# Tongji-MIC-Lab/TDVC

Measured on AMD Instinct MI355X. Metric: 1080p P-frames/sec (encode + reconstruct, lambda=2048 config), higher is better.
Workload: dtype f16; 1 GPU; 1x 1920x1080 (padded 1088x1920) 7-frame synthetic GOP (seed 1234), batch 1, P-frames coded in GOP order; gop=7, batch=1, parallelism=gop-sharded x1, weights=closed-form filler (no checkpoint ships)

## Files before the change

include/tdvc_hip.h:

```cpp
#ifndef TDVC_HIP_H
#define TDVC_HIP_H

#include <stdint.h>

#ifdef __cplusplus
extern "C" {
#endif

#define TDVC_OK 0
#define TDVC_EINVAL (-1)
#define TDVC_ENOSUP (-2)

typedef struct {
  void* p;
  int32_t N, H, W, C;
  int64_t sn;
  int32_t sp;
  int32_t dtype;
} tdvc_fmap;

enum { TDVC_F16 = 0, TDVC_F32 = 1 };
enum { TDVC_ACT_NONE = 0, TDVC_ACT_RELU = 1, TDVC_ACT_LRELU = 2, TDVC_ACT_CLAMP01 = 3, TDVC_ACT_SIGMOID = 4 };
enum { TDVC_GDN_NONE = 0, TDVC_GDN_FWD = 1, TDVC_GDN_INV = 2 };
enum { TDVC_OUT_NHWC = 0,
       TDVC_OUT_SHUFFLE2 = 1,
       TDVC_OUT_NCHW_F32 = 2 };

#define TDVC_MAX_TAPS 49

typedef struct {
  tdvc_fmap x;
  tdvc_fmap y;
  const void* w;
  const float* bias;
  int32_t cout;
  int32_t ntaps;
  int8_t tap_dy[TDVC_MAX_TAPS], tap_dx[TDVC_MAX_TAPS];
  int32_t kh, kw, stride, pad;
  int32_t ck;
  int32_t square_input;
  int32_t gdn;
  tdvc_fmap aux;
  int32_t act; float slope;
  int32_t round_before_act;
  tdvc_fmap res;
  tdvc_fmap res2;
  int32_t out_mode;
  int32_t s2d;
  int32_t bcast_T;
  float bcast_slope;
  float* chan_sum;
} tdvc_conv_desc;

int tdvc_abi_version(void);
const char* tdvc_last_error(void);
int tdvc_prepare_device(void);
const char* tdvc_last_conv_kernel(void);


int tdvc_conv_plan(int cin, int kh, int kw, int stride);
int64_t tdvc_conv_packed_bytes(int cout, int cin, int ntaps, int ck);
int tdvc_pack_conv_weights(const float* w_oihw, int cout, int cin_real, int cin, int kh, int kw,
                           int ntaps, const int8_t* tap_dy, const int8_t* tap_dx, int ck, uint16_t* dst);
int tdvc_conv2d(const tdvc_conv_desc* d, void* stream);
int tdvc_conv_chan_sum_rows(const tdvc_conv_desc* d);
int tdvc_conv2d_f32(const tdvc_conv_desc* d, void* stream);

typedef struct {
  tdvc_fmap x, y;
  const void* w;
  const float* bias;
  int32_t act1; float slope1;
  int32_t act2; float slope2;
  int32_t add_input;
  tdvc_fmap res2;
} tdvc_conv_pair_desc;
int64_t tdvc_conv_pair_packed_bytes(void);
int tdvc_pack_conv_pair_weights(const float* w1_oihw, const float* w2_oihw, uint16_t* dst);
int tdvc_conv_pair_supported(const tdvc_conv_pair_desc* d);
int tdvc_conv_pair(const tdvc_conv_pair_desc* d, void* stream);

typedef struct {
  tdvc_fmap x, om, y;
  const void* w;
  const float* bias;
  int32_t groups;
  int32_t act; float slope; int32_t round_before_act;
  void* x_planar;
} tdvc_dcn_desc;
int tdvc_dcn_fused(const tdvc_dcn_desc* d, void* stream);

int tdvc_dcn_v2_forward_f32(const float* input, const float* weight, const float* bias,
                            const float* offset, const float* mask, float* output,
                            int B, int C, int H, int W, int Cout,
                            int kh, int kw, int sh, int sw, int ph, int pw, int dh, int dw,
                            int deformable_group, void* stream);
int tdvc_dcn_v2_backward_f32(const float* input, const float* weight, const float* bias,
                             const float* offset, const float* mask, const float* grad_output,
                             float* grad_input, float* grad_offset, float* grad_mask,
                             float* grad_weight, float* grad_bias, float* columns,
                             int B, int C, int H, int W, int Cout,
                             int kh, int kw, int sh, int sw, int ph, int pw, int dh, int dw,
                             int deformable_group, void* stream);

int tdvc_nchw_to_fmap(const float* src, int C, const tdvc_fmap* y, void* stream);
int tdvc_fmap_to_nchw(const tdvc_fmap* x, int C, float* dst, void* stream);
int tdvc_scale_act_res(const tdvc_fmap* a, const float* gate, int act, float slope,
                       const tdvc_fmap* r, float r_sign, const tdvc_fmap* y, const tdvc_fmap* y2, void* stream);
int tdvc_add_flow(const tdvc_fmap* off, const tdvc_fmap* flow, void* stream);
int tdvc_bcast_add_act(const tdvc_fmap* x, const tdvc_fmap* b, int T, float slope, void* stream);

int tdvc_channel_sum(const tdvc_fmap* x, float* partial, int nblocks, void* stream);
int tdvc_se_gate(const float* partial, int nblocks, float inv_count, int N, int C, int Cmid,
                 const float* w1, const float* b1, const float* w2, const float* b2,
                 float* gate, void* stream);

int tdvc_upsample2x(const tdvc_fmap* x, const tdvc_fmap* y, void* stream);
int tdvc_avgpool2(const tdvc_fmap* x, const tdvc_fmap* y, void* stream);
int tdvc_spynet_level_input(const tdvc_fmap* ref, const tdvc_fmap* supp, const tdvc_fmap* flow_lo,
                            const tdvc_fmap* flow_up, const tdvc_fmap* cat8, void* stream);
int tdvc_resize_bilinear(const tdvc_fmap* x, const tdvc_fmap* y, const float* chscale, void* stream);

int64_t tdvc_avgpool_k_work_floats(int N, int hp, int wp, int C, int scale);
int tdvc_avgpool_k(const tdvc_fmap* x, int scale, float* pooled, int hp, int wp, float* work, int64_t work_floats, void* stream);
int tdvc_patch_match(const float* pin, const float* pref, int N, int hp, int wp, int C,
                     int32_t* idx, void* stream);
int tdvc_match_gather(const tdvc_fmap* fin, const tdvc_fmap* fref, const int32_t* idx, int scale,
                      int hp, int wp, const tdvc_fmap* cat, void* stream);

int tdvc_eb_forward(const tdvc_fmap* z, const float* params, const tdvc_fmap* noise,
                    const tdvc_fmap* z_hat, double* bits_out, float* partial, int partial_cap, void* stream);
int tdvc_gc_forward(const tdvc_fmap* y, const tdvc_fmap* gp, const tdvc_fmap* noise,
                    double* bits_out, float* partial, int partial_cap, void* stream);
int tdvc_quantize(const tdvc_fmap* y, const tdvc_fmap* noise, const tdvc_fmap* y_hat, void* stream);

int64_t tdvc_rans_encode(const int32_t* symbols, const int32_t* indexes, int64_t n,
                         const int32_t* cdfs, int32_t cdf_stride, const int32_t* cdf_sizes,
                         const int32_t* offsets, uint8_t* out, int64_t cap);
int tdvc_rans_decode(const uint8_t* data, int64_t nbytes, const int32_t* indexes, int64_t n,
                     const int32_t* cdfs, int32_t cdf_stride, const int32_t* cdf_sizes,
                     const int32_t* offsets, int32_t* symbols_out);

void* tdvc_rans_decoder_create(const uint8_t* data, int64_t nbytes);
int tdvc_rans_decoder_decode(void* handle, const int32_t* indexes, int64_t n, const int32_t* cdfs,
                             int32_t cdf_stride, const int32_t* cdf_sizes, const int32_t* offsets,
                             int32_t* symbols_out);
void tdvc_rans_decoder_destroy(void* handle);

int tdvc_pmf_to_quantized_cdf(const float* pmf, int n, int precision, int32_t* cdf_out);

int tdvc_ar_gather(const tdvc_fmap* y_hat, const tdvc_fmap* params, const int32_t* pos, int npos,
                   const tdvc_fmap* x1, const tdvc_fmap* pc, void* stream);
int tdvc_ar_quantize(const tdvc_fmap* y, const tdvc_fmap* gp, const int32_t* pos, int npos,
                     const float* scale_table, int ntable, const int32_t* symbols_in,
                     const tdvc_fmap* y_hat, int32_t* symbols, int32_t* indexes, void* stream);
int tdvc_ar_indexes(const tdvc_fmap* gp, const int32_t* pos, int npos, const float* scale_table, int ntable,
                    int M, int W, int32_t* indexes, void* stream);
int tdvc_ar_decode_serial(const uint8_t* data, int64_t nbytes, const int32_t* cdfs, int32_t cdf_stride, const int32_t* cdf_sizes,
                          const int32_t* offsets, const tdvc_fmap* y_hat, const tdvc_fmap* params, const tdvc_fmap* x1,
                          const tdvc_fmap* pc, const tdvc_conv_desc* convs, int nconvs, const tdvc_fmap* gp,
                          const int32_t* pos_table, int npos_total, int M, int W, const float* scale_table, int ntable,
                          int32_t* idx_dev, int32_t* sym_dev, void* stream);
int tdvc_ar_wavefront(const uint8_t* data, int64_t nbytes, const int32_t* cdfs, int32_t cdf_stride, const int32_t* cdf_sizes,
                      const int32_t* offsets, const tdvc_fmap* y, const tdvc_fmap* y_hat, const tdvc_fmap* params,
                      const tdvc_fmap* x1, const tdvc_fmap* pc, const tdvc_conv_desc* convs, int nconvs, const tdvc_fmap* gp,
                      const int32_t* pos_dev, const int32_t* step_sizes, int nsteps, int M, int W,
                      const float* scale_table, int ntable, int32_t* idx_dev, int32_t* sym_dev, void* stream);
int tdvc_round_symbols(const tdvc_fmap* z, const float* median, int32_t* out, void* stream);

int tdvc_pack_conv_weights_indexed(const float* w, const int32_t* row_off, const int32_t* chan_off, const int32_t* tap_off,
                                   const uint8_t* row_mask, const uint8_t* chan_mask, const uint8_t* tap_mask,
                                   int cout, int cin, int ntaps, int ck, void* dst, void* stream);
int tdvc_pack_conv_weights_indexed_f32(const float* w, const int32_t* row_off, const int32_t* chan_off, const int32_t* tap_off,
                                       const uint8_t* row_mask, const uint8_t* chan_mask, const uint8_t* tap_mask,
                                       int cout, int cin, int ntaps, int ck, float* dst, void* stream);
typedef struct tdvc_pack_job {
  const float* w;
  const int32_t *row_off, *chan_off, *tap_off;
  const uint8_t *row_mask, *chan_mask, *tap_mask;
  void* dst;
  const float* bias_src;
  float* bias_dst;
  const int32_t* bias_perm;
  int32_t cout, cin, ntaps, ck;
} tdvc_pack_job;
int64_t tdvc_pack_job_blocks(int cout, int cin, int ntaps, int ck);
int tdvc_pack_conv_weights_batch(const tdvc_pack_job* jobs, const int32_t* block_start, int njobs, int total_blocks, void* stream);
int64_t tdvc_conv_wgrad_work_floats(int cout, int cin, int ntaps, int N, int Ho, int Wo);
int tdvc_conv_wgrad(const tdvc_fmap* g, const tdvc_fmap* x, int cout, int kh, int kw, int stride, int pad,
                    int ntaps, const int8_t* tap_dy, const int8_t* tap_dx, const int32_t* row_off, const int32_t* chan_off,
                    const int32_t* tap_off, int square_x, float scale, float* dw, float* work, int64_t work_floats, void* stream);
int tdvc_conv_wgrad_bias(const tdvc_fmap* g, const tdvc_fmap* x, int cout, int kh, int kw, int stride, int pad,
                         int ntaps, const int8_t* tap_dy, const int8_t* tap_dx, const int32_t* row_off, const int32_t* chan_off,
                         const int32_t* tap_off, int square_x, float scale, float* dw, const int32_t* bias_index, float* db,
                         float* work, int64_t work_floats, void* stream);

typedef struct tdvc_wgrad_reduce_job {
  const float* work;
  const float* bwork;
  const int32_t *row_off, *chan_off, *tap_off, *bias_index;
  float *dw, *db;
  float scale;
  int32_t nworkers, cow, ciw, ntaps, cout, cin, wblocks, nblocks;
} tdvc_wgrad_reduce_job;
int tdvc_conv_wgrad_partials(const tdvc_fmap* g, const tdvc_fmap* x, int cout, int kh, int kw, int stride, int pad,
                             int ntaps, const int8_t* tap_dy, const int8_t* tap_dx, const int32_t* row_off, const int32_t* chan_off,
                             const int32_t* tap_off, int square_x, float scale, float* dw, const int32_t* bias_index, float* db,
                             float* work, int64_t work_floats, tdvc_wgrad_reduce_job* job, void* stream);
int tdvc_wgrad_reduce_batch(const tdvc_wgrad_reduce_job* jobs, const int32_t* block_start, int njobs, int total_blocks, void* stream);

int tdvc_act_backward(const tdvc_fmap* g, const tdvc_fmap* y, const tdvc_fmap* res, int act, float slope, const tdvc_fmap* out, void* stream);
int tdvc_pixel_unshuffle(const tdvc_fmap* y, const tdvc_fmap* out, void* stream);
int64_t tdvc_bias_grad_work_floats(int N, int C);
int tdvc_bias_grad(const tdvc_fmap* g, int nvalid, const int32_t* dst_index, float scale, float* db, float* work, int64_t work_floats, void* stream);

int tdvc_copy_cast(const tdvc_fmap* src, const tdvc_fmap* dst, void* stream);
int tdvc_clamp01_backward(const tdvc_fmap* g, const tdvc_fmap* y, void* stream);
int64_t tdvc_gate_backward_work_floats(int N, int C);
int tdvc_gate_backward(const tdvc_fmap* g, const tdvc_fmap* a, const float* gate, const tdvc_fmap* da, float* dgate, float* work,
                       int64_t work_floats, void* stream);
int tdvc_se_gate_backward(const float* partial, int nblocks, float inv_count, int N, int C, int Cmid, const float* w1, const float* b1,
                          const float* w2, const float* b2, const float* gate, const float* dgate, float scale, float* dmean,
                          float* dw1, float* db1, float* dw2, float* db2, void* stream);
int tdvc_bcast_channel_add(const tdvc_fmap* dx, const float* v, float scale, void* stream);
int tdvc_add_flow_backward(const tdvc_fmap* doff, const tdvc_fmap* dflow, void* stream);
int tdvc_bcast_add_act_backward(const tdvc_fmap* dx, const tdvc_fmap* x, const tdvc_fmap* db, float slope, void* stream);
int tdvc_upsample2x_backward(const tdvc_fmap* dy, const tdvc_fmap* dx, void* stream);
int tdvc_resize_bilinear_backward(const tdvc_fmap* dy, const tdvc_fmap* dx, const float* chscale, void* stream);

int tdvc_spynet_level_input_backward(const tdvc_fmap* supp, const tdvc_fmap* flow_up, const tdvc_fmap* dcat8, const tdvc_fmap* dflow_up,
                                     const tdvc_fmap* dflow_lo, void* stream);

int tdvc_sigmoid_f32(const float* x, float* out, int64_t n, void* stream);
int tdvc_sigmoid_backward_f32(float* g, const float* s, int64_t n, void* stream);
int tdvc_axpy_f32(float* dst, const float* src, float scale, int64_t n, void* stream);

int tdvc_match_gather_backward(const tdvc_fmap* fin, const tdvc_fmap* fref, const int32_t* idx, int scale, int hp, int wp,
                               const tdvc_fmap* dcat, const tdvc_fmap* dfin, const tdvc_fmap* dfref, void* stream);

int tdvc_gdn_backward(const tdvc_fmap* g, const tdvc_fmap* x, const tdvc_fmap* n32, int inverse, const tdvc_fmap* dn, const tdvc_fmap* dx, void* stream);
int tdvc_mul2_accumulate(const tdvc_fmap* dx, const tdvc_fmap* x, const tdvc_fmap* t, void* stream);

int tdvc_eb_backward(const tdvc_fmap* z, const float* params, const tdvc_fmap* noise, float gscale, const tdvc_fmap* dz, float* dparams, void* stream);
int tdvc_gc_backward(const tdvc_fmap* y, const tdvc_fmap* gp, const tdvc_fmap* noise, float gscale, const tdvc_fmap* dy, const tdvc_fmap* dgp, void* stream);
int tdvc_eb_pack(const float* const* raw, const float* quantiles, float* packed, int C, void* stream);
int tdvc_eb_param_chain(const float* dpacked, const float* const* raw, float* const* grad, float scale, int C, void* stream);
int tdvc_eb_aux(const float* params, const float* quantiles, float target, float* dq, float* loss, int C, void* stream);

int tdvc_dcn_columns(const tdvc_fmap* x, const tdvc_fmap* om, int groups, const tdvc_fmap* col, void* stream);
int64_t tdvc_dcn_col2im_work_floats(int N, int H, int W, int groups);
int tdvc_dcn_col2im(const tdvc_fmap* x, const tdvc_fmap* om, const tdvc_fmap* dcol, int groups, float* dx32, const tdvc_fmap* dom,
                    float* work, int64_t work_floats, void* stream);
int tdvc_dcn_col2im_det(const tdvc_fmap* x, const tdvc_fmap* om, const tdvc_fmap* dcol, int groups, float* dx32, const tdvc_fmap* dom,
                        float* work, int64_t work_floats, int64_t* far_keys, float* far_vals, int32_t* far_count, int32_t far_cap, void* stream);
int tdvc_dcn_far_apply(const int64_t* keys_sorted, const int64_t* order, const float* far_vals, int32_t count, float* dx32, void* stream);

int64_t tdvc_ssim_level_work_floats(int N, int C, int H, int W, int win_size);
int tdvc_ssim_level(const float* x, const float* y, int N, int C, int H, int W, const float* win, int win_size,
                    float c1, float c2, float* ssim_out, float* cs_out, float* work, int64_t work_floats, void* stream);
int tdvc_avgpool2_pad_f32(const float* x, int64_t planes, int H, int W, float* out, void* stream);

#ifdef __cplusplus
}
#endif
#endif
```

tdvc_amd/_lib.py:

```python
from __future__ import annotations

import ctypes as C
import os

_HERE = os.path.dirname(os.path.abspath(__file__))
LIB_PATH = os.path.join(_HERE, "libtdvc_hip.so")

MAX_TAPS = 49
F16, F32 = 0, 1
ACT_NONE, ACT_RELU, ACT_LRELU, ACT_CLAMP01, ACT_SIGMOID = 0, 1, 2, 3, 4
GDN_NONE, GDN_FWD, GDN_INV = 0, 1, 2
OUT_NHWC, OUT_SHUFFLE2, OUT_NCHW_F32 = 0, 1, 2


class FMapDesc(C.Structure):
    _fields_ = [("p", C.c_void_p), ("N", C.c_int32), ("H", C.c_int32), ("W", C.c_int32), ("C", C.c_int32),
                ("sn", C.c_int64), ("sp", C.c_int32), ("dtype", C.c_int32)]


class ConvDesc(C.Structure):
    _fields_ = [("x", FMapDesc), ("y", FMapDesc), ("w", C.c_void_p), ("bias", C.c_void_p),
                ("cout", C.c_int32), ("ntaps", C.c_int32),
                ("tap_dy", C.c_int8 * MAX_TAPS), ("tap_dx", C.c_int8 * MAX_TAPS),
                ("kh", C.c_int32), ("kw", C.c_int32), ("stride", C.c_int32), ("pad", C.c_int32),
                ("ck", C.c_int32), ("square_input", C.c_int32), ("gdn", C.c_int32),
                ("aux", FMapDesc), ("act", C.c_int32), ("slope", C.c_float),
                ("round_before_act", C.c_int32), ("res", FMapDesc), ("res2", FMapDesc), ("out_mode", C.c_int32), ("s2d", C.c_int32),
                ("bcast_T", C.c_int32), ("bcast_slope", C.c_float), ("chan_sum", C.c_void_p)]


class DcnDesc(C.Structure):
    _fields_ = [("x", FMapDesc), ("om", FMapDesc), ("y", FMapDesc), ("w", C.c_void_p), ("bias", C.c_void_p),
                ("groups", C.c_int32), ("act", C.c_int32), ("slope", C.c_float), ("round_before_act", C.c_int32), ("x_planar", C.c_void_p)]


class ConvPairDesc(C.Structure):
    _fields_ = [("x", FMapDesc), ("y", FMapDesc), ("w", C.c_void_p), ("bias", C.c_void_p), ("act1", C.c_int32), ("slope1", C.c_float),
                ("act2", C.c_int32), ("slope2", C.c_float), ("add_input", C.c_int32), ("res2", FMapDesc)]


class WgradReduceJob(C.Structure):
    _fields_ = [("work", C.c_void_p), ("bwork", C.c_void_p), ("row_off", C.c_void_p), ("chan_off", C.c_void_p), ("tap_off", C.c_void_p),
                ("bias_index", C.c_void_p), ("dw", C.c_void_p), ("db", C.c_void_p), ("scale", C.c_float),
                ("nworkers", C.c_int32), ("cow", C.c_int32), ("ciw", C.c_int32), ("ntaps", C.c_int32), ("cout", C.c_int32), ("cin", C.c_int32),
                ("wblocks", C.c_int32), ("nblocks", C.c_int32)]


_P = C.c_void_p
_FM = C.POINTER(FMapDesc)
_i, _f, _i64 = C.c_int, C.c_float, C.c_int64

SIGNATURES = {
    "tdvc_abi_version": (_i, []),
    "tdvc_conv_chan_sum_rows": (_i, [C.POINTER(ConvDesc)]),
    "tdvc_last_error": (C.c_char_p, []),
    "tdvc_last_conv_kernel": (C.c_char_p, []),
    "tdvc_prepare_device": (_i, []),
    "tdvc_conv_plan": (_i, [_i, _i, _i, _i]),
    "tdvc_conv_packed_bytes": (_i64, [_i, _i, _i, _i]),
    "tdvc_pack_conv_weights": (_i, [_P, _i, _i, _i, _i, _i, _i, _P, _P, _i, _P]),
    "tdvc_conv2d": (_i, [C.POINTER(ConvDesc), _P]),
    "tdvc_conv2d_f32": (_i, [C.POINTER(ConvDesc), _P]),
    "tdvc_pack_conv_weights_indexed": (_i, [_P] * 7 + [_i] * 4 + [_P, _P]),
    "tdvc_pack_conv_weights_indexed_f32": (_i, [_P] * 7 + [_i] * 4 + [_P, _P]),
    "tdvc_pack_job_blocks": (_i64, [_i, _i, _i, _i]),
    "tdvc_pack_conv_weights_batch": (_i, [_P, _P, _i, _i, _P]),
    "tdvc_act_backward": (_i, [_FM, _FM, _FM, _i, _f, _FM, _P]),
    "tdvc_pixel_unshuffle": (_i, [_FM, _FM, _P]),
    "tdvc_bias_grad_work_floats": (_i64, [_i, _i]),
    "tdvc_bias_grad": (_i, [_FM, _i, _P, _f, _P, _P, _i64, _P]),
    "tdvc_copy_cast": (_i, [_FM, _FM, _P]),
    "tdvc_clamp01_backward": (_i, [_FM, _FM, _P]),
    "tdvc_gate_backward_work_floats": (_i64, [_i, _i]),
    "tdvc_gate_backward": (_i, [_FM, _FM, _P, _FM, _P, _P, _i64, _P]),
    "tdvc_se_gate_backward": (_i, [_P, _i, _f, _i, _i, _i] + [_P] * 6 + [_f] + [_P] * 6),
    "tdvc_bcast_channel_add": (_i, [_FM, _P, _f, _P]),
    "tdvc_add_flow_backward": (_i, [_FM, _FM, _P]),
    "tdvc_bcast_add_act_backward": (_i, [_FM, _FM, _FM, _f, _P]),
    "tdvc_upsample2x_backward": (_i, [_FM, _FM, _P]),
    "tdvc_resize_bilinear_backward": (_i, [_FM, _FM, _P, _P]),
    "tdvc_spynet_level_input_backward": (_i, [_FM, _FM, _FM, _FM, _FM, _P]),
    "tdvc_sigmoid_f32": (_i, [_P, _P, _i64, _P]),
    "tdvc_sigmoid_backward_f32": (_i, [_P, _P, _i64, _P]),
    "tdvc_axpy_f32": (_i, [_P, _P, _f, _i64, _P]),
    "tdvc_match_gather_backward": (_i, [_FM, _FM, _P, _i, _i, _i, _FM, _FM, _FM, _P]),
    "tdvc_eb_backward": (_i, [_FM, _P, _FM, _f, _FM, _P, _P]),
    "tdvc_eb_pack": (_i, [_P, _P, _P, _i, _P]),
    "tdvc_eb_param_chain": (_i, [_P, _P, _P, _f, _i, _P]),
    "tdvc_eb_aux": (_i, [_P, _P, _f, _P, _P, _i, _P]),
    "tdvc_gc_backward": (_i, [_FM, _FM, _FM, _f, _FM, _FM, _P]),
    "tdvc_dcn_columns": (_i, [_FM, _FM, _i, _FM, _P]),
    "tdvc_ar_decode_serial": (_i, [_P, _i64, _P, _i, _P, _P, _FM, _FM, _FM, _FM, _P, _i, _FM, _P, _i, _i, _i, _P, _i, _P, _P, _P]),
    "tdvc_ar_wavefront": (_i, [_P, _i64, _P, _i, _P, _P, _FM, _FM, _FM, _FM, _FM, _P, _i, _FM, _P, _P, _i, _i, _i, _P, _i, _P, _P, _P]),
    "tdvc_ssim_level_work_floats": (_i64, [_i] * 5),
    "tdvc_ssim_level": (_i, [_P, _P, _i, _i, _i, _i, _P, _i, _f, _f, _P, _P, _P, _i64, _P]),
    "tdvc_avgpool2_pad_f32": (_i, [_P, _i64, _i, _i, _P, _P]),
    "tdvc_dcn_col2im_work_floats": (_i64, [_i, _i, _i, _i]),
    "tdvc_dcn_col2im": (_i, [_FM, _FM, _FM, _i, _P, _FM, _P, _i64, _P]),
    "tdvc_dcn_col2im_det": (_i, [_FM, _FM, _FM, _i, _P, _FM, _P, _i64, _P, _P, _P, _i, _P]),
    "tdvc_dcn_far_apply": (_i, [_P, _P, _P, _i, _P, _P]),
    "tdvc_conv_wgrad_work_floats": (_i64, [_i] * 6),
    "tdvc_conv_wgrad": (_i, [_FM, _FM] + [_i] * 6 + [_P] * 5 + [_i, _f, _P, _P, _i64, _P]),
    "tdvc_conv_wgrad_bias": (_i, [_FM, _FM] + [_i] * 6 + [_P] * 5 + [_i, _f, _P, _P, _P, _P, _i64, _P]),
    "tdvc_conv_wgrad_partials": (_i, [_FM, _FM] + [_i] * 6 + [_P] * 5 + [_i, _f, _P, _P, _P, _P, _i64, C.POINTER(WgradReduceJob), _P]),
    "tdvc_wgrad_reduce_batch": (_i, [_P, _P, _i, _i, _P]),
    "tdvc_gdn_backward": (_i, [_FM, _FM, _FM, _i, _FM, _FM, _P]),
    "tdvc_mul2_accumulate": (_i, [_FM, _FM, _FM, _P]),
    "tdvc_dcn_fused": (_i, [C.POINTER(DcnDesc), _P]),
    "tdvc_conv_pair_packed_bytes": (_i64, []),
    "tdvc_pack_conv_pair_weights": (_i, [_P, _P, _P]),
    "tdvc_conv_pair_supported": (_i, [C.POINTER(ConvPairDesc)]),
    "tdvc_conv_pair": (_i, [C.POINTER(ConvPairDesc), _P]),
    "tdvc_dcn_v2_forward_f32": (_i, [_P] * 6 + [_i] * 14 + [_P]),
    "tdvc_dcn_v2_backward_f32": (_i, [_P] * 12 + [_i] * 14 + [_P]),
    "tdvc_nchw_to_fmap": (_i, [_P, _i, _FM, _P]),
    "tdvc_fmap_to_nchw": (_i, [_FM, _i, _P, _P]),
    "tdvc_scale_act_res": (_i, [_FM, _P, _i, _f, _FM, _f, _FM, _FM, _P]),
    "tdvc_add_flow": (_i, [_FM, _FM, _P]),
    "tdvc_bcast_add_act": (_i, [_FM, _FM, _i, _f, _P]),
    "tdvc_channel_sum": (_i, [_FM, _P, _i, _P]),
    "tdvc_se_gate": (_i, [_P, _i, _f, _i, _i, _i, _P, _P, _P, _P, _P, _P]),
    "tdvc_upsample2x": (_i, [_FM, _FM, _P]),
    "tdvc_avgpool2": (_i, [_FM, _FM, _P]),
    "tdvc_spynet_level_input": (_i, [_FM, _FM, _FM, _FM, _FM, _P]),
    "tdvc_resize_bilinear": (_i, [_FM, _FM, _P, _P]),
    "tdvc_avgpool_k_work_floats": (_i64, [_i, _i, _i, _i, _i]),
    "tdvc_avgpool_k": (_i, [_FM, _i, _P, _i, _i, _P, _i64, _P]),
    "tdvc_patch_match": (_i, [_P, _P, _i, _i, _i, _i, _P, _P]),
    "tdvc_match_gather": (_i, [_FM, _FM, _P, _i, _i, _i, _FM, _P]),
    "tdvc_eb_forward": (_i, [_FM, _P, _FM, _FM, _P, _P, _i, _P]),
    "tdvc_gc_forward": (_i, [_FM, _FM, _FM, _P, _P, _i, _P]),
    "tdvc_quantize": (_i, [_FM, _FM, _FM, _P]),
    "tdvc_rans_encode": (_i64, [_P, _P, _i64, _P, C.c_int32, _P, _P, _P, _i64]),
    "tdvc_rans_decode": (_i, [_P, _i64, _P, _i64, _P, C.c_int32, _P, _P, _P]),
    "tdvc_rans_decoder_create": (_P, [_P, _i64]),
    "tdvc_rans_decoder_decode": (_i, [_P, _P, _i64, _P, C.c_int32, _P, _P, _P]),
    "tdvc_rans_decoder_destroy": (None, [_P]),
    "tdvc_pmf_to_quantized_cdf": (_i, [_P, _i, _i, _P]),
    "tdvc_ar_gather": (_i, [_FM, _FM, _P, _i, _FM, _FM, _P]),
    "tdvc_ar_quantize": (_i, [_FM, _FM, _P, _i, _P, _i, _P, _FM, _P, _P, _P]),
    "tdvc_ar_indexes": (_i, [_FM, _P, _i, _P, _i, _i, _i, _P, _P]),
    "tdvc_round_symbols": (_i, [_FM, _P, _P, _P]),
}

_lib = None


class TdvcHipError(RuntimeError):
    pass


def lib():
    global _lib
    if _lib is None:
        if not os.path.exists(LIB_PATH):
            raise TdvcHipError(
                f"{LIB_PATH} is missing: build it with `python -c 'import __graft_entry__ as g; g.build()'` "
                "(hipcc --offload-arch=gfx950).  tdvc_amd has no CPU fallback.")
        l = C.CDLL(LIB_PATH)
        for name, (res, args) in SIGNATURES.items():
            fn = getattr(l, name)
            fn.restype = res
            fn.argtypes = args
        _lib = l
    return _lib


def check(rc: int, what: str = ""):
    if rc != 0:
        msg = lib().tdvc_last_error().decode("utf-8", "replace")
        raise TdvcHipError(f"{what}: rc={rc}: {msg}")
```

tdvc_amd/csrc/conv_mfma.hip:

```cpp
#include "conv_common.h"

using convk::ConvParams;
int launch_conv_v2(const ConvParams& p, int ntiles, int cout_blocks, int N, hipStream_t st);
bool conv_v2_eligible(const tdvc_conv_desc* d, int Ho, int Wo);
int launch_conv_v3(const ConvParams& p, int cout_blocks, int N, hipStream_t st);
bool conv_v3_eligible(const tdvc_conv_desc* d, int Ho, int Wo);
int launch_conv_v5(const ConvParams& p, int cout_blocks, int N, hipStream_t st);
bool conv_v5_eligible(const tdvc_conv_desc* d, int Ho, int Wo);
int conv_v5_chan_sum_rows(int Ho, int Wo, int cout_blocks, int N);
int launch_conv_v7(const ConvParams& p, int cout_blocks, int N, hipStream_t st);
bool conv_v7_eligible(const tdvc_conv_desc* d, const ConvParams& p, int Ho, int Wo);
int launch_conv_v11(const ConvParams& p, int cout_blocks, int N, hipStream_t st);
bool conv_v11_eligible(const tdvc_conv_desc* d, const ConvParams& p, int Ho, int Wo);
int launch_conv_row(int geo, const ConvParams& p, int N, hipStream_t st);
int conv_row_geometry(const tdvc_conv_desc* d, const ConvParams& p, int Ho, int Wo);
int launch_conv_v10(const ConvParams& p, int cout_blocks, int N, hipStream_t st);
bool conv_v10_eligible(const tdvc_conv_desc* d, const ConvParams& p, int Ho, int Wo);
int launch_conv_v9(const ConvParams& p, int ck8, int cout_tiles32, int N, hipStream_t st);
bool conv_v9_eligible(const tdvc_conv_desc* d, int Ho, int Wo, bool v3_ok);
bool conv_c8_eligible(const tdvc_conv_desc* d, const ConvParams& p, int Ho, int Wo);
int launch_conv_c8(const ConvParams& p, int N, hipStream_t st);
bool conv_n16_eligible(const tdvc_conv_desc* d, int Ho, int Wo);
int launch_conv_n16(const ConvParams& p, int N, hipStream_t st);
bool gdn128_eligible(const tdvc_conv_desc* d, const ConvParams& p, int Ho, int Wo);
int launch_gdn128(const ConvParams& p, int N, hipStream_t st);

namespace {

constexpr int TH = 8, TW = 32;

template <int CK8, int MT, int STRIDE, bool LEAN = false>
__global__ __launch_bounds__(256, LEAN ? 3 : 1) void conv_mfma_kernel(const ConvParams p) {
  extern __shared__ __attribute__((aligned(16))) unsigned char smem[];
  constexpr int CK = CK8 * 8;
  constexpr int PS = (CK8 == 1) ? 16 : CK * 2 + 16;
  int* tapoff = reinterpret_cast<int*>(smem);
  unsigned char* tile = smem + 256;

  const int tid = threadIdx.x, lane = tid & 63, wave = tid >> 6;
  const int hh = lane >> 5, r = lane & 31;
  const int tile_id = p.reverse ? (int)gridDim.x - 1 - tdvc_xcd_tile(blockIdx.x) : tdvc_xcd_tile(blockIdx.x);
  const int tx = tile_id % p.tiles_x, ty = tile_id / p.tiles_x;
  const int cb = blockIdx.y, n = blockIdx.z;

  const int TIH = (TH - 1) * STRIDE + p.kh;
  const int TIW = (TW - 1) * STRIDE + p.kw;
  const int HALFW = (TIW + 1) >> 1;
  const int TIWp = (STRIDE == 2) ? 2 * HALFW : TIW;

  if (tid < p.ntaps) {
    const int dy = p.tap_dy[tid], dx = p.tap_dx[tid];
    tapoff[tid] = (STRIDE == 2) ? (dy * TIWp + (dx & 1) * HALFW + (dx >> 1)) * PS : (dy * TIWp + dx) * PS;
  }

  int base[2];
#pragma unroll
  for (int nt = 0; nt < 2; ++nt) base[nt] = (((wave * 2 + nt) * STRIDE) * TIWp + r) * PS;

  f32x16 acc[MT][2];
#pragma unroll
  for (int mt = 0; mt < MT; ++mt)
#pragma unroll
    for (int nt = 0; nt < 2; ++nt)
#pragma unroll
      for (int i = 0; i < 16; ++i) acc[mt][nt][i] = 0.f;

  const half_t* xn = p.x + (long)n * p.x_sn;
  const int iy0 = ty * TH * STRIDE - p.pad, ix0 = tx * TW * STRIDE - p.pad;
  const int total = TIH * TIW * CK8;

  for (int ch = 0; ch < p.nchunks; ++ch) {
    if (ch > 0) __syncthreads();
    for (int idx = tid; idx < total; idx += 256) {
      const int c8 = idx % CK8;
      const int pix = idx / CK8;
      const int c = pix % TIW, rr = pix / TIW;
      const int iy = iy0 + rr, ix = ix0 + c;
      const int cg = ch * CK + c8 * 8;
      half8 v = {0, 0, 0, 0, 0, 0, 0, 0};
      if (iy >= 0 && iy < p.H && ix >= 0 && ix < p.W && cg < p.Cin)
        v = *reinterpret_cast<const half8*>(xn + ((long)iy * p.W + ix) * p.x_sp + cg);
      if (p.square) v = v * v;
      const int cpos = (STRIDE == 2) ? ((c & 1) * HALFW + (c >> 1)) : c;
      *reinterpret_cast<half8*>(tile + (rr * TIWp + cpos) * PS + c8 * 16) = v;
    }
    __syncthreads();

    const half_t* wp[MT];
#pragma unroll
    for (int mt = 0; mt < MT; ++mt)
      wp[mt] = p.w + ((((long)(cb * MT + mt) * p.nchunks + ch) * p.steps) * 64 + lane) * 8;

    if constexpr (CK8 == 1) {
      for (int s = 0; s < p.steps; ++s) {
        int tap = 2 * s + hh;
        tap = tap < p.ntaps ? tap : p.ntaps - 1;
        const int toff = tapoff[tap];
        half8 a[MT], b[2];
#pragma unroll
        for (int mt = 0; mt < MT; ++mt) { a[mt] = *reinterpret_cast<const half8*>(wp[mt]); wp[mt] += 512; }
#pragma unroll
        for (int nt = 0; nt < 2; ++nt) b[nt] = *reinterpret_cast<const half8*>(tile + base[nt] + toff);
#pragma unroll
        for (int mt = 0; mt < MT; ++mt)
#pragma unroll
          for (int nt = 0; nt < 2; ++nt)
            acc[mt][nt] = __builtin_amdgcn_mfma_f32_32x32x16_f16(a[mt], b[nt], acc[mt][nt], 0, 0, 0);
      }
    } else {
      for (int tap = 0; tap < p.ntaps; ++tap) {
        const int toff = tapoff[tap] + hh * 16;
#pragma unroll
        for (int s2 = 0; s2 < CK8 / 2; ++s2) {
          half8 a[MT], b[2];
#pragma unroll
          for (int mt = 0; mt < MT; ++mt) { a[mt] = *reinterpret_cast<const half8*>(wp[mt]); wp[mt] += 512; }
#pragma unroll
          for (int nt = 0; nt < 2; ++nt)
            b[nt] = *reinterpret_cast<const half8*>(tile + base[nt] + toff + s2 * 32);
#pragma unroll
          for (int mt = 0; mt < MT; ++mt)
#pragma unroll
            for (int nt = 0; nt < 2; ++nt)
              acc[mt][nt] = __builtin_amdgcn_mfma_f32_32x32x16_f16(a[mt], b[nt], acc[mt][nt], 0, 0, 0);
        }
      }
    }
  }

  if constexpr (MT == 2 && LEAN) {
    __syncthreads();
    convk::epilogue_simple_rows<2, false, 2>(p, acc, p.bias + cb * 64, tile + wave * (32 * 144), n, cb * 64,
                                             ty * TH + wave * 2, tx * TW, lane, false);
    return;
  } else if constexpr (MT == 2) {
    if (p.simple) {
      __syncthreads();
      convk::epilogue_simple_rows<2, false, 1>(p, acc, p.bias + cb * 64, tile + wave * (32 * 144), n, cb * 64,
                                               ty * TH + wave * 2, tx * TW, lane, false);
      return;
    }
  }
  const int ox = tx * TW + r;
#pragma unroll
  for (int nt = 0; nt < 2; ++nt) {
    const int oy = ty * TH + wave * 2 + nt;
    if (oy >= p.Ho || ox >= p.Wo) continue;
#pragma unroll
    for (int mt = 0; mt < MT; ++mt) {
#pragma unroll
      for (int g = 0; g < 4; ++g) {
        const int co = (cb * MT + mt) * 32 + 8 * g + 4 * hh;
        float v[4];
#pragma unroll
        for (int i = 0; i < 4; ++i) v[i] = acc[mt][nt][4 * g + i];
        convk::epilogue4(p, n, oy, ox, co, v);
      }
    }
  }
}

template <int CK8, int MT, int STRIDE>
int launch(const ConvParams& p, dim3 grid, size_t lds, hipStream_t st) {
  if constexpr (MT == 2) {
    if (p.simple == 2) {
      hipLaunchKernelGGL((conv_mfma_kernel<CK8, MT, STRIDE, true>), grid, dim3(256), lds, st, p);
      return tdvc_launch_status("tdvc_conv2d");
    }
  }
  hipLaunchKernelGGL((conv_mfma_kernel<CK8, MT, STRIDE, false>), grid, dim3(256), lds, st, p);
  return tdvc_launch_status("tdvc_conv2d");
}

template <int CK8, int MT>
int launch_s(const ConvParams& p, int stride, dim3 grid, size_t lds, hipStream_t st) {
  return stride == 1 ? launch<CK8, MT, 1>(p, grid, lds, st) : launch<CK8, MT, 2>(p, grid, lds, st);
}

template <int CK8>
int launch_m(const ConvParams& p, int mt, int stride, dim3 grid, size_t lds, hipStream_t st) {
  return mt == 1 ? launch_s<CK8, 1>(p, stride, grid, lds, st) : launch_s<CK8, 2>(p, stride, grid, lds, st);
}

inline int lds_bytes(int ck, int kh, int kw, int stride) {
  const int ps = (ck == 8) ? 16 : ck * 2 + 16;
  const int tih = (TH - 1) * stride + kh, tiw = (TW - 1) * stride + kw;
  const int tiwp = stride == 2 ? 2 * ((tiw + 1) >> 1) : tiw;
  return 256 + tih * tiwp * ps;
}

inline int cout_tiles(int cout) { return cout <= 32 ? 1 : 2 * ((cout + 63) / 64); }

}

extern "C" int tdvc_conv_plan(int cin, int kh, int kw, int stride) {
  if (cin <= 0 || (cin % 8) != 0 || kh < 1 || kw < 1 || kh > 7 || kw > 7 || (stride != 1 && stride != 2)) {
    tdvc_set_error("tdvc_conv_plan: unsupported geometry cin=%d k=%dx%d stride=%d", cin, kh, kw, stride);
    return TDVC_EINVAL;
  }
  const int cands[4] = {64, 32, 16, 8};
  for (int i = 0; i < 4; ++i) {
    const int ck = cands[i];
    if (ck > cin && ck != 8) {
      if (cin % ck != 0 && cin < ck) continue;
    }
    if (lds_bytes(ck, kh, kw, stride) <= 64 * 1024) return ck;
  }
  tdvc_set_error("tdvc_conv_plan: no LDS plan for k=%dx%d stride=%d", kh, kw, stride);
  return TDVC_EINVAL;
}

extern "C" int64_t tdvc_conv_packed_bytes(int cout, int cin, int ntaps, int ck) {
  if (cout <= 0 || cin <= 0 || ntaps <= 0 || ntaps > TDVC_MAX_TAPS || (ck != 8 && ck != 16 && ck != 32 && ck != 64)) return TDVC_EINVAL;
  const int ck8 = ck / 8;
  const int64_t nchunks = (cin + ck - 1) / ck;
  const int64_t steps = (ntaps * ck8 + 1) / 2;
  return (int64_t)cout_tiles(cout) * nchunks * steps * 64 * 8 * 2;
}

extern "C" int tdvc_pack_conv_weights(const float* w, int cout, int cin_real, int cin, int kh, int kw,
                                      int ntaps, const int8_t* tap_dy, const int8_t* tap_dx, int ck, uint16_t* dst) {
  TDVC_CHECK(w && dst && tap_dy && tap_dx, "tdvc_pack_conv_weights: null pointer");
  TDVC_CHECK(tdvc_conv_packed_bytes(cout, cin, ntaps, ck) > 0, "tdvc_pack_conv_weights: bad geometry");
  TDVC_CHECK(cin_real <= cin, "tdvc_pack_conv_weights: cin_real > cin");
  const int ck8 = ck / 8;
  const int nchunks = (cin + ck - 1) / ck;
  const int steps = (ntaps * ck8 + 1) / 2;
  const int tiles = cout_tiles(cout);
  half_t* out = reinterpret_cast<half_t*>(dst);
  for (int t = 0; t < tiles; ++t)
    for (int ch = 0; ch < nchunks; ++ch)
      for (int s = 0; s < steps; ++s)
        for (int lane = 0; lane < 64; ++lane) {
          const int r = lane & 31, h = lane >> 5;
          const int co = t * 32 + r;
          const int kc = 2 * s + h;
          half_t* o = out + ((((int64_t)t * nchunks + ch) * steps + s) * 64 + lane) * 8;
          for (int j = 0; j < 8; ++j) {
            float v = 0.f;
            if (kc < ntaps * ck8 && co < cout) {
              const int tap = kc / ck8, c8 = kc % ck8;
              const int ci = ch * ck + c8 * 8 + j;
              const int dy = tap_dy[tap], dx = tap_dx[tap];
              if (ci < cin_real && dy >= 0 && dy < kh && dx >= 0 && dx < kw)
                v = w[(((int64_t)co * cin_real + ci) * kh + dy) * kw + dx];
            }
            o[j] = (half_t)v;
          }
        }
  return TDVC_OK;
}

static thread_local char g_last_kernel[48] = "";

static thread_local unsigned g_walk_parity = 0;
static int g_walk_mode = -1;
extern "C" void tdvc_debug_set_conv_walk(int mode) { g_walk_mode = mode; }
static int next_walk_reverse() {
  if (g_walk_mode < 0) { const char* e = getenv("TDVC_CONV_WALK"); g_walk_mode = e ? atoi(e) : 1; }
  return g_walk_mode == 1 ? (int)(g_walk_parity++ & 1u) : 0;
}

static int conv2d_impl(const tdvc_conv_desc* d, void* stream, bool query_rows) {
  TDVC_CHECK(d, "tdvc_conv2d: null descriptor");
  if (d->x.dtype == TDVC_F32) {
    if (query_rows) return 0;
    TDVC_CHECK(!d->chan_sum, "tdvc_conv2d: chan_sum is not available on the fp32 path (tdvc_conv_chan_sum_rows() == 0)");
    snprintf(g_last_kernel, sizeof(g_last_kernel), "conv_f32");
    return tdvc_conv2d_f32(d, stream);
  }
  TDVC_CHECK(fmap_ok16(d->x), "tdvc_conv2d: input must be an fp16 fmap with C,sp %% 8 == 0 and 16-byte aligned");
  TDVC_CHECK(d->w && aligned16(d->w), "tdvc_conv2d: weights null/unaligned");
  TDVC_CHECK(d->stride == 1 || d->stride == 2, "tdvc_conv2d: stride %d unsupported", d->stride);
  TDVC_CHECK(d->ntaps >= 1 && d->ntaps <= TDVC_MAX_TAPS && d->kh >= 1 && d->kh <= 7 && d->kw >= 1 && d->kw <= 7,
             "tdvc_conv2d: bad kernel %dx%d ntaps=%d", d->kh, d->kw, d->ntaps);
  TDVC_CHECK(d->ck == 8 || d->ck == 16 || d->ck == 32 || d->ck == 64, "tdvc_conv2d: bad ck %d", d->ck);
  TDVC_CHECK(d->cout >= 1, "tdvc_conv2d: cout");
  for (int t = 0; t < d->ntaps; ++t)
    TDVC_CHECK(d->tap_dy[t] >= 0 && d->tap_dy[t] < d->kh && d->tap_dx[t] >= 0 && d->tap_dx[t] < d->kw,
               "tdvc_conv2d: tap %d out of the %dx%d window", t, d->kh, d->kw);
  int Ho = (d->x.H + 2 * d->pad - d->kh) / d->stride + 1;
  int Wo = (d->x.W + 2 * d->pad - d->kw) / d->stride + 1;
  if (d->s2d) {
    TDVC_CHECK(d->kh == 2 && d->kw == 2 && d->stride == 1 && d->pad == 1 && d->ntaps == 4 && d->ck == 32 && !d->square_input && !d->gdn,
               "tdvc_conv2d: s2d expects the virtual 2x2 / stride 1 / pad 1 conv packed with ck=32");
    TDVC_CHECK((d->x.H % 2) == 0 && (d->x.W % 2) == 0 && (d->x.C % 32) == 0 && d->cout >= 64,
               "tdvc_conv2d: s2d needs even H, W, C %% 32 == 0 and cout >= 64 (got %dx%dx%d, cout %d)", d->x.H, d->x.W, d->x.C, d->cout);
    Ho = d->x.H / 2;
    Wo = d->x.W / 2;
  }
  TDVC_CHECK(Ho > 0 && Wo > 0, "tdvc_conv2d: empty output");
  TDVC_CHECK((long)Ho * Wo * 4 < 2147483647L && (long)d->x.H * d->x.W < 2147483647L, "tdvc_conv2d: image too large (pixel indices are 32-bit)");
  const int lds = lds_bytes(d->ck, d->kh, d->kw, d->stride);

  const int shuf = d->out_mode == TDVC_OUT_SHUFFLE2;
  if (d->out_mode == TDVC_OUT_NCHW_F32) {
    TDVC_CHECK(d->y.p && d->y.N == d->x.N, "tdvc_conv2d: NCHW output null / batch mismatch");
  } else {
    TDVC_CHECK(d->y.dtype == TDVC_F32 ? fmap_ok32(d->y) : fmap_ok16(d->y), "tdvc_conv2d: bad output fmap");
    TDVC_CHECK(d->y.N == d->x.N && d->y.H == (shuf ? 2 * Ho : Ho) && d->y.W == (shuf ? 2 * Wo : Wo),
               "tdvc_conv2d: output geometry %dx%d does not match conv result %dx%d%s", d->y.H, d->y.W, Ho, Wo,
               shuf ? " (x2 shuffle)" : "");
    if (shuf) TDVC_CHECK((d->cout % 128) == 0, "tdvc_conv2d: SHUFFLE2 needs cout %% 128 == 0");
    if (d->y.dtype == TDVC_F16) TDVC_CHECK((d->y.C % 8) == 0, "tdvc_conv2d: fp16 output C %% 8");
  }
  if (d->gdn) {
    TDVC_CHECK(fmap_ok16(d->aux) && d->aux.H == Ho && d->aux.W == Wo && d->aux.N == d->x.N && d->aux.C >= d->cout &&
                   !shuf && (d->cout % 64) == 0,
               "tdvc_conv2d: GDN aux fmap mismatch");
  }
  if (d->res.p) {
    TDVC_CHECK(d->res.dtype == TDVC_F32 ? fmap_ok32(d->res) : fmap_ok16(d->res), "tdvc_conv2d: bad residual fmap");
    TDVC_CHECK(d->res.N == d->x.N && d->res.H == (shuf ? 2 * Ho : Ho) && d->res.W == (shuf ? 2 * Wo : Wo),
               "tdvc_conv2d: residual geometry mismatch");
  }
  if (d->res2.p) {
    TDVC_CHECK(fmap_ok16(d->res2) && d->res2.N == d->x.N && d->res2.H == (shuf ? 2 * Ho : Ho) && d->res2.W == (shuf ? 2 * Wo : Wo),
               "tdvc_conv2d: bad second residual fmap");
  }
  if (d->bias) TDVC_CHECK(aligned16(d->bias), "tdvc_conv2d: bias unaligned");

  ConvParams p;
  memset(&p, 0, sizeof(p));
  p.x = reinterpret_cast<const half_t*>(d->x.p); p.x_sn = d->x.sn; p.x_sp = d->x.sp;
  p.H = d->x.H; p.W = d->x.W; p.Cin = d->x.C;
  p.w = reinterpret_cast<const half_t*>(d->w); p.bias = d->bias;
  p.y = to_dev(d->y); p.Ho = Ho; p.Wo = Wo; p.cout = d->cout;
  p.aux = d->gdn ? to_dev(d->aux) : null_fmap();
  p.res = d->res.p ? to_dev(d->res) : null_fmap();
  p.res2 = d->res2.p ? to_dev(d->res2) : null_fmap();
  p.ntaps = d->ntaps; p.kh = d->kh; p.kw = d->kw; p.pad = d->pad;
  p.in_stride = d->stride;
  const int ck8 = d->ck / 8;
  p.s2d = d->s2d; p.Corig = d->x.C;
  p.bcast_T = d->bcast_T; p.bcast_slope = d->bcast_slope;
  p.nchunks = d->s2d ? (4 * d->x.C) / d->ck : (d->x.C + d->ck - 1) / d->ck;
  p.steps = (d->ntaps * ck8 + 1) / 2;
  p.square = d->square_input; p.gdn = d->gdn; p.act = d->act; p.slope = d->slope;
  p.round16 = d->round_before_act; p.out_mode = d->out_mode;
  memcpy(p.tap_dy, d->tap_dy, sizeof(p.tap_dy));
  memcpy(p.tap_dx, d->tap_dx, sizeof(p.tap_dx));
  const int tiles_x = (Wo + TW - 1) / TW, tiles_y = (Ho + TH - 1) / TH;
  p.tiles_x = tiles_x;
  p.reverse = query_rows ? 0 : next_walk_reverse();
  p.csum = nullptr;
  const int tiles = cout_tiles(d->cout);
  const int mt = tiles == 1 ? 1 : 2;
  if (mt == 2 && convk::conv_is_simple(p)) {
    p.simple = convk::conv_is_lean(p) ? 2 : 1;
    p.slope = convk::conv_simple_slope(p);
  }
  {
    const bool csum_ok = !d->bcast_T && !d->s2d && tiles == 2 && p.simple == 2 && !conv_v9_eligible(d, Ho, Wo, conv_v3_eligible(d, Ho, Wo)) &&
                         !gdn128_eligible(d, p, Ho, Wo) && conv_v5_eligible(d, Ho, Wo);
    if (query_rows) return csum_ok ? conv_v5_chan_sum_rows(Ho, Wo, 1, d->x.N) : 0;
    TDVC_CHECK(!d->chan_sum || (csum_ok && (reinterpret_cast<uintptr_t>(d->chan_sum) & 15) == 0),
               "tdvc_conv2d: chan_sum on a conv whose kernel has no fused channel sum (tdvc_conv_chan_sum_rows() == 0) or unaligned");
    p.csum = d->chan_sum;
  }
  hipStream_t st = reinterpret_cast<hipStream_t>(stream);
  auto chose = [](const char* name) { snprintf(g_last_kernel, sizeof(g_last_kernel), "%s", name); };
  if (d->bcast_T) {
    TDVC_CHECK(d->bcast_T == 4 && d->kh == 1 && d->kw == 1 && d->stride == 1 && d->pad == 0 && d->cout == 64 && d->y.C == 64 && d->y.sp >= 4 * 64 &&
                   d->y.dtype == TDVC_F16 && d->out_mode == TDVC_OUT_NHWC && d->act == TDVC_ACT_NONE && !d->gdn && !d->res.p && !d->res2.p &&
                   !d->square_input && !d->round_before_act && d->bias && d->bcast_slope >= 0.f && d->bcast_slope <= 1.f && conv_v5_eligible(d, Ho, Wo) &&
                   convk::conv_is_lean(p),
               "tdvc_conv2d: bcast_T needs a plain 1x1 / stride 1 conv to 64 channels of >= 8192 pixels, y a 64-channel window of a buffer with >= 4 slices, bcast_T == 4");
    p.simple = 2;
    p.slope = 1.f;
    chose("conv_mfma_v5(bcast)");
    return launch_conv_v5(p, 1, d->x.N, st);
  }
  if (d->s2d) {
    if (const int geo = conv_row_geometry(d, p, Ho, Wo); geo >= 0) { chose("conv_row(s2d)"); return launch_conv_row(geo, p, d->x.N, st); }
    TDVC_CHECK(conv_v3_eligible(d, Ho, Wo), "tdvc_conv2d: s2d conv not eligible for the stage-pipelined kernel");
    chose("conv_mfma_v3(s2d)");
    return launch_conv_v3(p, tiles / 2, d->x.N, st);
  }
  if (conv_v9_eligible(d, Ho, Wo, conv_v3_eligible(d, Ho, Wo))) { chose("conv_mfma_v9"); return launch_conv_v9(p, ck8, tiles, d->x.N, st); }
  if (gdn128_eligible(d, p, Ho, Wo)) { chose("gdn128"); return launch_gdn128(p, d->x.N, st); }
  if (conv_v5_eligible(d, Ho, Wo)) { chose("conv_mfma_v5"); return launch_conv_v5(p, tiles / 2, d->x.N, st); }
  if (conv_c8_eligible(d, p, Ho, Wo)) { chose("conv_c8"); return launch_conv_c8(p, d->x.N, st); }
  if (conv_n16_eligible(d, Ho, Wo)) { chose("conv_n16"); return launch_conv_n16(p, d->x.N, st); }
  if (const int geo = conv_row_geometry(d, p, Ho, Wo); geo >= 0) { chose("conv_row"); return launch_conv_row(geo, p, d->x.N, st); }
  if (conv_v10_eligible(d, p, Ho, Wo)) { chose("conv_mfma_v10"); return launch_conv_v10(p, tiles / 2, d->x.N, st); }
  if (conv_v7_eligible(d, p, Ho, Wo)) { chose("conv_mfma_v7"); return launch_conv_v7(p, tiles / 2, d->x.N, st); }
  if (conv_v11_eligible(d, p, Ho, Wo)) { chose("conv_mfma_v11"); return launch_conv_v11(p, tiles / 2, d->x.N, st); }
  if (conv_v3_eligible(d, Ho, Wo)) { chose("conv_mfma_v3"); return launch_conv_v3(p, tiles / 2, d->x.N, st); }
  if (conv_v2_eligible(d, Ho, Wo)) { chose("conv_mfma_v2"); return launch_conv_v2(p, 0, tiles / 2, d->x.N, st); }
  TDVC_CHECK(lds <= 64 * 1024, "tdvc_conv2d: LDS plan %d bytes too large for the direct kernel (use tdvc_conv_plan)", lds);
  dim3 grid(tiles_x * tiles_y, tiles / mt, d->x.N);
  snprintf(g_last_kernel, sizeof(g_last_kernel), "conv_mfma<%d,%d,%d>", ck8, mt, d->stride);
  const size_t lds_v1 = (p.simple && lds < 256 + 4 * 32 * 144) ? 256 + 4 * 32 * 144 : lds;
  switch (ck8) {
    case 1: return launch_m<1>(p, mt, d->stride, grid, lds_v1, st);
    case 2: return launch_m<2>(p, mt, d->stride, grid, lds_v1, st);
    case 4: return launch_m<4>(p, mt, d->stride, grid, lds_v1, st);
    default: return launch_m<8>(p, mt, d->stride, grid, lds_v1, st);
  }
}

extern "C" int tdvc_conv2d(const tdvc_conv_desc* d, void* stream) { return conv2d_impl(d, stream, false); }
extern "C" int tdvc_conv_chan_sum_rows(const tdvc_conv_desc* d) { return conv2d_impl(d, nullptr, true); }

extern "C" const char* tdvc_last_conv_kernel(void) { return g_last_kernel; }
```

tdvc_amd/csrc/conv_row.hip:

```cpp
#include <type_traits>

#include "conv_common.h"

using convk::ConvParams;

namespace {

enum { GEO_C128 = 0, GEO_C64 = 1, GEO_C128W = 2, GEO_S2D64 = 3 };
template <int GID> struct RowGeo;
template <> struct RowGeo<GEO_C128> { static constexpr int NKC = 4, KH = 3, KW = 3, SW = 32, NCG = 8, PIECES = 9, XRING = 8, PF = 6, HD = 4, DMA_POS = 1, CORIG = 128; static constexpr bool S2D = false; };
template <> struct RowGeo<GEO_C64> { static constexpr int NKC = 2, KH = 3, KW = 3, SW = 64, NCG = 4, PIECES = 9, XRING = 8, PF = 6, HD = 4, DMA_POS = 2, CORIG = 64; static constexpr bool S2D = false; };
template <> struct RowGeo<GEO_C128W> { static constexpr int NKC = 4, KH = 3, KW = 3, SW = 64, NCG = 4, PIECES = 17, XRING = 6, PF = 4, HD = 2, DMA_POS = 2, CORIG = 128; static constexpr bool S2D = false; };
template <> struct RowGeo<GEO_S2D64> { static constexpr int NKC = 8, KH = 2, KW = 2, SW = 32, NCG = 8, PIECES = 17, XRING = 6, PF = 4, HD = 2, DMA_POS = 1, CORIG = 64; static constexpr bool S2D = true; };
template <int GID> struct RowDerived : RowGeo<GID> {
  using G = RowGeo<GID>;
  static constexpr int CO = 16 * G::NCG;
  static constexpr int PXB = G::NKC * 64;
  static constexpr int LPP = PXB / 16;
  static constexpr int SLOTS = CO / 8;
  static constexpr int ROWB = G::PIECES * 1024;
  static constexpr int STEPS = (G::KH * G::KW * 4 + 1) / 2;
  static constexpr int NP = G::PIECES / 4 + 1;
  static constexpr int X0 = 0, S0 = G::XRING * ROWB, B0 = S0 + 4 * 8192, LDS = B0 + 512;
  static_assert(G::SW * CO * 2 == 8192, "a staging row is 8 KB = 512 items of 16 bytes");
  static_assert((G::SW + G::KW - 1) * PXB <= ROWB && (G::PIECES % 4) == 1, "ring row");
  static_assert(G::SW / 16 == 2 * (8 / G::NCG), "a wave computes two column blocks");
  static_assert(G::PF + 2 <= G::XRING && G::PF >= G::HD + 2, "ring conditions (BI = 2)");
  static_assert(G::HD == 4 || G::HD == 2, "land_wait(): four-step history with the odd piece going round the loaders, or two steps with a fixed owner");
  static_assert(LDS <= 160 * 1024, "LDS");
};
constexpr int RW_BI = 2;
constexpr int RW_SRING = 2 * RW_BI;
constexpr int RW_SROW = 8192;
constexpr int RW_NTHR = 512;
#ifndef RW_DMA_POS
#define RW_DMA_POS G::DMA_POS
#endif

struct RowParams {
  const half_t* x; long x_sn; int x_sp;
  half_t* y; long y_sn; int y_sp;
  const half_t* res; long r1_sn; int r1_sp;
  const half_t* w;
  const float* bias;
  const half_t* zeros;
  half_t* dump;
  int N, H, W;
  int Win;
  int ncb;
  int cq;
  int strips;
  float slope;
  int reverse;
};

template <int PXB> __device__ __forceinline__ int rw_f(int q) {
  return PXB == 128 ? ((q >> 1) & 7) : ((q & 12) | ((q & 1) << 1) | ((q >> 1) & 1));
}
__device__ __forceinline__ int rw_sigma(int r) { return r < 4 ? 2 * r : (r >= 12 ? 2 * r - 16 : 2 * r - 7); }
__device__ __forceinline__ int rw_g(int q) { return (q >> 1) & 7; }

__device__ __forceinline__ void rw_glds16(const half_t* gsrc, unsigned lds_dst) {
  unsigned keep;
  asm volatile("s_mov_b32 %0, m0\n\ts_mov_b32 m0, %2\n\ts_nop 0\n\tglobal_load_lds_dwordx4 %1, off\n\ts_mov_b32 m0, %0"
               : "=&s"(keep) : "v"(gsrc), "s"(lds_dst) : "memory");
}
template <int XRING> __device__ __forceinline__ int rw_slot(int kk) {
  if constexpr ((XRING & (XRING - 1)) == 0) return kk & (XRING - 1);
  else return __builtin_amdgcn_readfirstlane(kk) % XRING;
}
__device__ __forceinline__ void rw_barrier(bool skip = false) {
  asm volatile("s_waitcnt lgkmcnt(0)" ::: "memory");
  if (!skip) __builtin_amdgcn_s_barrier();
  asm volatile("" ::: "memory");
}

template <int GID> constexpr bool rw_frag(int dy, int dx, int kc) {
  using G = RowGeo<GID>;
  if (!G::S2D) return true;
  const int q = kc / (G::CORIG / 32), py = q >> 1, px = q & 1;
  return (dy == 1 || py == 1) && (dx == 1 || px == 1);
}
template <int GID> constexpr bool rw_group(int dx, int kc) {
  for (int dy = 0; dy < RowGeo<GID>::KH; ++dy)
    if (rw_frag<GID>(dy, dx, kc)) return true;
  return false;
}
template <int GID> constexpr int rw_ngroups() {
  int n = 0;
  for (int g = 0; g < RowGeo<GID>::KW * RowGeo<GID>::NKC; ++g) n += rw_group<GID>(g % RowGeo<GID>::KW, g / RowGeo<GID>::KW);
  return n;
}
template <int GID> constexpr int rw_group_at(int i) {
  int n = 0;
  for (int g = 0; g < RowGeo<GID>::KW * RowGeo<GID>::NKC; ++g)
    if (rw_group<GID>(g % RowGeo<GID>::KW, g / RowGeo<GID>::KW)) {
      if (n == i) return g;
      ++n;
    }
  return -1;
}
template <int GID> constexpr int rw_first_group_of_row0() {
  for (int i = 0; i < rw_ngroups<GID>(); ++i) {
    const int g = rw_group_at<GID>(i);
    if (rw_frag<GID>(0, g % RowGeo<GID>::KW, g / RowGeo<GID>::KW)) return i;
  }
  return -1;
}

template <int GID, int ACT, int NRES, bool SHUF>
__global__ __launch_bounds__(RW_NTHR, 1) void conv_row_kernel(const RowParams p) {
  using G = RowDerived<GID>;
  constexpr int NKC = G::NKC, KH = G::KH, KW = G::KW, SW = G::SW, CO = G::CO, PXB = G::PXB, XRING = G::XRING, PF = G::PF, NP = G::NP;
  constexpr int NG = rw_ngroups<GID>(), G0 = rw_first_group_of_row0<GID>();
  extern __shared__ __attribute__((aligned(1024))) unsigned char smem[];
  const unsigned lds0 = static_cast<unsigned>(reinterpret_cast<uintptr_t>(smem));
  const int tid = threadIdx.x, lane = tid & 63;
  const int wave = __builtin_amdgcn_readfirstlane(tid >> 6);
  const bool loader = wave < 4;
  const int wq = wave & 3;
  const int cg = wave % G::NCG, cbp = wave / G::NCG;
  const int r16 = lane & 15, kb = lane >> 4;

  const int nwg = (int)gridDim.x, b = (int)blockIdx.x;
  int cbk, pos_slot, nslots;
  if ((nwg & 7) == 0 && ((nwg >> 3) % p.ncb) == 0) {
    const int slot = b >> 3, per_xcd = (nwg >> 3) / p.ncb;
    cbk = slot % p.ncb;
    pos_slot = (b & 7) * per_xcd + slot / p.ncb;
    nslots = 8 * per_xcd;
  } else {
    cbk = b % p.ncb; pos_slot = b / p.ncb; nslots = nwg / p.ncb;
  }
  if (p.reverse) pos_slot = nslots - 1 - pos_slot;
  const long allrows = (long)p.N * p.strips * p.H;
  const long run_begin = allrows * pos_slot / nslots, run_end = allrows * (pos_slot + 1) / nslots;

  half8 wf[KH * KW * NKC];
  {
    const int co = cbk * CO + 16 * cg + r16;
    const half_t* wb = p.w + ((long)(co >> 5) * NKC * G::STEPS * 64 + (kb & 1) * 32 + (co & 31)) * 8 + (long)(kb >> 1) * 512;
#pragma unroll
    for (int tap = 0; tap < KH * KW; ++tap)
#pragma unroll
      for (int kc = 0; kc < NKC; ++kc)
        if (rw_frag<GID>(tap / KW, tap % KW, kc))
          wf[tap * NKC + kc] = *reinterpret_cast<const half8*>(wb + ((long)kc * G::STEPS + tap * 2) * 512);
  }
  if (tid < CO) reinterpret_cast<float*>(smem + G::B0)[tid] = p.bias[cbk * CO + tid];
  const int boff = G::B0 + (16 * cg + 4 * kb) * 4;

  int foff[KW];
#pragma unroll
  for (int dx = 0; dx < KW; ++dx) {
    const int q = 32 * cbp + dx + rw_sigma(r16), f = rw_f<PXB>(q);
    foff[dx] = q * PXB + ((kb ^ f) << 4);
  }
  int doff[2];
#pragma unroll
  for (int cb = 0; cb < 2; ++cb) {
    const int q = 32 * cbp + 16 * cb + rw_sigma(r16), c = 2 * cg + (kb >> 1);
    doff[cb] = q * (CO * 2) + ((c ^ rw_g(q)) << 4) + 8 * (kb & 1);
  }
  auto run = [&](auto LOADERc) __attribute__((always_inline)) {
  constexpr bool LOADER = decltype(LOADERc)::value;
  constexpr int SRC = G::S2D ? NP : 2;
  constexpr int QSTEP = 4 * (64 / G::LPP);
  static_assert(G::S2D || (QSTEP % 16) == 0, "regular pieces of a loader share their swizzle terms");
  int soff[SRC], sq[SRC];
#pragma unroll
  for (int j = 0; j < SRC; ++j) {
    const int piece = j == SRC - 1 ? G::PIECES - 1 : wq + 4 * j;
    const int q = (64 / G::LPP) * piece + lane / G::LPP, c = (lane % G::LPP) ^ rw_f<PXB>(q);
    sq[j] = q;
    if constexpr (G::S2D) {
      const int par = c / (G::CORIG / 8), within = c % (G::CORIG / 8);
      soff[j] = (2 * q + (par & 1)) * p.x_sp + (par >> 1) * p.Win * p.x_sp + within * 8;
    } else {
      soff[j] = q * p.x_sp + c * 8;
    }
  }
  const int s_t = tid & 255;
  int s_px[2], s_co[2];
#pragma unroll
  for (int j = 0; j < 2; ++j) {
    const int it = s_t + 256 * j;
    s_px[j] = it / G::SLOTS;
    s_co[j] = cbk * CO + (((it % G::SLOTS) ^ rw_g(it / G::SLOTS)) << 3);
  }
  int s_pc[2], s_sub[2];
#pragma unroll
  for (int j = 0; j < 2; ++j) {
    if constexpr (SHUF) { s_sub[j] = s_co[j] / p.cq; s_pc[j] = s_co[j] - s_sub[j] * p.cq; }
    else { s_sub[j] = 0; s_pc[j] = s_co[j]; }
  }
  const int OW = SHUF ? 2 * p.W : p.W;

  const half_t hs = (half_t)p.slope;
  const half4 sl4 = {hs, hs, hs, hs};
  f32x4 acc[KH][2];
  half8 r1v[2] = {};

  for (long pos = run_begin; pos < run_end;) {
    const int sid = (int)(pos / p.H);
    const int ra = (int)(pos - (long)sid * p.H), rb = (int)min((long)p.H, ra + (run_end - pos));
    const int rows = rb - ra;
    pos += rows;
    const int n = sid / p.strips, strip = sid - n * p.strips;
    const int c0 = strip * SW;
    const half_t* xn = p.x + (long)n * p.x_sn;
    const int last_in = rows + KH - 2;

    unsigned colok = 0;
#pragma unroll
    for (int j = 0; j < NP; ++j) {
      const int q = G::S2D ? sq[j] : (j == NP - 1 ? sq[1] : sq[0] + QSTEP * j);
      colok |= (q < SW + KW - 1 && c0 - 1 + q >= 0 && c0 - 1 + q < p.W) ? (1u << j) : 0u;
    }
    bool s_ok[2];
    int y_lo[2], r_lo[2];
#pragma unroll
    for (int j = 0; j < 2; ++j) {
      const int col = c0 + s_px[j], colc = min(col, p.W - 1);
      s_ok[j] = col < p.W;
      const int off = SHUF ? (s_sub[j] >> 1) * OW + 2 * col + (s_sub[j] & 1) : col;
      const int offc = SHUF ? (s_sub[j] >> 1) * OW + 2 * colc + (s_sub[j] & 1) : colc;
      y_lo[j] = off * p.y_sp + s_pc[j];
      r_lo[j] = offc * p.r1_sp + s_pc[j];
    }
    const half_t* const yimg = p.y + (long)n * p.y_sn;
    const half_t* const rimg = NRES >= 1 ? p.res + (long)n * p.r1_sn : nullptr;
    const long yrow_stride = (long)(SHUF ? 2 : 1) * OW * p.y_sp, rrow_stride = (long)(SHUF ? 2 : 1) * OW * p.r1_sp;
    const long xrow_stride = (long)(G::S2D ? 2 : 1) * p.Win * p.x_sp;
    const half_t* const xcol = xn + (long)(G::S2D ? 2 : 1) * (c0 - 1) * p.x_sp;
#pragma unroll
    for (int s3 = 0; s3 < KH; ++s3)
#pragma unroll
      for (int cb = 0; cb < 2; ++cb) acc[s3][cb] = f32x4{0.f, 0.f, 0.f, 0.f};

    auto issue_row = [&](int kk) __attribute__((always_inline)) -> int {
      const int row = ra - 1 + kk;
      const bool rowok = row >= 0 && row < p.H;
      const half_t* base = xcol + row * xrow_stride;
      const unsigned dst = lds0 + G::X0 + rw_slot<XRING>(kk) * G::ROWB;
      const unsigned okb = rowok ? colok : 0u;
      if constexpr (G::S2D || NP <= 3) {
#pragma unroll
        for (int j = 0; j < NP - 1; ++j) {
          const half_t* src = G::S2D ? base + soff[j] : base + (long)(QSTEP * j) * p.x_sp + soff[0];
          rw_glds16(((okb >> j) & 1u) ? src : p.zeros, dst + (wq + 4 * j) * 1024);
        }
      } else {
#pragma nounroll
        for (int j = 0; j < NP - 1; ++j) {
          const half_t* src = base + (long)(QSTEP * j) * p.x_sp + soff[0];
          rw_glds16(((okb >> j) & 1u) ? src : p.zeros, dst + (wq + 4 * j) * 1024);
        }
      }
      if (G::HD == 4 ? wq == (kk & 3) : wq == 0) {
        rw_glds16(((okb >> (NP - 1)) & 1u) ? base + soff[SRC - 1] : p.zeros, dst + (G::PIECES - 1) * 1024);
        return NP;
      }
      return NP - 1;
    };

    if constexpr (LOADER) {
#pragma unroll
      for (int kk = 0; kk < PF; ++kk)
        if (kk <= last_in) issue_row(kk);
    }
    asm volatile("s_waitcnt vmcnt(0)" ::: "memory");
    rw_barrier();

    const int K = (rows + KH - 1 + RW_BI + RW_BI - 1) & ~(RW_BI - 1);
    auto land_wait = [&](int nvm) __attribute__((always_inline)) {
      if (!nvm) { asm volatile("s_waitcnt vmcnt(0)" ::: "memory"); return; }
      if constexpr (G::HD == 4) {
        static_assert(G::HD != 4 || NP == 3, "vmcnt(9)");
        asm volatile("s_waitcnt vmcnt(9)" ::: "memory");
      } else {
        static_assert(G::HD != 2 || NP == 5, "vmcnt(10) / vmcnt(8)");
        if (wq == 0) asm volatile("s_waitcnt vmcnt(10)" ::: "memory");
        else asm volatile("s_waitcnt vmcnt(8)" ::: "memory");
      }
    };

    auto step = [&](auto PHc, auto FULLc, int k) __attribute__((always_inline)) {
      constexpr int PH = decltype(PHc)::value;
      constexpr bool FULL = decltype(FULLc)::value;
      constexpr int SD = (PH + 1) % KH;
      if constexpr (!LOADER) {
        const int srow = ra + k - RW_BI - (KH - 1);
        if (FULL || (srow >= ra && srow < rb)) {
          const unsigned char* sb = smem + G::S0 + ((k - RW_BI) & (RW_SRING - 1)) * RW_SROW;
          half_t* const yrow = const_cast<half_t*>(yimg) + srow * yrow_stride;
#pragma unroll
          for (int j = 0; j < 2; ++j) {
            half8 yv = *reinterpret_cast<const half8*>(sb + (s_t + 256 * j) * 16);
            if constexpr (NRES >= 1) yv = yv + r1v[j];
            *reinterpret_cast<half8*>(s_ok[j] ? yrow + y_lo[j] : p.dump + (s_t + 256 * j) * 8) = yv;
          }
        }
        if constexpr (NRES >= 1) {
          const int nrow = srow + 1;
          const bool rok = FULL || (nrow >= ra && nrow < rb);
          const half_t* const rrow = rimg + (rok ? nrow : ra) * rrow_stride;
#pragma unroll
          for (int j = 0; j < 2; ++j) r1v[j] = *reinterpret_cast<const half8*>(rrow + r_lo[j]);
        }
      }
      int nvm = 0;
      if (FULL || k <= last_in) {
        const unsigned char* xb = smem + G::X0 + rw_slot<XRING>(k) * G::ROWB;
        constexpr int FBN = (PXB == 256 && (NRES == 1 || GID == GEO_C128W)) ? 2 : 3;
        half8 fb[FBN][2];
        auto load_group = [&](int gi, int buf) __attribute__((always_inline)) {
          const int g = rw_group_at<GID>(gi), kc = g / KW, dx = g - KW * kc;
          const unsigned char* b0 = xb + (foff[dx] ^ (kc << 6));
#pragma unroll
          for (int cb = 0; cb < 2; ++cb) fb[buf][cb] = *reinterpret_cast<const half8*>(b0 + cb * 16 * PXB);
        };
        const f32x4 bias4 = *reinterpret_cast<const f32x4*>(smem + boff);
        load_group(0, 0);
        if (FBN == 3) load_group(1, 1);
        if (RW_DMA_POS == 0 && LOADER && k + PF <= last_in) nvm = issue_row(k + PF);
#pragma unroll
        for (int gi = 0; gi < NG; ++gi) {
          const int g = rw_group_at<GID>(gi), kc = g / KW, dx = g - KW * kc;
          if (gi + FBN - 1 < NG) load_group(gi + FBN - 1, (gi + FBN - 1) % FBN);
          if (RW_DMA_POS == 1 && gi == NG / 2 && LOADER && k + PF <= last_in) nvm = issue_row(k + PF);
#pragma unroll
          for (int dyo = 0; dyo < KH; ++dyo) {
            const int dy = KH - 1 - dyo;
            if (!rw_frag<GID>(dy, dx, kc)) continue;
            const int slot = (PH + KH - dy) % KH;
#pragma unroll
            for (int cb = 0; cb < 2; ++cb) {
              const bool first = dy == 0 && gi == G0;
              acc[slot][cb] = __builtin_amdgcn_mfma_f32_16x16x32_f16(wf[(dy * KW + dx) * NKC + kc], fb[gi % FBN][cb],
                                                                     first ? bias4 : acc[slot][cb], 0, 0, 0);
            }
          }
        }
        if (RW_DMA_POS == 2 && LOADER && k + PF <= last_in) nvm = issue_row(k + PF);
        {
          unsigned char* sb = smem + G::S0 + (k & (RW_SRING - 1)) * RW_SROW;
#pragma unroll
          for (int cb = 0; cb < 2; ++cb) {
            const f32x4 v = acc[SD][cb];
            half4 h = {(half_t)v[0], (half_t)v[1], (half_t)v[2], (half_t)v[3]};
            if constexpr (ACT == 1) {
              const half4 z = {(half_t)0.f, (half_t)0.f, (half_t)0.f, (half_t)0.f};
              h = __builtin_elementwise_max(h, z);
            } else if constexpr (ACT == 2) {
              h = __builtin_elementwise_max(h, h * sl4);
            }
            *reinterpret_cast<half4*>(sb + doff[cb]) = h;
          }
        }
      }
      if constexpr (LOADER) land_wait(nvm);
      rw_barrier((k & (RW_BI - 1)) != RW_BI - 1);
    };
    auto steps_of = [&](auto FULLc, int k0, int kend) __attribute__((always_inline)) {
      step(std::integral_constant<int, 0>{}, FULLc, k0);
      if (k0 + 1 < kend) step(std::integral_constant<int, 1 % KH>{}, FULLc, k0 + 1);
      if constexpr (KH == 3) {
        if (k0 + 2 < kend) step(std::integral_constant<int, 2 % KH>{}, FULLc, k0 + 2);
      }
    };
    constexpr int KF = ((RW_BI + KH - 1 + KH - 1) / KH) * KH;
    int k = 0;
    for (; k < KF; k += KH) steps_of(std::false_type{}, k, KF);
    for (; k + KH - 1 <= last_in; k += KH) steps_of(std::true_type{}, k, k + KH);
    for (; k < K; k += KH) steps_of(std::false_type{}, k, K);
    rw_barrier();
  }
  };
  if (loader) run(std::true_type{});
  else run(std::false_type{});
}

}

static int g_row_enabled = 15;
extern "C" void tdvc_debug_enable_conv_row(int enable) { g_row_enabled = enable; }

static bool row_off() {
  static const bool off = getenv("TDVC_CONV_NO_ROW") != nullptr || getenv("TDVC_CONV_V1") != nullptr;
  return off || !g_row_enabled;
}

int conv_row_geometry(const tdvc_conv_desc* d, const ConvParams& p, int Ho, int Wo) {
  if (row_off() || d->ck != 32 || d->square_input || !d->bias || (long)Ho * Wo < 8192 || Ho < 16 || (d->res.p && d->res2.p)) return -1;
  const bool shuf = p.out_mode == TDVC_OUT_SHUFFLE2;
  const int ych = shuf ? (d->cout >> 2) : d->cout;
  if (d->y.C < ych || (d->res.p && d->res.C < ych) || (d->res2.p && d->res2.C < ych)) return -1;
  if (d->s2d) {
    const bool ok = (g_row_enabled & 8) && d->x.C == 64 && (d->cout % 128) == 0 && convk::conv_is_lean(p) && d->kh == 2 && d->kw == 2 && d->ntaps == 4 &&
                    d->tap_dy[0] == 0 && d->tap_dx[0] == 0 && d->tap_dy[1] == 0 && d->tap_dx[1] == 1 && d->tap_dy[2] == 1 && d->tap_dx[2] == 0 &&
                    d->tap_dy[3] == 1 && d->tap_dx[3] == 1;
    return ok ? GEO_S2D64 : -1;
  }
  bool taps33 = d->ntaps == 9 && d->kh == 3 && d->kw == 3 && d->pad == 1 && d->stride == 1;
  for (int t = 0; taps33 && t < 9; ++t) taps33 = d->tap_dy[t] == t / 3 && d->tap_dx[t] == t % 3;
  if (!taps33) return -1;
  const bool lean = convk::conv_is_lean(p);
  if (d->x.C == 128 && (d->cout % 128) == 0 && (g_row_enabled & 1) && (lean || (convk::conv_is_simple(p) && !p.gdn && shuf && (ych % 8) == 0))) return GEO_C128;
  if (d->x.C == 128 && (d->cout % 64) == 0 && (g_row_enabled & 4) && lean) return GEO_C128W;
  if (d->x.C == 64 && (d->cout % 64) == 0 && (g_row_enabled & 2) && lean) return GEO_C64;
  return -1;
}

template <int GID>
static int launch_conv_row_t(const ConvParams& p, int N, hipStream_t st) {
  using G = RowDerived<GID>;
  const void* zeros = nullptr;
  void* dump = nullptr;
  if (const int zrc = tdvc_scratch_pages(&zeros, &dump)) return zrc;
  RowParams q;
  q.x = p.x; q.x_sn = p.x_sn; q.x_sp = p.x_sp;
  q.y = reinterpret_cast<half_t*>(p.y.p); q.y_sn = p.y.sn; q.y_sp = p.y.sp;
  q.res = reinterpret_cast<const half_t*>(p.res.p); q.r1_sn = p.res.p ? p.res.sn : 0; q.r1_sp = p.res.p ? p.res.sp : 0;
  q.w = p.w; q.bias = p.bias;
  q.zeros = reinterpret_cast<const half_t*>(zeros);
  q.dump = reinterpret_cast<half_t*>(dump);
  q.N = N; q.H = p.Ho; q.W = p.Wo; q.Win = p.W;
  q.ncb = p.cout / G::CO;
  const bool shuf = p.out_mode == TDVC_OUT_SHUFFLE2;
  q.cq = shuf ? p.cout >> 2 : 0;
  q.slope = convk::conv_simple_slope(p);
  q.reverse = p.reverse;
  q.strips = (q.W + G::SW - 1) / G::SW;
  const long allrows = (long)N * q.strips * q.H;
  int per = 256 / q.ncb;
  if (per < 1) per = 1;
  if (allrows < per) per = (int)allrows;
  const int grid = per * q.ncb;
  if (!p.res.p && p.res2.p) {
    q.res = reinterpret_cast<const half_t*>(p.res2.p); q.r1_sn = p.res2.sn; q.r1_sp = p.res2.sp;
  }
  const bool has1 = q.res != nullptr;
  const int act = q.slope == 1.f ? 0 : (q.slope == 0.f ? 1 : 2);
  auto go = [&](auto kern) -> int {
    hipError_t err = hipFuncSetAttribute(reinterpret_cast<const void*>(kern), hipFuncAttributeMaxDynamicSharedMemorySize, G::LDS);
    if (err != hipSuccess) { tdvc_set_error("conv_row: hipFuncSetAttribute failed: %s", hipGetErrorString(err)); return (int)err; }
    hipLaunchKernelGGL(kern, dim3(grid), dim3(RW_NTHR), G::LDS, st, q);
    return 0;
  };
  const int nres = has1 ? 1 : 0;
  int rc = TDVC_EINVAL;
#define RW_CASE(A, R, S) if (act == A && nres == R && shuf == S) rc = go(&conv_row_kernel<GID, A, R, S>);
  RW_CASE(0, 0, false) RW_CASE(0, 1, false) RW_CASE(1, 0, false) RW_CASE(1, 1, false) RW_CASE(2, 0, false) RW_CASE(2, 1, false)
  if constexpr (GID == GEO_C128) {
    RW_CASE(0, 0, true) RW_CASE(0, 1, true) RW_CASE(1, 0, true) RW_CASE(1, 1, true) RW_CASE(2, 0, true) RW_CASE(2, 1, true)
  }
#undef RW_CASE
  if (rc) return rc;
  return tdvc_launch_status("tdvc_conv2d(conv_row)");
}

int launch_conv_row(int geo, const ConvParams& p, int N, hipStream_t st) {
  switch (geo) {
    case GEO_C128: return launch_conv_row_t<GEO_C128>(p, N, st);
    case GEO_C64: return launch_conv_row_t<GEO_C64>(p, N, st);
    case GEO_C128W: return launch_conv_row_t<GEO_C128W>(p, N, st);
    default: return launch_conv_row_t<GEO_S2D64>(p, N, st);
  }
}
```

tdvc_amd/csrc/lib.cpp:

```cpp
#include <hip/hip_runtime.h>
#include <stdarg.h>
#include <stdio.h>

#include <mutex>

#include "../../include/tdvc_hip.h"

static thread_local char g_err[512] = "";

void tdvc_set_error(const char* fmt, ...) {
  va_list ap;
  va_start(ap, fmt);
  vsnprintf(g_err, sizeof(g_err), fmt, ap);
  va_end(ap);
}

extern "C" int tdvc_abi_version(void) { return 4; }
extern "C" const char* tdvc_last_error(void) { return g_err; }

namespace {
constexpr int kMaxDev = 64;
constexpr size_t kZeroBytes = 4096, kDumpBytes = 16384;
std::mutex g_scratch_mu;
unsigned char* g_scratch[kMaxDev] = {};
}

int tdvc_scratch_pages(const void** zeros, void** dump) {
  int dev = 0;
  hipError_t err = hipGetDevice(&dev);
  if (err != hipSuccess || dev < 0 || dev >= kMaxDev) {
    tdvc_set_error("scratch pages: hipGetDevice failed or device index %d out of range: %s", dev, hipGetErrorString(err));
    return err != hipSuccess ? (int)err : TDVC_EINVAL;
  }
  std::lock_guard<std::mutex> lk(g_scratch_mu);
  if (!g_scratch[dev]) {
    unsigned char* p = nullptr;
    err = hipMalloc(reinterpret_cast<void**>(&p), kZeroBytes + kDumpBytes);
    if (err == hipSuccess) err = hipMemset(p, 0, kZeroBytes + kDumpBytes);
    if (err == hipSuccess) err = hipDeviceSynchronize();
    if (err != hipSuccess) {
      if (p) (void)hipFree(p);
      tdvc_set_error("scratch pages: allocation on device %d failed: %s", dev, hipGetErrorString(err));
      return (int)err;
    }
    g_scratch[dev] = p;
  }
  if (zeros) *zeros = g_scratch[dev];
  if (dump) *dump = g_scratch[dev] + kZeroBytes;
  return TDVC_OK;
}

extern "C" int tdvc_prepare_device(void) { return tdvc_scratch_pages(nullptr, nullptr); }
```

tdvc_amd/model/coder.py:

```python
from __future__ import annotations

import math

import numpy as np
import torch
import torch.nn as nn
import torch.nn.functional as F

from .. import ops
from ..ops import ACT_LRELU, ACT_NONE, FM, GDN_FWD, GDN_INV
from .modules import PackCache, SELayer, pk_conv


class _LowerBoundGrad(torch.autograd.Function):

    @staticmethod
    def forward(ctx, x, bound):
        ctx.save_for_backward(x, bound)
        return torch.max(x, bound)

    @staticmethod
    def backward(ctx, g):
        x, bound = ctx.saved_tensors
        return ((x >= bound) | (g < 0)).to(g.dtype) * g, None


class LowerBound(nn.Module):
    def __init__(self, bound):
        super().__init__()
        self.register_buffer("bound", torch.Tensor([float(bound)]))

    def forward(self, x):
        return _LowerBoundGrad.apply(x, self.bound)


class NonNegativeParametrizer(nn.Module):
    def __init__(self, minimum=0.0, reparam_offset=2 ** -18):
        super().__init__()
        ped = float(reparam_offset) ** 2
        self.register_buffer("pedestal", torch.Tensor([ped]))
        self.lower_bound = LowerBound((float(minimum) + ped) ** 0.5)

    def init(self, x):
        return torch.sqrt(torch.max(x + self.pedestal, self.pedestal))

    def effective(self, x):
        return self.lower_bound(x) ** 2 - self.pedestal


class GDN(nn.Module, PackCache):
    def __init__(self, ch, inverse=False, beta_min=1e-6, gamma_init=0.1):
        super().__init__()
        self.inverse = bool(inverse)
        self.beta_reparam = NonNegativeParametrizer(minimum=beta_min)
        self.beta = nn.Parameter(self.beta_reparam.init(torch.ones(ch)))
        self.gamma_reparam = NonNegativeParametrizer()
        self.gamma = nn.Parameter(self.gamma_reparam.init(gamma_init * torch.eye(ch)))

    def run(self, x: FM, out: FM | None = None, res: FM | None = None) -> FM:
        def build():
            g = self.gamma_reparam.effective(self.gamma.detach())
            b = self.beta_reparam.effective(self.beta.detach())
            c = g.shape[0]
            pc = ops.pack_conv(g.reshape(c, c, 1, 1).contiguous(), b.contiguous(), stride=1, pad=0, device=self.gamma.device)
            pc.owner = self
            return pc
        pc = self._pk("gdn", build)
        return ops.conv(x, pc, out=out, square=True, gdn=GDN_INV if self.inverse else GDN_FWD, aux=x, res=res)

    def refresh_packed(self):
        pc = self.__dict__.get("_packed", {}).get("gdn")
        if pc is not None:
            with torch.no_grad():
                pc.wsrc.copy_(self.gamma_reparam.effective(self.gamma).reshape(pc.wsrc.shape))
                pc.bsrc.copy_(self.beta_reparam.effective(self.beta))
            pc.repack()

    def accumulate_param_grads(self, dgamma_eff: torch.Tensor, dbeta_eff: torch.Tensor):
        with torch.enable_grad():
            g = self.gamma_reparam.effective(self.gamma)
            b = self.beta_reparam.effective(self.beta)
            torch.autograd.backward([g, b], [dgamma_eff.to(g.dtype), dbeta_eff.to(b.dtype)])


def gdn_refresh_batched(gdns) -> list:
    gdns = [m for m in gdns if m.__dict__.get("_packed", {}).get("gdn") is not None]
    if not gdns:
        return []
    pcs = [m.__dict__["_packed"]["gdn"] for m in gdns]
    with torch.no_grad():
        for attr, rep, dst in (("gamma", "gamma_reparam", "wsrc"), ("beta", "beta_reparam", "bsrc")):
            rp = getattr(gdns[0], rep)
            eff = torch.maximum(torch.stack([getattr(m, attr) for m in gdns]), rp.lower_bound.bound) ** 2 - rp.pedestal
            torch._foreach_copy_([getattr(pc, dst).view(getattr(m, attr).shape) for pc, m in zip(pcs, gdns)], list(eff.unbind(0)))
    return pcs


def gdn_chain_batched(items, grad_of) -> None:
    if not items:
        return
    with torch.no_grad():
        for k, attr, rep in ((1, "gamma", "gamma_reparam"), (2, "beta", "beta_reparam")):
            rp = getattr(items[0][0], rep)
            bound = rp.lower_bound.bound
            P = torch.stack([getattr(it[0], attr) for it in items])
            D = torch.stack([it[k].to(P.dtype).view(getattr(it[0], attr).shape) for it in items])
            d_lb = D * (torch.maximum(P, bound) * 2.0)
            G = d_lb * ((P >= bound) | (d_lb < 0)).to(d_lb.dtype)
            torch._foreach_add_([grad_of(getattr(it[0], attr)) for it in items], list(G.unbind(0)))


def conv3x3(cin, cout, stride=1):
    return nn.Conv2d(cin, cout, 3, stride, 1)


def conv1x1(cin, cout, stride=1):
    return nn.Conv2d(cin, cout, 1, stride)


def subpel_conv3x3(cin, cout, r=1):
    return nn.Sequential(nn.Conv2d(cin, cout * r ** 2, 3, padding=1), nn.PixelShuffle(r))


LR = dict(act=ACT_LRELU, slope=0.01)
STREAM_ORDERS = ("raster", "wavefront")

_RANS_POOL = None


def _rans_pool():
    global _RANS_POOL
    if _RANS_POOL is None:
        from concurrent.futures import ThreadPoolExecutor
        _RANS_POOL = ThreadPoolExecutor(max_workers=2, thread_name_prefix="tdvc-rans")
    return _RANS_POOL


class PendingStrings:

    def __init__(self, y_futs, z_strings):
        self._y, self._z = y_futs, z_strings

    def result(self):
        return [[f.result() for f in self._y], self._z]


class ResidualBlock(nn.Module, PackCache):
    def __init__(self, cin, cout):
        super().__init__()
        self.conv1 = conv3x3(cin, cout)
        self.conv2 = conv3x3(cout, cout)
        self.skip = conv1x1(cin, cout) if cin != cout else None

    def run(self, x: FM, out: FM | None = None) -> FM:
        t = ops.conv(x, pk_conv(self, "c1", self.conv1), **LR)
        idt = x if self.skip is None else ops.conv(x, pk_conv(self, "sk", self.skip))
        return ops.conv(t, pk_conv(self, "c2", self.conv2), out=out, res=idt, **LR)


class ResidualBlockWithStride(nn.Module, PackCache):
    def __init__(self, cin, cout, stride=2):
        super().__init__()
        self.conv1 = conv3x3(cin, cout, stride)
        self.conv2 = conv3x3(cout, cout)
        self.gdn = GDN(cout)
        self.skip = conv1x1(cin, cout, stride) if (stride != 1 or cin != cout) else None

    def run(self, x: FM, out: FM | None = None) -> FM:
        t = ops.conv(x, pk_conv(self, "c1", self.conv1), **LR)
        t = ops.conv(t, pk_conv(self, "c2", self.conv2))
        idt = x if self.skip is None else ops.conv(x, pk_conv(self, "sk", self.skip))
        return self.gdn.run(t, out=out, res=idt)


class ResidualBlockUpsample(nn.Module, PackCache):
    def __init__(self, cin, cout, upsample=2):
        super().__init__()
        assert upsample == 2
        self.subpel_conv = subpel_conv3x3(cin, cout, upsample)
        self.conv = conv3x3(cout, cout)
        self.igdn = GDN(cout, inverse=True)
        self.upsample = subpel_conv3x3(cin, cout, upsample)

    def run(self, x: FM, out: FM | None = None) -> FM:
        t = ops.conv(x, pk_conv(self, "sp", self.subpel_conv[0], shuffle=True), **LR)
        t = ops.conv(t, pk_conv(self, "c", self.conv))
        up = ops.conv(x, pk_conv(self, "up", self.upsample[0], shuffle=True))
        return self.igdn.run(t, out=out, res=up)


class MaskedConv2d(nn.Conv2d):

    def __init__(self, *args, **kwargs):
        super().__init__(*args, **kwargs)
        self.register_buffer("mask", torch.ones_like(self.weight.data))
        _, _, h, w = self.mask.shape
        self.mask[:, :, h // 2, w // 2:] = 0
        self.mask[:, :, h // 2 + 1:] = 0

    def live_taps(self):
        h, w = self.kernel_size
        return [(dy, dx) for dy in range(h) for dx in range(w) if dy < h // 2 or (dy == h // 2 and dx < w // 2)]


class _CdfBuffers:

    _cdf_buffer_names = ("_quantized_cdf", "_offset", "_cdf_length", "scale_table")

    def _load_from_state_dict(self, state_dict, prefix, *args, **kwargs):
        for n in self._cdf_buffer_names:
            src = state_dict.get(prefix + n)
            buf = self._buffers.get(n)
            if src is not None and buf is not None and buf.shape != src.shape:
                self._buffers[n] = torch.empty(src.shape, dtype=buf.dtype, device=buf.device)
        return super()._load_from_state_dict(state_dict, prefix, *args, **kwargs)


class EntropyBottleneck(_CdfBuffers, nn.Module, PackCache):

    def __init__(self, channels, tail_mass=1e-9, init_scale=10, filters=(3, 3, 3, 3), likelihood_bound=1e-9):
        super().__init__()
        self.channels = int(channels)
        self.filters = tuple(int(f) for f in filters)
        self.init_scale = float(init_scale)
        self.tail_mass = float(tail_mass)
        self.likelihood_lower_bound = LowerBound(likelihood_bound)
        self.register_buffer("_offset", torch.IntTensor())
        self.register_buffer("_quantized_cdf", torch.IntTensor())
        self.register_buffer("_cdf_length", torch.IntTensor())
        f = (1,) + self.filters + (1,)
        scale = self.init_scale ** (1 / (len(self.filters) + 1))
        for i in range(len(self.filters) + 1):
            init = np.log(np.expm1(1 / scale / f[i + 1]))
            self.register_parameter(f"_matrix{i:d}", nn.Parameter(torch.full((channels, f[i + 1], f[i]), float(init))))
            self.register_parameter(f"_bias{i:d}", nn.Parameter(torch.zeros(channels, f[i + 1], 1).uniform_(-0.5, 0.5)))
            if i < len(self.filters):
                self.register_parameter(f"_factor{i:d}", nn.Parameter(torch.zeros(channels, f[i + 1], 1)))
        q = torch.Tensor([-self.init_scale, 0, self.init_scale])
        self.quantiles = nn.Parameter(q.repeat(channels, 1, 1))
        target = np.log(2 / self.tail_mass - 1)
        self.register_buffer("target", torch.Tensor([-target, 0, target]))

    def _packed_tensor(self) -> torch.Tensor:
        C_ = self.channels
        parts = [F.softplus(getattr(self, f"_matrix{i}")).reshape(C_, -1) for i in range(5)]
        parts += [getattr(self, f"_bias{i}").reshape(C_, -1) for i in range(5)]
        parts += [torch.tanh(getattr(self, f"_factor{i}")).reshape(C_, -1) for i in range(4)]
        parts += [self.quantiles[:, 0, 1:2]]
        p = torch.cat(parts, 1).float().contiguous()
        assert p.shape == (C_, 59)
        return p

    def packed_params(self) -> torch.Tensor:
        def build():
            with torch.no_grad():
                p = self._packed_tensor()
            p.owner = self
            return p
        return self._pk("eb", build)

    def _raw_params(self):
        return ([getattr(self, f"_matrix{i}") for i in range(5)] + [getattr(self, f"_bias{i}") for i in range(5)] +
                [getattr(self, f"_factor{i}") for i in range(4)])

    def _ptr_table(self, name, tensors):
        ptrs = tuple(t.data_ptr() for t in tensors)
        c = self.__dict__.get(name)
        if c is None or c[0] != ptrs:
            assert all(t.is_cuda and t.dtype == torch.float32 and t.is_contiguous() for t in tensors)
            c = self.__dict__[name] = (ptrs, torch.tensor(ptrs, dtype=torch.int64, device=tensors[0].device))
        return c[1]

    def refresh_packed(self):
        p = self.__dict__.get("_packed", {}).get("eb")
        if p is None:
            return
        if not p.is_cuda:
            self.__dict__["_packed"].pop("eb", None)
            return
        raw = self._raw_params()
        ops.eb_pack(self._ptr_table("_raw_table", [t.data for t in raw]), self.quantiles.data, p, self.channels)

    def accumulate_param_grads(self, dpacked: torch.Tensor, scale: float = 1.0):
        if dpacked.is_cuda:
            from ..autograd import param_grad
            raw = self._raw_params()
            grads = [param_grad(t) for t in raw]
            ops.eb_param_chain(dpacked, self._ptr_table("_raw_table", [t.data for t in raw]), self._ptr_table("_grad_table", grads), scale, self.channels)
            return
        with torch.enable_grad():
            p = self._packed_tensor()
            d = dpacked * scale
            d[:, 58] = 0.0
            torch.autograd.backward([p], [d])

    @torch.no_grad()
    def loss_fused(self, write_grad: bool = True) -> torch.Tensor:
        q = self.quantiles
        if write_grad:
            if q.grad is None or q.grad.shape != q.shape:
                q.grad = torch.empty_like(q)
            dq = q.grad
        else:
            dq = self.__dict__.get("_dq_scratch")
            if dq is None or dq.device != q.device:
                dq = self.__dict__["_dq_scratch"] = torch.empty_like(q)
        out = torch.empty(1, dtype=torch.float32, device=q.device)
        ops.eb_aux(self.packed_params(), q.data, float(np.log(2 / self.tail_mass - 1)), dq, out, self.channels)
        return out

    def logits_cumulative(self, x, stop_gradient):
        for i in range(len(self.filters) + 1):
            m, b = getattr(self, f"_matrix{i:d}"), getattr(self, f"_bias{i:d}")
            if stop_gradient:
                m, b = m.detach(), b.detach()
            x = torch.matmul(F.softplus(m), x) + b
            if i < len(self.filters):
                fac = getattr(self, f"_factor{i:d}")
                if stop_gradient:
                    fac = fac.detach()
                x = x + torch.tanh(fac) * torch.tanh(x)
        return x

    def loss(self):
        logits = self.logits_cumulative(self.quantiles, stop_gradient=True)
        return torch.abs(logits - self.target).sum()


class GaussianConditional(_CdfBuffers, nn.Module):
    def __init__(self, scale_bound=0.11, tail_mass=1e-9, likelihood_bound=1e-9):
        super().__init__()
        self.tail_mass = float(tail_mass)
        self.likelihood_lower_bound = LowerBound(likelihood_bound)
        self.register_buffer("_offset", torch.IntTensor())
        self.register_buffer("_quantized_cdf", torch.IntTensor())
        self.register_buffer("_cdf_length", torch.IntTensor())
        self.register_buffer("scale_table", torch.Tensor())
        self.lower_bound_scale = LowerBound(scale_bound)


class Cheng2020Anchor(nn.Module, PackCache):
    def __init__(self, N=192):
        super().__init__()
        self.N = self.M = M = N
        self.entropy_bottleneck = EntropyBottleneck(N)
        self.h_a = nn.Sequential(
            conv3x3(N, N), nn.LeakyReLU(inplace=True), conv3x3(N, N), nn.LeakyReLU(inplace=True),
            conv3x3(N, N, stride=2), nn.LeakyReLU(inplace=True), conv3x3(N, N), nn.LeakyReLU(inplace=True),
            conv3x3(N, N, stride=2))
        self.h_s = nn.Sequential(
            conv3x3(N, N), nn.LeakyReLU(inplace=True), subpel_conv3x3(N, N, 2), nn.LeakyReLU(inplace=True),
            conv3x3(N, N * 3 // 2), nn.LeakyReLU(inplace=True), subpel_conv3x3(N * 3 // 2, N * 3 // 2, 2),
            nn.LeakyReLU(inplace=True), conv3x3(N * 3 // 2, N * 2))
        self.entropy_parameters = nn.Sequential(
            nn.Conv2d(M * 12 // 3, M * 10 // 3, 1), nn.LeakyReLU(inplace=True),
            nn.Conv2d(M * 10 // 3, M * 8 // 3, 1), nn.LeakyReLU(inplace=True),
            nn.Conv2d(M * 8 // 3, M * 6 // 3, 1))
        self.context_prediction = MaskedConv2d(M, 2 * M, kernel_size=5, padding=2, stride=1)
        self.gaussian_conditional = GaussianConditional()

    def run_g_a(self, x: FM):
        g = self.g_a
        t = g[0].run(x)
        t = g[1].run(t)
        t = g[2].run(t)
        t = g[3].run(t)
        t = g[4].run(t)
        t = g[5].run(t)
        t = g[6].run(t)
        f32 = x.f32
        t = ops.conv(t, pk_conv(self, "ga7", g[7]), out_dtype=torch.float32)
        y32 = FM.empty(t.N, t.H, t.W, t.C, dtype=torch.float32, device=t.t.device)
        if f32:
            g[8].run(t, out=y32)
            return y32, y32
        y16 = FM.empty(t.N, t.H, t.W, t.C, device=t.t.device)
        g[8].run(t, out=y32, out2=y16)
        return y32, y16

    def run_g_s(self, y_hat: FM, out: FM | None = None, res: FM | None = None) -> FM:
        g = self.g_s
        t = g[0].run(y_hat)
        for i in range(1, 5):
            t = g[i].run(t)
        t = g[5].run(t)
        for i in range(6, 9):
            t = g[i].run(t)
        return ops.conv(t, pk_conv(self, "gs9", g[9][0], shuffle=True), out=out, res=res, out_dtype=torch.float16)

    def run_h_a(self, y16: FM) -> FM:
        h = self.h_a
        t = ops.conv(y16, pk_conv(self, "ha0", h[0]), **LR)
        t = ops.conv(t, pk_conv(self, "ha2", h[2]), **LR)
        t = ops.conv(t, pk_conv(self, "ha4", h[4]), **LR)
        t = ops.conv(t, pk_conv(self, "ha6", h[6]), **LR)
        return ops.conv(t, pk_conv(self, "ha8", h[8]), out_dtype=torch.float32)

    def run_h_s(self, z_hat: FM, out: FM) -> FM:
        h = self.h_s
        t = ops.conv(z_hat, pk_conv(self, "hs0", h[0]), **LR)
        t = ops.conv(t, pk_conv(self, "hs2", h[2][0], shuffle=True), **LR)
        t = ops.conv(t, pk_conv(self, "hs4", h[4]), **LR)
        t = ops.conv(t, pk_conv(self, "hs6", h[6][0], shuffle=True), **LR)
        return ops.conv(t, pk_conv(self, "hs8", h[8]), out=out)

    def run_entropy_parameters(self, pc_in: FM) -> FM:
        e = self.entropy_parameters
        t = ops.conv(pc_in, pk_conv(self, "ep0", e[0]), **LR)
        t = ops.conv(t, pk_conv(self, "ep2", e[2]), **LR)
        return ops.conv(t, pk_conv(self, "ep4", e[4]), out_dtype=torch.float32)

    def ctx_conv(self) -> ops.PackedConv:
        cp = self.context_prediction

        def build():
            pc = ops.pack_conv(cp.weight, cp.bias, stride=1, pad=2, taps=cp.live_taps(), device=cp.weight.device)
            pc.orig["wgrad_taps"] = [(dy, dx) for dy in range(5) for dx in range(5)]
            return pc
        return self._pk("ctx", build)

    def _as_f32(self, x: FM) -> FM:
        return x if x.f32 else ops.copy_cast(x, FM.empty(x.N, x.H, x.W, x.C, dtype=torch.float32, device=x.t.device))

    def run(self, x: FM, training: bool, out: FM | None = None, res: FM | None = None, trace=None, noise=None, f32=False):
        dev = x.t.device
        if f32:
            if training:
                raise RuntimeError("the fp32-island mode has no backward: train with the default (fp16-in / fp32-accumulate) coders")
            x = self._as_f32(x)
        adt = torch.float32 if f32 else torch.float16
        y32, y16 = self.run_g_a(x)
        z = self.run_h_a(y16)
        B, h, w, M = y32.N, y32.H, y32.W, self.M
        bits = torch.zeros(2, dtype=torch.float64, device=dev)
        z_hat = FM.empty(z.N, z.H, z.W, z.C, dtype=adt, device=dev)
        nz = ny = nl = None
        if training:
            noise = noise or {}
            nz = noise.get("z") or FM(torch.rand((z.N, z.H, z.W, z.C), device=dev) - 0.5)
            ny = noise.get("y") or FM(torch.rand((B, h, w, M), device=dev) - 0.5)
            nl = noise.get("y_lik") or FM(torch.rand((B, h, w, M), device=dev) - 0.5)
        ops.eb_forward(z, self.entropy_bottleneck.packed_params(), z_hat, bits[1:2], noise=nz)
        pcat = FM.empty(B, h, w, 4 * M, dtype=adt, device=dev)
        self.run_h_s(z_hat, out=pcat.ch(0, 2 * M))
        y_hat = ops.quantize(y32, FM.empty(B, h, w, M, dtype=adt, device=dev), noise=ny)
        ops.conv(y_hat, self.ctx_conv(), out=pcat.ch(2 * M, 2 * M))
        gp = self.run_entropy_parameters(pcat)
        ops.gc_forward(y32, gp, bits[0:1], noise=nl)
        x_hat = self.run_g_s(y_hat, out=out, res=res)
        if trace is not None:
            trace.update(y=y32, z=z, z_hat=z_hat, y_hat=y_hat, gp=gp)
        return x_hat, bits

    def aux_loss(self):
        eb = self.entropy_bottleneck
        if ops.TAPE is not None and getattr(ops.TAPE, "fused_aux", False) and eb.quantiles.is_cuda:
            return eb.loss_fused(write_grad=False).reshape(())
        return eb.loss()

    @torch.no_grad()
    def update(self, force=False):
        import scipy.stats
        dev = self.context_prediction.weight.device
        eb, gc = self.entropy_bottleneck, self.gaussian_conditional
        changed = False
        if gc._offset.numel() == 0 or force:
            table = torch.exp(torch.linspace(math.log(0.11), math.log(256), 64))
            mult = -scipy.stats.norm.ppf(gc.tail_mass / 2)
            center = torch.ceil(table * mult).int()
            length = 2 * center + 1
            maxlen = int(length.max())
            samples = torch.abs(torch.arange(maxlen).int() - center[:, None]).float()
            sc = table.unsqueeze(1).float()
            cdfn = lambda v: 0.5 * torch.erfc(-(2 ** -0.5) * v)
            upper, lower = cdfn((0.5 - samples) / sc), cdfn((-0.5 - samples) / sc)
            pmf, tail = upper - lower, 2 * lower[:, :1]
            cdf = torch.zeros((64, maxlen + 2), dtype=torch.int32)
            for i in range(64):
                prob = torch.cat((pmf[i, : int(length[i])], tail[i])).numpy()
                c = ops.pmf_to_quantized_cdf(prob)
                cdf[i, : c.size] = torch.from_numpy(c)
            gc._quantized_cdf, gc._offset, gc._cdf_length = cdf.to(dev), (-center).to(dev), (length + 2).to(dev)
            gc.scale_table = table.to(dev)
            changed = True
        if eb._offset.numel() == 0 or force:
            q = eb.quantiles.detach().float().cpu()
            med = q[:, 0, 1]
            minima = torch.clamp(torch.ceil(med - q[:, 0, 0]).int(), min=0)
            maxima = torch.clamp(torch.ceil(q[:, 0, 2] - med).int(), min=0)
            start, length = med - minima, maxima + minima + 1
            maxlen = int(length.max())
            samples = torch.arange(maxlen)[None, :] + start[:, None, None]
            ebc = EntropyBottleneck(eb.channels)
            ebc.load_state_dict({k: v.cpu() for k, v in eb.state_dict().items()}, strict=False)
            lower = ebc.logits_cumulative(samples - 0.5, True)
            upper = ebc.logits_cumulative(samples + 0.5, True)
            sign = -torch.sign(lower + upper)
            pmf = torch.abs(torch.sigmoid(sign * upper) - torch.sigmoid(sign * lower))[:, 0, :]
            tail = torch.sigmoid(lower[:, 0, :1]) + torch.sigmoid(-upper[:, 0, -1:])
            cdf = torch.zeros((eb.channels, maxlen + 2), dtype=torch.int32)
            for i in range(eb.channels):
                prob = torch.cat((pmf[i, : int(length[i])], tail[i])).numpy()
                c = ops.pmf_to_quantized_cdf(prob)
                cdf[i, : c.size] = torch.from_numpy(c)
            eb._quantized_cdf, eb._offset, eb._cdf_length = cdf.to(dev), (-minima).to(dev), (length + 2).to(dev)
            changed = True
        self.__dict__.pop("_tables", None)
        return changed

    def _coder_tables(self):
        t = self.__dict__.get("_tables")
        if t is None:
            eb, gc = self.entropy_bottleneck, self.gaussian_conditional
            if eb._offset.numel() == 0 or gc._offset.numel() == 0:
                raise RuntimeError("entropy coder tables are empty: call update(force=True) first (pnet.py:47)")
            t = (ops.CdfTables(eb._quantized_cdf, eb._cdf_length, eb._offset),
                 ops.CdfTables(gc._quantized_cdf, gc._cdf_length, gc._offset), gc.scale_table.float().contiguous())
            self.__dict__["_tables"] = t
        return t

    def _ctx_1x1(self) -> ops.PackedConv:
        cp = self.context_prediction

        def build():
            co, ci, kh, kw = cp.weight.shape
            chan = np.array([c * kh * kw + dy * kw + dx for dy, dx in cp.live_taps() for c in range(ci)], dtype=np.int64)
            lay = ops.convpack.WeightLayout(co, len(chan), 1, 1, np.arange(co, dtype=np.int64) * ci * kh * kw, chan, np.zeros(1, dtype=np.int64))
            return ops.pack_conv(cp.weight, cp.bias, stride=1, pad=0, device=cp.weight.device, layout=lay, param_w=cp.weight, param_b=cp.bias)
        return self._pk("ctx1x1", build)

    @staticmethod
    def wavefront_steps(H, W):
        steps = []
        for t in range(W + 3 * (H - 1)):
            ps = [(h, t - 3 * h) for h in range(H) if 0 <= t - 3 * h < W]
            if ps:
                steps.append(ps)
        return steps

    def _ar_setup(self, H, W, adt, dev, B):
        cache = self.__dict__.setdefault("_ar_cache", {})
        key = (H, W, adt, str(dev), B)
        c = cache.get(key)
        if c is not None and not all(a is b for a, b in zip(c["chain"]["pcs"], self._ar_packed())):
            c = None
        if c is None:
            steps = self.wavefront_steps(H, W)
            flat = torch.tensor([p for st in steps for p in st], dtype=torch.int32, device=dev)
            c = dict(flat=flat, fl=flat.long(), sizes=np.array([len(st) for st in steps], dtype=np.int32), chain=self._ar_chain(H, adt, dev),
                     host=[(torch.empty((H * W, self.M), dtype=torch.int32).pin_memory(), torch.empty((H * W, self.M), dtype=torch.int32).pin_memory())
                           for _ in range(B)])
            cache.clear()
            cache[key] = c
        return c

    @torch.no_grad()
    def compress(self, x: FM, f32=False, order="raster", defer=False):
        if order not in STREAM_ORDERS:
            raise ValueError(f"order must be one of {STREAM_ORDERS}, got {order!r}")
        dev = x.t.device
        ebt, gct, table = self._coder_tables()
        M = self.M
        if f32:
            x = self._as_f32(x)
        adt = torch.float32 if f32 else torch.float16
        y32, y16 = self.run_g_a(x)
        z = self.run_h_a(y16)
        B, H, W = y32.N, y32.H, y32.W
        med = self.entropy_bottleneck.quantiles.detach()[:, 0, 1].float().contiguous()
        zsym = ops.round_symbols(z, med)
        z_hat = FM((zsym.float() + med).to(adt))
        params = FM.empty(B, H, W, 2 * M, dtype=adt, device=dev)
        self.run_h_s(z_hat, out=params)
        zs = zsym.permute(0, 3, 1, 2).contiguous().cpu().numpy()
        zidx = np.broadcast_to(np.arange(M, dtype=np.int32)[:, None, None], zs.shape[1:])
        z_strings = [ops.rans_encode(zs[b], zidx, ebt) for b in range(B)]
        st = self._ar_setup(H, W, adt, dev, B)
        flat, sizes, chain, fl = st["flat"], st["sizes"], st["chain"], st["fl"]
        y_jobs, dbg = [], []
        for b in range(B):
            y_hat = FM.empty(1, H, W, M, dtype=adt, device=dev)
            sym = torch.empty((H, W, M), dtype=torch.int32, device=dev)
            idx = torch.empty((H, W, M), dtype=torch.int32, device=dev)
            ops.ar_wavefront(None, None, y32.batch(b, 1), y_hat, params.batch(b, 1), chain["x1"], chain["pc"], chain["descs"], chain["gp"],
                             flat, sizes, M, W, table, idx, sym)
            hs, hi = st["host"][b]
            if order == "wavefront":
                hs.copy_(sym[fl[:, 0], fl[:, 1]], non_blocking=True)
                hi.copy_(idx[fl[:, 0], fl[:, 1]], non_blocking=True)
            else:
                hs.copy_(sym.view(H * W, M), non_blocking=True)
                hi.copy_(idx.view(H * W, M), non_blocking=True)
            ev = torch.cuda.Event()
            ev.record()

            def job(ev=ev, hs=hs, hi=hi):
                ev.synchronize()
                return ops.rans_encode(hs.numpy(), hi.numpy(), gct)
            y_jobs.append(_rans_pool().submit(job) if defer else job())
            dbg.append({"y_hat": y_hat, "symbols": sym, "indexes": idx})
        if defer:
            return {"strings": PendingStrings(y_jobs, z_strings), "shape": (z.H, z.W), "_debug": dbg}
        return {"strings": [y_jobs, z_strings], "shape": (z.H, z.W), "_debug": dbg}

    @torch.no_grad()
    def decompress(self, strings, shape, synth=True, f32=False, order="raster"):
        if order not in STREAM_ORDERS:
            raise ValueError(f"order must be one of {STREAM_ORDERS}, got {order!r}")
        dev = self.context_prediction.weight.device
        adt = torch.float32 if f32 else torch.float16
        ebt, gct, table = self._coder_tables()
        M = self.M
        zh, zw = shape
        B = len(strings[1])
        H, W = zh * 4, zw * 4
        med = self.entropy_bottleneck.quantiles.detach()[:, 0, 1].float().contiguous()
        zidx = np.broadcast_to(np.arange(M, dtype=np.int32)[:, None, None], (M, zh, zw))
        zs = np.stack([ops.RansDecoder(s).decode(zidx, ebt).reshape(M, zh, zw) for s in strings[1]])
        zsym = torch.from_numpy(zs).to(dev).permute(0, 2, 3, 1).contiguous()
        z_hat = FM((zsym.float() + med).to(adt))
        params = FM.empty(B, H, W, 2 * M, dtype=adt, device=dev)
        self.run_h_s(z_hat, out=params)
        y_hat_all = FM.zeros(B, H, W, M, dtype=adt, device=dev)
        sym = torch.zeros((H, W, M), dtype=torch.int32, device=dev)
        idx = torch.zeros((H, W, M), dtype=torch.int32, device=dev)
        if order == "wavefront":
            for b in range(B):
                self._decode_wavefront(strings[0][b], gct, table, y_hat_all.batch(b, 1), params.batch(b, 1))
            return {"x_hat": self.run_g_s(y_hat_all) if synth else None, "y_hat": y_hat_all}
        chain = self._ar_chain(1, adt, dev)
        pos_table = torch.tensor([[h, w] for h in range(H) for w in range(W)], dtype=torch.int32, device=dev)
        for b in range(B):
            ops.ar_decode_serial(strings[0][b], gct, y_hat_all.batch(b, 1), params.batch(b, 1), chain["x1"], chain["pc"], chain["descs"],
                                 chain["gp"], pos_table, M, W, table, idx, sym)
        return {"x_hat": self.run_g_s(y_hat_all) if synth else None, "y_hat": y_hat_all}

    def _ar_chain(self, cap, adt, dev):
        M, e = self.M, self.entropy_parameters
        x1 = FM.empty(1, 1, cap, 12 * M, dtype=adt, device=dev)
        pc = FM.empty(1, 1, cap, 4 * M, dtype=adt, device=dev)
        t0 = FM.empty(1, 1, cap, ops.pad8(e[0].out_channels), dtype=adt, device=dev)
        t1 = FM.empty(1, 1, cap, ops.pad8(e[2].out_channels), dtype=adt, device=dev)
        gp = FM.empty(1, 1, cap, 2 * M, dtype=torch.float32, device=dev)
        v = lambda fm, c0, C_: FM(fm.t, c0, 1, C_)
        pcs = self._ar_packed()
        descs = [ops.conv_desc(v(x1, 0, x1.C), pcs[0], out=v(pc, 2 * M, 2 * M))[0],
                 ops.conv_desc(v(pc, 0, 4 * M), pcs[1], out=t0, **LR)[0],
                 ops.conv_desc(t0, pcs[2], out=t1, **LR)[0],
                 ops.conv_desc(t1, pcs[3], out=gp, out_dtype=torch.float32)[0]]
        return {"x1": x1, "pc": pc, "gp": gp, "descs": descs, "keep": (t0, t1), "pcs": pcs}

    def _ar_packed(self):
        e = self.entropy_parameters
        return [self._ctx_1x1(), pk_conv(self, "ep0", e[0]), pk_conv(self, "ep2", e[2]), pk_conv(self, "ep4", e[4])]

    def _decode_wavefront(self, data, gct, table, y_hat, params):
        dev, M = y_hat.t.device, self.M
        H, W = y_hat.H, y_hat.W
        steps = self.wavefront_steps(H, W)
        flat = torch.tensor([p for st in steps for p in st], dtype=torch.int32, device=dev)
        chain = self._ar_chain(H, y_hat.t.dtype, dev)
        sym = torch.zeros((H * W, M), dtype=torch.int32, device=dev)
        idx = torch.zeros((H * W, M), dtype=torch.int32, device=dev)
        ops.ar_wavefront(data, gct, None, y_hat, params, chain["x1"], chain["pc"], chain["descs"], chain["gp"], flat,
                         np.array([len(st) for st in steps], dtype=np.int32), M, W, table, idx, sym)

def _g_a(N):
    return nn.Sequential(
        ResidualBlockWithStride(64, N, stride=2), ResidualBlock(N, N),
        ResidualBlockWithStride(N, N, stride=2), SELayer(N), ResidualBlock(N, N),
        ResidualBlockWithStride(N, N, stride=2), ResidualBlock(N, N),
        conv3x3(N, N, stride=2), SELayer(N))


def _g_s(N):
    return nn.Sequential(
        SELayer(N), ResidualBlock(N, N), ResidualBlockUpsample(N, N, 2), ResidualBlock(N, N),
        ResidualBlockUpsample(N, N, 2), SELayer(N), ResidualBlock(N, N),
        ResidualBlockUpsample(N, N, 2), ResidualBlock(N, N), subpel_conv3x3(N, 64, 2))


class ResCoder(Cheng2020Anchor):

    def __init__(self, N=192):
        super().__init__(N=N)
        self.g_a, self.g_s = _g_a(N), _g_s(N)


class MVCoder(Cheng2020Anchor):

    def __init__(self, N=192):
        super().__init__(N=N)
        self.g_a, self.g_s = _g_a(N), _g_s(N)
```

tdvc_amd/ops.py:

```python
from __future__ import annotations

import ctypes as C
from dataclasses import dataclass

import numpy as np
import torch

from . import _lib as L
from . import convpack
from ._lib import (ACT_CLAMP01, ACT_LRELU, ACT_NONE, ACT_RELU, GDN_FWD, GDN_INV, GDN_NONE, OUT_NCHW_F32,
                   OUT_NHWC, OUT_SHUFFLE2)


_raw_stream = torch._C._cuda_getCurrentRawStream
_cur_dev = torch._C._cuda_getDevice
FORCE_STREAM = None
FORCE_KEEP = None


def _stream():
    if FORCE_STREAM is not None:
        return C.c_void_p(FORCE_STREAM)
    return C.c_void_p(_raw_stream(_cur_dev()))


PROFILE = None
TAPE = None
_IN_BACKWARD = False


def _rec(name, *args):
    if TAPE is not None and not _IN_BACKWARD:
        from . import autograd
        getattr(autograd, "record_" + name)(TAPE, *args)


def pad8(c: int) -> int:
    return (c + 7) // 8 * 8


class FM:

    __slots__ = ("t", "off", "N", "C", "H", "W", "sn", "sp", "_d")

    def __init__(self, t: torch.Tensor, off: int = 0, N: int | None = None, C_: int | None = None, sn: int | None = None):
        assert t.dim() == 4 and (t.shape[3] == 1 or t.stride(3) == 1)
        self.t, self.off = t, off
        self._d = None
        self.N = t.shape[0] if N is None else N
        self.C = t.shape[3] if C_ is None else C_
        self.H, self.W = t.shape[1], t.shape[2]
        if self.W > 1:
            self.sp = t.stride(2)
        elif self.H > 1:
            self.sp = t.stride(1)
        else:
            self.sp = t.shape[3]
        assert self.H == 1 or t.stride(1) == self.W * self.sp, "rows of a feature map must be dense (row stride = W * pixel stride)"
        self.sn = (t.stride(0) if t.shape[0] > 1 else self.H * self.W * self.sp) if sn is None else sn

    @staticmethod
    def empty(N, H, W, C_, dtype=torch.float16, device="cuda"):
        return FM(torch.empty((N, H, W, C_), dtype=dtype, device=device))

    @staticmethod
    def zeros(N, H, W, C_, dtype=torch.float16, device="cuda"):
        return FM(torch.zeros((N, H, W, C_), dtype=dtype, device=device))

    @property
    def f32(self):
        return self.t.dtype == torch.float32

    def ch(self, c0, C_):
        assert 0 <= c0 and c0 + C_ <= self.C
        return FM(self.t, self.off + c0, self.N, C_, self.sn)

    def batch(self, n0, N):
        assert 0 <= n0 and n0 + N <= self.N
        return FM(self.t, self.off + n0 * self.sn, N, self.C, self.sn)

    def as_slices(self, b, T, Cs):
        assert self.C == T * Cs and 0 <= b < self.N
        return FM(self.t, self.off + b * self.sn, T, Cs, Cs)

    def desc(self) -> L.FMapDesc:
        d = self._d
        if d is None:
            p = self.t.data_ptr() + self.off * self.t.element_size()
            d = self._d = L.FMapDesc(p, self.N, self.H, self.W, self.C, self.sn, self.sp, L.F32 if self.f32 else L.F16)
        return d

    def to_nchw(self, C_=None) -> torch.Tensor:
        C_ = self.C if C_ is None else C_
        out = torch.empty((self.N, C_, self.H, self.W), dtype=torch.float32, device=self.t.device)
        d = self.desc()
        L.check(L.lib().tdvc_fmap_to_nchw(C.byref(d), C_, out.data_ptr(), _stream()), "fmap_to_nchw")
        return out


_NULL_FM = L.FMapDesc(None, 0, 0, 0, 0, 0, 0, 0)


def from_nchw(x: torch.Tensor, Cpad: int | None = None, dtype=torch.float16, out: FM | None = None) -> FM:
    assert x.is_cuda and x.dtype == torch.float32
    x = x.contiguous()
    N, Cc, H, W = x.shape
    if out is None:
        out = FM.empty(N, H, W, pad8(Cc) if Cpad is None else Cpad, dtype=dtype, device=x.device)
    d = out.desc()
    L.check(L.lib().tdvc_nchw_to_fmap(x.data_ptr(), Cc, C.byref(d), _stream()), "nchw_to_fmap")
    return out


@dataclass
class PackedConv:
    w: torch.Tensor
    bias: torch.Tensor
    cout: int
    cin: int
    kh: int
    kw: int
    stride: int
    pad: int
    ck: int
    taps: list
    shuffle: bool = False
    cin_real: int = 0
    s2d: bool = False
    flops_per_px: float = 0.0
    wsrc: torch.Tensor | None = None
    bsrc: torch.Tensor | None = None
    layout: convpack.WeightLayout | None = None
    tables: convpack.PackTables | None = None
    orig: dict | None = None
    dgrad: "PackedConv | None" = None
    param_w: torch.Tensor | None = None
    param_b: torch.Tensor | None = None
    owner: object | None = None
    w32: torch.Tensor | None = None

    def packed_f32(self) -> torch.Tensor:
        if self.w32 is None:
            self.w32 = _pack_from_tables_f32(self.wsrc, self.tables)
        return self.w32

    def repack(self):
        _pack_from_tables(self.wsrc, self.tables, self.w)
        self.w32 = None
        if self.bsrc is not None:
            b = self.bsrc.detach().float()
            self.bias[:self.cout] = b[torch.from_numpy(convpack.shuffle_perm(self.cout)).to(b.device)] if self.shuffle else b
        if self.dgrad is not None:
            self.dgrad.repack()
        for key in ("_colpc", "_plain"):
            aux = self.__dict__.get(key)
            if aux is not None:
                aux.repack()


def _cout_pad(cout):
    return 32 if cout <= 32 else 64 * ((cout + 63) // 64)


def _s2d_weights(w: torch.Tensor) -> torch.Tensor:
    cout, C_, kh, kw = w.shape
    assert (kh, kw) == (3, 3)
    w2 = torch.zeros(cout, 4 * C_, 2, 2)
    for py in range(2):
        for px in range(2):
            q = py * 2 + px
            for dy in range(2):
                for dx in range(2):
                    ky, kx = 2 * dy + py - 1, 2 * dx + px - 1
                    if 0 <= ky <= 2 and 0 <= kx <= 2:
                        w2[:, q * C_:(q + 1) * C_, dy, dx] = w[:, :, ky, kx]
    return w2


def _pack_from_tables(wsrc: torch.Tensor, tb: convpack.PackTables, dst: torch.Tensor | None = None) -> torch.Tensor:
    lib = L.lib()
    nbytes = lib.tdvc_conv_packed_bytes(tb.cout, tb.cin, len(tb.taps), tb.ck)
    assert nbytes > 0
    w = wsrc.detach()
    assert w.is_cuda and w.dtype == torch.float32 and w.is_contiguous()
    if dst is None:
        dst = torch.empty(nbytes, dtype=torch.uint8, device=w.device)
    assert dst.numel() == nbytes
    L.check(lib.tdvc_pack_conv_weights_indexed(w.data_ptr(), tb.row_off.data_ptr(), tb.chan_off.data_ptr(), tb.tap_off.data_ptr(),
                                               tb.row_mask.data_ptr(), tb.chan_mask.data_ptr(), tb.tap_mask.data_ptr(),
                                               tb.cout, tb.cin, len(tb.taps), tb.ck, dst.data_ptr(), _stream()), "pack_conv_weights_indexed")
    return dst


def _pack_from_tables_f32(wsrc: torch.Tensor, tb: convpack.PackTables) -> torch.Tensor:
    lib = L.lib()
    nbytes = lib.tdvc_conv_packed_bytes(tb.cout, tb.cin, len(tb.taps), tb.ck)
    assert nbytes > 0
    w = wsrc.detach()
    assert w.is_cuda and w.dtype == torch.float32 and w.is_contiguous()
    dst = torch.empty(nbytes // 2, dtype=torch.float32, device=w.device)
    L.check(lib.tdvc_pack_conv_weights_indexed_f32(w.data_ptr(), tb.row_off.data_ptr(), tb.chan_off.data_ptr(), tb.tap_off.data_ptr(),
                                                   tb.row_mask.data_ptr(), tb.chan_mask.data_ptr(), tb.tap_mask.data_ptr(),
                                                   tb.cout, tb.cin, len(tb.taps), tb.ck, dst.data_ptr(), _stream()), "pack_conv_weights_indexed_f32")
    return dst


class _PackJob(C.Structure):
    _fields_ = [("w", C.c_void_p), ("row_off", C.c_void_p), ("chan_off", C.c_void_p), ("tap_off", C.c_void_p),
                ("row_mask", C.c_void_p), ("chan_mask", C.c_void_p), ("tap_mask", C.c_void_p), ("dst", C.c_void_p),
                ("bias_src", C.c_void_p), ("bias_dst", C.c_void_p), ("bias_perm", C.c_void_p),
                ("cout", C.c_int32), ("cin", C.c_int32), ("ntaps", C.c_int32), ("ck", C.c_int32)]


class PackBatch:

    def __init__(self, pcs):
        self.pcs = []
        seen = set()

        def walk(pc):
            if pc is None or id(pc) in seen:
                return
            seen.add(id(pc))
            self.pcs.append(pc)
            walk(pc.dgrad)
            walk(pc.__dict__.get("_colpc"))
            walk(pc.__dict__.get("_plain"))
        for pc in pcs:
            walk(pc)
        self._build()

    def _tensors(self, pc):
        tb = pc.tables
        return [pc.wsrc, tb.row_off, tb.chan_off, tb.tap_off, tb.row_mask, tb.chan_mask, tb.tap_mask, pc.w] + \
               ([pc.bsrc, pc.bias] if pc.bsrc is not None else [])

    def _build(self):
        lib = L.lib()
        jobs = (_PackJob * len(self.pcs))()
        starts = [0]
        self._keep = []
        self._ptrs = []
        dev = self.pcs[0].w.device
        for j, pc in zip(jobs, self.pcs):
            tb = pc.tables
            w = pc.wsrc.detach()
            assert w.is_cuda and w.dtype == torch.float32 and w.is_contiguous()
            j.w, j.row_off, j.chan_off, j.tap_off = w.data_ptr(), tb.row_off.data_ptr(), tb.chan_off.data_ptr(), tb.tap_off.data_ptr()
            j.row_mask, j.chan_mask, j.tap_mask = tb.row_mask.data_ptr(), tb.chan_mask.data_ptr(), tb.tap_mask.data_ptr()
            j.dst = pc.w.data_ptr()
            j.cout, j.cin, j.ntaps, j.ck = tb.cout, tb.cin, len(tb.taps), tb.ck
            if pc.bsrc is not None:
                b = pc.bsrc.detach()
                assert b.is_cuda and b.dtype == torch.float32 and b.is_contiguous() and pc.bias.dtype == torch.float32
                j.bias_src, j.bias_dst = b.data_ptr(), pc.bias.data_ptr()
                if pc.shuffle:
                    perm = torch.from_numpy(convpack.shuffle_perm(pc.cout).astype(np.int32)).to(dev)
                    self._keep.append(perm)
                    j.bias_perm = perm.data_ptr()
            nb = lib.tdvc_pack_job_blocks(tb.cout, tb.cin, len(tb.taps), tb.ck)
            assert nb > 0
            starts.append(starts[-1] + nb)
            self._ptrs.append([t.data_ptr() for t in self._tensors(pc)])
        self.total_blocks = starts[-1]
        self.jobs = torch.frombuffer(bytearray(bytes(jobs)), dtype=torch.uint8).to(dev)
        self.starts = torch.tensor(starts, dtype=torch.int32, device=dev)

    def run(self):
        self._runs = getattr(self, "_runs", 0) + 1
        full = (self._runs & 63) == 1
        for pc, ptrs in zip(self.pcs, self._ptrs):
            if (([t.data_ptr() for t in self._tensors(pc)] != ptrs) if full else (pc.wsrc.data_ptr() != ptrs[0] or pc.w.data_ptr() != ptrs[7])):
                self._build()
                break
        L.check(L.lib().tdvc_pack_conv_weights_batch(self.jobs.data_ptr(), self.starts.data_ptr(), len(self.pcs), self.total_blocks, _stream()),
                "pack_conv_weights_batch")
        for pc in self.pcs:
            pc.w32 = None


def _pick_ck(cin, cout, kh, kw, stride, pad):
    if (stride == 1 or (stride == 2 and kh == 1 and kw == 1 and pad == 0)) and cin >= 32 and cout >= 64:
        return 32
    ck = L.lib().tdvc_conv_plan(cin, kh, kw, stride)
    L.check(0 if ck > 0 else ck, "conv_plan")
    return ck


def pack_conv(weight: torch.Tensor, bias: torch.Tensor | None, stride=1, pad=0, cin_pad: int | None = None,
              taps=None, shuffle=False, cin_perm=None, device="cuda", ck=None, allow_s2d=True,
              layout: convpack.WeightLayout | None = None, param_w: torch.Tensor | None = None,
              param_b: torch.Tensor | None = None) -> PackedConv:
    wsrc = weight if (weight.is_cuda and weight.dtype == torch.float32 and weight.is_contiguous()) else \
        weight.detach().float().contiguous().to(device)
    dev = wsrc.device
    if layout is None:
        cout, cin_real, kh, kw = weight.shape
        layout = convpack.WeightLayout.dense(cout, cin_real, kh, kw)
    cout, kh, kw = layout.cout, layout.kh, layout.kw
    cin_real = layout.cin if cin_perm is None else len(cin_perm)
    bsrc = None if bias is None else (bias if bias.is_cuda else bias.detach().float().to(dev))
    orig = dict(stride=stride, pad=pad, taps=taps, cin_perm=cin_perm, kh=kh, kw=kw)
    s2d = (allow_s2d and stride == 2 and (kh, kw) == (3, 3) and pad == 1 and cin_real % 32 == 0 and cout >= 64
           and taps is None and not shuffle and ck is None and cin_perm is None and cin_pad is None)
    if shuffle:
        assert cout % 4 == 0
    if s2d:
        tb = convpack.forward_tables_s2d(layout, ck=32, device=dev)
        cin, k_stride, k_pad = cin_real, 1, 1
    else:
        cin = pad8(cin_real) if cin_pad is None else cin_pad
        if taps is None:
            taps = [(dy, dx) for dy in range(kh) for dx in range(kw)]
        if ck is None:
            ck = _pick_ck(cin, cout, kh, kw, stride, pad)
        tb = convpack.forward_tables(layout, cin_pad=cin, taps=taps, pad=pad, ck=ck, shuffle=shuffle, cin_perm=cin_perm, device=dev)
        k_stride, k_pad = stride, pad
    orig["taps"] = [(dy, dx) for dy in range(kh) for dx in range(kw)] if orig["taps"] is None else list(orig["taps"])
    bp = torch.zeros(_cout_pad(cout), dtype=torch.float32, device=dev)
    pc = PackedConv(_pack_from_tables(wsrc, tb), bp, cout, cin, tb.kh, tb.kw, k_stride, k_pad, tb.ck, tb.taps, shuffle, cin_real,
                    s2d=s2d, flops_per_px=2.0 * cout * cin_real * 9 if s2d else 0.0,
                    wsrc=wsrc, bsrc=bsrc, layout=layout, tables=tb, orig=orig,
                    param_w=param_w if param_w is not None else (weight if isinstance(weight, torch.nn.Parameter) else None),
                    param_b=param_b if param_b is not None else (bias if isinstance(bias, torch.nn.Parameter) else None))
    if bsrc is not None:
        b = bsrc.detach().float()
        bp[:cout] = b[torch.from_numpy(convpack.shuffle_perm(cout)).to(dev)] if shuffle else b
    return pc


SMALL_MAP_PIXELS = 8192


def _plain_form(pc: PackedConv) -> PackedConv:
    alt = pc.__dict__.get("_plain")
    if alt is None:
        alt = pack_conv(pc.wsrc, pc.bsrc, stride=2, pad=1, allow_s2d=False, layout=pc.layout, param_w=pc.param_w, param_b=pc.param_b)
        pc.__dict__["_plain"] = alt
    return alt


def conv_desc(x: FM, pc: PackedConv, out: FM | None = None, act=ACT_NONE, slope=0.0, res: FM | None = None,
              res2: FM | None = None, gdn=GDN_NONE, aux: FM | None = None, square=False, out_dtype=None,
              round16=False, nchw_out: torch.Tensor | None = None, bcast_T=0, bcast_slope=0.0):
    assert x.C == pc.cin, f"conv: input has {x.C} channels, layer packed for {pc.cin}"
    rec_pc = pc
    if out_dtype is None:
        out_dtype = torch.float32 if x.f32 else torch.float16
    if pc.s2d and (x.f32 or x.N * (x.H // 2) * (x.W // 2) <= SMALL_MAP_PIXELS):
        pc = _plain_form(pc)
    if pc.s2d:
        if x.H % 2 or x.W % 2:
            raise L.TdvcHipError("conv: the space-to-depth stride-2 path needs even H, W")
        Ho, Wo = x.H // 2, x.W // 2
    else:
        Ho = (x.H + 2 * pc.pad - pc.kh) // pc.stride + 1
        Wo = (x.W + 2 * pc.pad - pc.kw) // pc.stride + 1
    wt = pc.packed_f32() if x.f32 else pc.w
    key = "_tmpl32" if x.f32 else "_tmpl16"
    tm = pc.__dict__.get(key)
    if tm is None or tm[1] != wt.data_ptr():
        t_ = L.ConvDesc()
        t_.w = wt.data_ptr()
        t_.bias = pc.bias.data_ptr()
        t_.cout, t_.ntaps = pc.cout, len(pc.taps)
        for i, (dy, dx) in enumerate(pc.taps):
            t_.tap_dy[i], t_.tap_dx[i] = dy, dx
        t_.kh, t_.kw, t_.stride, t_.pad, t_.ck = pc.kh, pc.kw, pc.stride, pc.pad, pc.ck
        t_.s2d = int(pc.s2d)
        tm = pc.__dict__[key] = (t_, wt.data_ptr())
    d = L.ConvDesc.from_buffer_copy(tm[0])
    d.x = x.desc()
    d.square_input, d.gdn = int(square), gdn
    d.aux = aux.desc() if aux is not None else _NULL_FM
    d.act, d.slope, d.round_before_act = act, slope, int(round16)
    d.res = res.desc() if res is not None else _NULL_FM
    d.res2 = res2.desc() if res2 is not None else _NULL_FM
    d.bcast_T, d.bcast_slope = int(bcast_T), float(bcast_slope)
    if nchw_out is not None:
        assert nchw_out.shape == (x.N, pc.cout, Ho, Wo) and nchw_out.dtype == torch.float32 and nchw_out.is_contiguous()
        d.out_mode = OUT_NCHW_F32
        d.y = L.FMapDesc(nchw_out.data_ptr(), x.N, Ho, Wo, pc.cout, pc.cout * Ho * Wo, 1, L.F32)
        ret = nchw_out
    else:
        if pc.shuffle:
            d.out_mode = OUT_SHUFFLE2
            if out is None:
                out = FM.empty(x.N, 2 * Ho, 2 * Wo, pad8(pc.cout // 4), dtype=out_dtype, device=x.t.device)
        else:
            d.out_mode = OUT_NHWC
            if out is None:
                out = FM.empty(x.N, Ho, Wo, pc.cout if (out_dtype == torch.float32 and not x.f32) else pad8(pc.cout),
                               dtype=out_dtype, device=x.t.device)
        d.y = out.desc()
        ret = out
    return d, ret, Ho, Wo, pc, rec_pc


def conv(x: FM, pc: PackedConv, out: FM | None = None, act=ACT_NONE, slope=0.0, res: FM | None = None,
         res2: FM | None = None, gdn=GDN_NONE, aux: FM | None = None, square=False, out_dtype=None,
         round16=False, nchw_out: torch.Tensor | None = None, bcast_T=0, bcast_slope=0.0, chan_sum: list | None = None) -> FM | torch.Tensor:
    d, ret, Ho, Wo, pc, rec_pc = conv_desc(x, pc, out, act, slope, res, res2, gdn, aux, square, out_dtype, round16, nchw_out, bcast_T, bcast_slope)
    if chan_sum is not None and TAPE is None and FUSE_CHAN_SUM:
        rows = L.lib().tdvc_conv_chan_sum_rows(C.byref(d))
        if rows > 0:
            part = torch.empty((x.N, rows, pc.cout), dtype=torch.float32, device=x.t.device)
            d.chan_sum = part.data_ptr()
            chan_sum.append((part, rows))
    if x.f32 and TAPE is not None and not _IN_BACKWARD:
        raise L.TdvcHipError("conv: the fp32 form has no backward (the fp32 islands are an inference / coding mode)")
    if bcast_T and TAPE is not None and not _IN_BACKWARD:
        raise L.TdvcHipError("conv: bcast_T is an inference-only fusion (under the tape use conv + bcast_add_act)")
    if PROFILE is not None:
        e0, e1 = torch.cuda.Event(enable_timing=True), torch.cuda.Event(enable_timing=True)
        e0.record()
        L.check(L.lib().tdvc_conv2d(C.byref(d), _stream()), "conv2d")
        e1.record()
        PROFILE.append(dict(kernel=L.lib().tdvc_last_conv_kernel().decode(),
                            shape=f"{pc.kh}x{pc.kw} s{pc.stride} {x.C}->{pc.cout} @{x.H}x{x.W}" + (" f32out" if out_dtype == torch.float32 else "") + (" nchw" if nchw_out is not None else ""),
                            e0=e0, e1=e1,
                            flops=2.0 * x.N * Ho * Wo * pc.cout * x.C * len(pc.taps),
                            flops_real=(x.N * Ho * Wo * pc.flops_per_px) if pc.s2d else 2.0 * x.N * Ho * Wo * pc.cout * pc.cin_real * len(pc.taps),
                            bytes=2.0 * x.N * (x.H * x.W * x.C + Ho * Wo * pc.cout * (4 if pc.shuffle else 1) / (4 if pc.shuffle else 1))))
        _rec("conv", x, rec_pc, None if nchw_out is not None else ret, act, slope, res, res2, gdn, aux, square, nchw_out)
        return ret
    L.check(L.lib().tdvc_conv2d(C.byref(d), _stream()), "conv2d")
    _rec("conv", x, rec_pc, None if nchw_out is not None else ret, act, slope, res, res2, gdn, aux, square, nchw_out)
    return ret


class PackedConvPair:

    def __init__(self, w: torch.Tensor, bias: torch.Tensor):
        self.w, self.bias = w, bias


def pack_conv_pair(w1: torch.Tensor, b1: torch.Tensor | None, w2: torch.Tensor, b2: torch.Tensor | None) -> PackedConvPair:
    for w in (w1, w2):
        if tuple(w.shape) != (64, 64, 3, 3):
            raise L.TdvcHipError(f"pack_conv_pair: weights must be (64, 64, 3, 3), got {tuple(w.shape)}")
    frag = lambda w: w.detach().float().reshape(4, 16, 2, 4, 8, 9).permute(0, 5, 2, 3, 1, 4)
    w = torch.stack([frag(w1), frag(w2)]).contiguous().to(torch.float16)
    zb = lambda b_: torch.zeros(64, device=w1.device) if b_ is None else b_.detach().float()
    return PackedConvPair(w, torch.cat([zb(b1), zb(b2)]).contiguous())


def _pair_desc(x: FM, pp: PackedConvPair, out: FM, act1, slope1, act2, slope2, add_input, res2):
    d = L.ConvPairDesc()
    d.x, d.y = x.desc(), out.desc()
    d.w, d.bias = pp.w.data_ptr(), pp.bias.data_ptr()
    d.act1, d.slope1, d.act2, d.slope2 = act1, slope1, act2, slope2
    d.add_input = 1 if add_input else 0
    d.res2 = res2.desc() if res2 is not None else L.FMapDesc()
    return d


def conv_pair_supported(x: FM, out: FM | None = None, res2: FM | None = None) -> bool:
    if TAPE is not None or x.f32 or x.C != 64:
        return False
    d = L.ConvPairDesc()
    d.x = x.desc()
    d.y = out.desc() if out is not None else x.desc()
    d.res2 = res2.desc() if res2 is not None else L.FMapDesc()
    d.w = d.bias = 1
    return bool(L.lib().tdvc_conv_pair_supported(C.byref(d)))


def conv_pair(x: FM, pp: PackedConvPair, out: FM | None = None, act1=ACT_RELU, slope1=0.0, act2=ACT_NONE, slope2=0.0,
              add_input=True, res2: FM | None = None) -> FM:
    if TAPE is not None:
        raise L.TdvcHipError("conv_pair: inference only (the intermediate map is not kept for the backward pass)")
    if out is None:
        out = FM.empty(x.N, x.H, x.W, 64, device=x.t.device)
    d = _pair_desc(x, pp, out, act1, slope1, act2, slope2, add_input, res2)
    if PROFILE is not None:
        e0, e1 = torch.cuda.Event(enable_timing=True), torch.cuda.Event(enable_timing=True)
        e0.record()
        L.check(L.lib().tdvc_conv_pair(C.byref(d), _stream()), "conv_pair")
        e1.record()
        fl = 2 * 2.0 * x.N * x.H * x.W * 64 * 64 * 9
        PROFILE.append(dict(kernel="conv_pair", shape=f"2x(3x3 s1 64->64) @{x.H}x{x.W}", e0=e0, e1=e1, flops=fl, flops_real=fl,
                            bytes=2.0 * x.N * x.H * x.W * 128))
        return out
    L.check(L.lib().tdvc_conv_pair(C.byref(d), _stream()), "conv_pair")
    return out


def act_backward(g: FM, y: FM, act, slope=0.0, res: FM | None = None, out: FM | None = None) -> FM:
    out = g if out is None else out
    dg, dy, do = g.desc(), y.desc(), out.desc()
    dr = res.desc() if res is not None else None
    L.check(L.lib().tdvc_act_backward(C.byref(dg), C.byref(dy), C.byref(dr) if dr is not None else None, act, slope, C.byref(do), _stream()),
            "act_backward")
    return out


def pixel_unshuffle(y: FM, out: FM | None = None) -> FM:
    if out is None:
        out = FM.empty(y.N, y.H // 2, y.W // 2, 4 * y.C, dtype=y.t.dtype, device=y.t.device)
    dy, do = y.desc(), out.desc()
    L.check(L.lib().tdvc_pixel_unshuffle(C.byref(dy), C.byref(do), _stream()), "pixel_unshuffle")
    return out


def _dgrad_conv(pc: PackedConv, g_channels: int, x_channels: int) -> PackedConv:
    if pc.dgrad is None:
        o = pc.orig
        tb0 = dict(g_channels=g_channels, x_channels=x_channels, taps=o["taps"], pad=o["pad"], stride=o["stride"], shuffle=pc.shuffle,
                   cin_perm=o["cin_perm"], device=pc.w.device)
        rows = x_channels * (4 if o["stride"] == 2 else 1)
        kk = 3 if (o["stride"] == 2 and o["kh"] == 3) else o["kh"]
        ck = _pick_ck(g_channels, rows, kk, kk, 1, 1)
        tb = convpack.dgrad_tables(pc.layout, ck=ck, **tb0)
        bias = torch.zeros(_cout_pad(tb.cout), dtype=torch.float32, device=pc.w.device)
        pc.dgrad = PackedConv(_pack_from_tables(pc.wsrc, tb), bias, tb.cout, tb.cin, tb.kh, tb.kw, 1, tb.pad, tb.ck, tb.taps, tb.shuffle,
                              tb.cin, wsrc=pc.wsrc, tables=tb)
    assert pc.dgrad.cin == g_channels
    return pc.dgrad


def conv_dgrad(pc: PackedConv, g: FM, dx: FM, accumulate=True, extra: FM | None = None) -> FM:
    dpc = _dgrad_conv(pc, g.C, dx.C)
    if accumulate:
        return conv(g, dpc, out=dx, res=dx, res2=extra)
    return conv(g, dpc, out=dx, res=extra)


class WgradBatch:

    def __init__(self):
        self.items = []

    def add(self, job, keep):
        self.items.append((job, keep))

    def flush(self):
        if not self.items:
            return
        rounds, nxt = [], {}
        for job, _ in self.items:
            r = nxt.get(job.dw, 0)
            nxt[job.dw] = r + 1
            if len(rounds) <= r:
                rounds.append([])
            rounds[r].append(job)
        lib = L.lib()
        for jobs in rounds:
            n = len(jobs)
            arr = (L.WgradReduceJob * n)(*jobs)
            starts = (C.c_int32 * (n + 1))()
            for i, j in enumerate(jobs):
                starts[i + 1] = starts[i] + j.nblocks
            nb_j, nb_s = C.sizeof(arr), C.sizeof(starts)
            host = torch.empty((nb_j + nb_s,), dtype=torch.uint8, pin_memory=True)
            C.memmove(host.data_ptr(), arr, nb_j)
            C.memmove(host.data_ptr() + nb_j, starts, nb_s)
            dev = host.to(jobs_device(jobs), non_blocking=True)
            if torch.cuda.is_current_stream_capturing():
                _GRAPH_KEEP.append((host, dev))
            L.check(lib.tdvc_wgrad_reduce_batch(dev.data_ptr(), dev.data_ptr() + nb_j, n, int(starts[n]), _stream()), "wgrad_reduce_batch")
        self.items.clear()


_GRAPH_KEEP: list = []


def jobs_device(jobs):
    return torch.device("cuda", torch.cuda.current_device())


def conv_wgrad(pc: PackedConv, g: FM, x: FM, dw: torch.Tensor, scale=1.0, square_x=False, db: torch.Tensor | None = None,
               defer: WgradBatch | None = None) -> None:
    o = pc.orig
    taps = o.get("wgrad_taps") or o["taps"]
    tb = pc.__dict__.get("_wg_tables")
    if tb is None:
        tb = convpack.forward_tables(pc.layout, cin_pad=x.C, taps=taps, pad=o["pad"], ck=8, shuffle=pc.shuffle, cin_perm=o["cin_perm"],
                                     device=pc.w.device)
        pc.__dict__["_wg_tables"] = tb
    assert dw.is_cuda and dw.dtype == torch.float32 and dw.is_contiguous() and dw.numel() == pc.wsrc.numel()
    lib = L.lib()
    Ho, Wo = g.H, g.W
    wk = pc.__dict__.get("_wg_static")
    if wk is None or wk[0] != (x.C, x.N, Ho, Wo):
        wk = pc.__dict__["_wg_static"] = ((x.C, x.N, Ho, Wo), lib.tdvc_conv_wgrad_work_floats(pc.cout, x.C, len(taps), x.N, Ho, Wo),
                                          (C.c_int8 * len(taps))(*[t[0] for t in taps]), (C.c_int8 * len(taps))(*[t[1] for t in taps]))
    _, nwork, dy, dxs = wk
    work = torch.empty((nwork,), dtype=torch.float32, device=dw.device)
    if FORCE_KEEP is not None:
        FORCE_KEEP.append(work)
    dg, dxd = g.desc(), x.desc()
    if PROFILE is not None:
        e0, e1 = torch.cuda.Event(enable_timing=True), torch.cuda.Event(enable_timing=True)
        e0.record()
    bidx = None
    if db is not None:
        assert db.is_cuda and db.dtype == torch.float32 and db.is_contiguous() and db.numel() >= pc.cout
        bidx = _bias_index(pc, db.device)
    if defer is not None and PROFILE is None:
        job = L.WgradReduceJob()
        L.check(lib.tdvc_conv_wgrad_partials(C.byref(dg), C.byref(dxd), pc.cout, o["kh"], o["kw"], o["stride"], o["pad"], len(taps), dy, dxs,
                                             tb.row_off.data_ptr(), tb.chan_off.data_ptr(), tb.tap_off.data_ptr(), int(square_x), scale, dw.data_ptr(),
                                             bidx.data_ptr() if bidx is not None else None, db.data_ptr() if db is not None else None,
                                             work.data_ptr(), nwork, C.byref(job), _stream()), "conv_wgrad_partials")
        defer.add(job, (work, dw, db, tb, bidx))
        return
    L.check(lib.tdvc_conv_wgrad_bias(C.byref(dg), C.byref(dxd), pc.cout, o["kh"], o["kw"], o["stride"], o["pad"], len(taps), dy, dxs,
                                tb.row_off.data_ptr(), tb.chan_off.data_ptr(), tb.tap_off.data_ptr(), int(square_x), scale, dw.data_ptr(),
                                bidx.data_ptr() if bidx is not None else None, db.data_ptr() if db is not None else None,
                                work.data_ptr(), nwork, _stream()), "conv_wgrad")
    if PROFILE is not None:
        e1.record()
        PROFILE.append(dict(kernel="conv_wgrad", shape=f"{o['kh']}x{o['kw']} s{o['stride']} {x.C}->{pc.cout} @{x.N}x{x.H}x{x.W}", e0=e0, e1=e1,
                            flops=2.0 * x.N * Ho * Wo * pc.cout * x.C * len(taps), flops_real=2.0 * x.N * Ho * Wo * pc.cout * pc.cin_real * len(taps),
                            bytes=0.0,
                            geo=(o["kh"], o["kw"], o["stride"], pc.cin_real, pc.cout, bool(pc.shuffle), bool(square_x), "wgrad_taps" in o)))


def _bias_index(pc: PackedConv, device):
    idx = pc.__dict__.get("_bg_index")
    if idx is None and pc.shuffle:
        idx = torch.from_numpy(convpack.shuffle_perm(pc.cout)).to(torch.int32).to(device)
        pc.__dict__["_bg_index"] = idx
    return idx


def conv_bgrad(pc: PackedConv, g: FM, db: torch.Tensor, scale=1.0) -> None:
    lib = L.lib()
    idx = _bias_index(pc, db.device)
    nwork = lib.tdvc_bias_grad_work_floats(g.N, g.C)
    work = torch.empty((nwork,), dtype=torch.float32, device=db.device)
    dg = g.desc()
    L.check(lib.tdvc_bias_grad(C.byref(dg), pc.cout, idx.data_ptr() if idx is not None else None, scale, db.data_ptr(), work.data_ptr(), nwork,
                               _stream()), "bias_grad")


def gdn_backward(g: FM, x: FM, n32: FM, inverse: bool, dx: FM) -> FM:
    dn = FM.empty(g.N, g.H, g.W, g.C, device=g.t.device)
    d1, d2, d3, d4, d5 = g.desc(), x.desc(), n32.desc(), dn.desc(), dx.desc()
    L.check(L.lib().tdvc_gdn_backward(C.byref(d1), C.byref(d2), C.byref(d3), int(inverse), C.byref(d4), C.byref(d5), _stream()), "gdn_backward")
    return dn


def mul2_accumulate(dx: FM, x: FM, t: FM) -> None:
    d1, d2, d3 = dx.desc(), x.desc(), t.desc()
    L.check(L.lib().tdvc_mul2_accumulate(C.byref(d1), C.byref(d2), C.byref(d3), _stream()), "mul2_accumulate")


def copy_cast(src: FM, dst: FM) -> FM:
    ds, dd = src.desc(), dst.desc()
    L.check(L.lib().tdvc_copy_cast(C.byref(ds), C.byref(dd), _stream()), "copy_cast")
    return dst


def clamp01_backward(g: FM, y: FM) -> FM:
    dg, dy = g.desc(), y.desc()
    L.check(L.lib().tdvc_clamp01_backward(C.byref(dg), C.byref(dy), _stream()), "clamp01_backward")
    return g


def gate_backward(g: FM, a: FM, gate: torch.Tensor, da: FM | None, dgate: torch.Tensor) -> None:
    lib = L.lib()
    nwork = lib.tdvc_gate_backward_work_floats(g.N, g.C)
    work = torch.empty((nwork,), dtype=torch.float32, device=gate.device)
    dg, dad = g.desc(), a.desc()
    dda = da.desc() if da is not None else None
    L.check(lib.tdvc_gate_backward(C.byref(dg), C.byref(dad), gate.data_ptr(), C.byref(dda) if dda is not None else None, dgate.data_ptr(),
                                   work.data_ptr(), nwork, _stream()), "gate_backward")


def se_gate_backward(p: "SEParams", partial: torch.Tensor, nblocks: int, npix: int, gate: torch.Tensor, dgate: torch.Tensor, scale: float,
                     grads) -> torch.Tensor:
    N = gate.shape[0]
    dmean = torch.empty_like(gate)
    L.check(L.lib().tdvc_se_gate_backward(partial.data_ptr(), nblocks, 1.0 / npix, N, p.C, p.Cmid, p.w1.data_ptr(), p.b1.data_ptr(),
                                          p.w2.data_ptr(), p.b2.data_ptr(), gate.data_ptr(), dgate.data_ptr(), scale, dmean.data_ptr(),
                                          grads[0].data_ptr(), grads[1].data_ptr(), grads[2].data_ptr(), grads[3].data_ptr(), _stream()),
            "se_gate_backward")
    return dmean


def bcast_channel_add(dx: FM, v: torch.Tensor, scale: float) -> None:
    d = dx.desc()
    L.check(L.lib().tdvc_bcast_channel_add(C.byref(d), v.data_ptr(), scale, _stream()), "bcast_channel_add")


def add_flow_backward(doff: FM, dflow: FM) -> None:
    do, df = doff.desc(), dflow.desc()
    L.check(L.lib().tdvc_add_flow_backward(C.byref(do), C.byref(df), _stream()), "add_flow_backward")


def bcast_add_act_backward(dx: FM, x: FM, db: FM, slope: float) -> None:
    d1, d2, d3 = dx.desc(), x.desc(), db.desc()
    L.check(L.lib().tdvc_bcast_add_act_backward(C.byref(d1), C.byref(d2), C.byref(d3), slope, _stream()), "bcast_add_act_backward")


def upsample2x_backward(dy: FM, dx: FM) -> None:
    d1, d2 = dy.desc(), dx.desc()
    L.check(L.lib().tdvc_upsample2x_backward(C.byref(d1), C.byref(d2), _stream()), "upsample2x_backward")


DCN_PLANAR_MIN_PIXELS = 1 << 16
DCN_PLANAR = __import__("os").environ.get("TDVC_DCN_PLANAR", "0") == "1"


def dcn_fused(x: FM, om: FM, pc: PackedConv, out: FM, groups=8, act=ACT_NONE, slope=0.0, round16=True, planar: bool | None = None) -> FM:
    d = L.DcnDesc()
    d.x, d.om, d.y = x.desc(), om.desc(), out.desc()
    d.w, d.bias = pc.w.data_ptr(), pc.bias.data_ptr()
    d.groups, d.act, d.slope, d.round_before_act = groups, act, slope, int(round16)
    if planar is None:
        planar = DCN_PLANAR and x.H * x.W >= DCN_PLANAR_MIN_PIXELS
    scratch = torch.empty((x.N, groups, x.H, x.W, 8), dtype=torch.float16, device=x.t.device) if planar else None
    d.x_planar = scratch.data_ptr() if scratch is not None else None
    L.check(L.lib().tdvc_dcn_fused(C.byref(d), _stream()), "dcn_fused")
    _rec("dcn_fused", x, om, pc, out, groups, act, slope)
    return out


def dcn_columns(x: FM, om: FM, groups: int) -> FM:
    col = FM.empty(x.N, x.H, x.W, 72 * groups, device=x.t.device)
    d1, d2, d3 = x.desc(), om.desc(), col.desc()
    L.check(L.lib().tdvc_dcn_columns(C.byref(d1), C.byref(d2), groups, C.byref(d3), _stream()), "dcn_columns")
    return col


DETERMINISTIC = False


def dcn_col2im(x: FM, om: FM, dcol: FM, groups: int, dom: FM) -> FM:
    dx32 = FM.zeros(x.N, x.H, x.W, x.C, dtype=torch.float32, device=x.t.device)
    lib = L.lib()
    nwork = lib.tdvc_dcn_col2im_work_floats(x.N, x.H, x.W, groups)
    work = torch.empty((nwork,), dtype=torch.float32, device=x.t.device)
    d1, d2, d3, d4 = x.desc(), om.desc(), dcol.desc(), dom.desc()
    if DETERMINISTIC:
        dev = x.t.device
        cap = max(1 << 16, x.N * x.H * x.W * groups * 36 // 8)
        keys = torch.empty((cap,), dtype=torch.int64, device=dev)
        vals = torch.empty((cap, 8), dtype=torch.float32, device=dev)
        cnt = torch.zeros((1,), dtype=torch.int32, device=dev)
        L.check(lib.tdvc_dcn_col2im_det(C.byref(d1), C.byref(d2), C.byref(d3), groups, dx32.t.data_ptr(), C.byref(d4), work.data_ptr(), nwork,
                                        keys.data_ptr(), vals.data_ptr(), cnt.data_ptr(), cap, _stream()), "dcn_col2im_det")
        n = int(cnt.item())
        if n > cap:
            raise L.TdvcHipError(f"dcn_col2im (deterministic): {n} far samples exceed the record capacity {cap}")
        if n:
            ks, order = torch.sort(keys[:n], stable=True)
            L.check(lib.tdvc_dcn_far_apply(ks.data_ptr(), order.data_ptr(), vals.data_ptr(), n, dx32.t.data_ptr(), _stream()), "dcn_far_apply")
        return dx32
    L.check(lib.tdvc_dcn_col2im(C.byref(d1), C.byref(d2), C.byref(d3), groups, dx32.t.data_ptr(), C.byref(d4), work.data_ptr(), nwork, _stream()),
            "dcn_col2im")
    return dx32


def dcn_column_conv(pc: PackedConv, groups: int) -> PackedConv:
    cp = pc.__dict__.get("_colpc")
    if cp is None:
        cin = 8 * groups
        chan = np.array([(g * 8 + j) * 9 + t for g in range(groups) for t in range(9) for j in range(8)], dtype=np.int64)
        lay = convpack.WeightLayout(pc.cout, 9 * cin, 1, 1, np.arange(pc.cout, dtype=np.int64) * cin * 9, chan, np.zeros(1, dtype=np.int64))
        cp = pack_conv(pc.wsrc, None, stride=1, pad=0, layout=lay, param_w=pc.param_w)
        pc.__dict__["_colpc"] = cp
    return cp


def sigmoid_f32(x: torch.Tensor) -> torch.Tensor:
    out = torch.empty_like(x)
    L.check(L.lib().tdvc_sigmoid_f32(x.data_ptr(), out.data_ptr(), x.numel(), _stream()), "sigmoid_f32")
    return out


def sigmoid_backward_f32(g: torch.Tensor, s: torch.Tensor) -> torch.Tensor:
    L.check(L.lib().tdvc_sigmoid_backward_f32(g.data_ptr(), s.data_ptr(), g.numel(), _stream()), "sigmoid_backward_f32")
    return g


def axpy_f32(dst: torch.Tensor, src: torch.Tensor, scale: float) -> None:
    assert dst.numel() == src.numel() and dst.dtype == src.dtype == torch.float32 and dst.is_contiguous() and src.is_contiguous()
    L.check(L.lib().tdvc_axpy_f32(dst.data_ptr(), src.data_ptr(), scale, dst.numel(), _stream()), "axpy_f32")


def scale_act_res(a: FM, out: FM, gate: torch.Tensor | None = None, act=ACT_NONE, slope=0.0, res: FM | None = None,
                  res_sign=1.0, out2: FM | None = None) -> FM:
    da, dy = a.desc(), out.desc()
    dr = res.desc() if res is not None else None
    d2 = out2.desc() if out2 is not None else None
    L.check(L.lib().tdvc_scale_act_res(C.byref(da), gate.data_ptr() if gate is not None else None, act, slope,
                                       C.byref(dr) if dr is not None else None, res_sign, C.byref(dy),
                                       C.byref(d2) if d2 is not None else None, _stream()), "scale_act_res")
    _rec("scale_act_res", a, out, gate, act, slope, res, res_sign, out2)
    return out


def clone(x: FM) -> FM:
    out = copy_cast(x, FM.empty(x.N, x.H, x.W, x.C, dtype=x.t.dtype, device=x.t.device))
    _rec("clone", x, out)
    return out


def add_flow(off: FM, flow: FM):
    do, df = off.desc(), flow.desc()
    L.check(L.lib().tdvc_add_flow(C.byref(do), C.byref(df), _stream()), "add_flow")
    _rec("add_flow", off, flow)


def bcast_add_act(x: FM, b: FM, T: int, slope: float):
    dx, db = x.desc(), b.desc()
    L.check(L.lib().tdvc_bcast_add_act(C.byref(dx), C.byref(db), T, slope, _stream()), "bcast_add_act")
    _rec("bcast_add_act", x, b, slope)


@dataclass
class SEParams:
    w1: torch.Tensor
    b1: torch.Tensor
    w2: torch.Tensor
    b2: torch.Tensor
    C: int
    Cmid: int
    params: tuple = ()


FUSE_CHAN_SUM = True


def se_gate(x: FM, p: SEParams, partial=None) -> torch.Tensor:
    npix = x.H * x.W
    gate = torch.empty((x.N, x.C), dtype=torch.float32, device=x.t.device)
    lib = L.lib()
    if partial is not None:
        partial, nblocks = partial
        assert tuple(partial.shape) == (x.N, nblocks, x.C) and partial.dtype == torch.float32
    else:
        nblocks = max(1, min(1024, npix // 256))
        partial = torch.empty((x.N, nblocks, x.C), dtype=torch.float32, device=x.t.device)
        dx = x.desc()
        L.check(lib.tdvc_channel_sum(C.byref(dx), partial.data_ptr(), nblocks, _stream()), "channel_sum")
    L.check(lib.tdvc_se_gate(partial.data_ptr(), nblocks, 1.0 / npix, x.N, p.C, p.Cmid, p.w1.data_ptr(),
                             p.b1.data_ptr(), p.w2.data_ptr(), p.b2.data_ptr(), gate.data_ptr(), _stream()), "se_gate")
    _rec("se_gate", x, p, partial, nblocks, gate)
    return gate


def upsample2x(x: FM, out: FM | None = None) -> FM:
    if out is None:
        out = FM.empty(x.N, 2 * x.H, 2 * x.W, x.C, device=x.t.device)
    dx, dy = x.desc(), out.desc()
    L.check(L.lib().tdvc_upsample2x(C.byref(dx), C.byref(dy), _stream()), "upsample2x")
    _rec("upsample2x", x, out)
    return out


def avgpool2(x: FM) -> FM:
    out = FM.empty(x.N, x.H // 2, x.W // 2, x.C, dtype=torch.float32, device=x.t.device)
    dx, dy = x.desc(), out.desc()
    L.check(L.lib().tdvc_avgpool2(C.byref(dx), C.byref(dy), _stream()), "avgpool2")
    return out


def spynet_level_input(ref: FM, supp: FM, flow_lo: FM | None, flow_up: FM, cat8: FM):
    dr, ds, du, dc = ref.desc(), supp.desc(), flow_up.desc(), cat8.desc()
    dl = flow_lo.desc() if flow_lo is not None else None
    L.check(L.lib().tdvc_spynet_level_input(C.byref(dr), C.byref(ds), C.byref(dl) if dl is not None else None,
                                            C.byref(du), C.byref(dc), _stream()), "spynet_level_input")
    _rec("spynet_level_input", supp, flow_lo, flow_up, cat8)


def spynet_level_input_backward(supp: FM, flow_up: FM, dcat8: FM, dflow_up: FM, dflow_lo: FM | None) -> None:
    d1, d2, d3, d4 = supp.desc(), flow_up.desc(), dcat8.desc(), dflow_up.desc()
    d5 = dflow_lo.desc() if dflow_lo is not None else None
    L.check(L.lib().tdvc_spynet_level_input_backward(C.byref(d1), C.byref(d2), C.byref(d3), C.byref(d4),
                                                     C.byref(d5) if d5 is not None else None, _stream()), "spynet_level_input_backward")


def resize_bilinear(x: FM, H: int, W: int, chscale: torch.Tensor | None = None) -> FM:
    out = FM.empty(x.N, H, W, x.C, dtype=torch.float32, device=x.t.device)
    dx, dy = x.desc(), out.desc()
    L.check(L.lib().tdvc_resize_bilinear(C.byref(dx), C.byref(dy), chscale.data_ptr() if chscale is not None else None,
                                         _stream()), "resize_bilinear")
    _rec("resize_bilinear", x, out, chscale)
    return out


def resize_bilinear_backward(dy: FM, dx: FM, chscale: torch.Tensor | None = None) -> None:
    d1, d2 = dy.desc(), dx.desc()
    L.check(L.lib().tdvc_resize_bilinear_backward(C.byref(d1), C.byref(d2), chscale.data_ptr() if chscale is not None else None, _stream()),
            "resize_bilinear_backward")


def avgpool_k(x: FM, scale: int) -> torch.Tensor:
    hp, wp = x.H // scale, x.W // scale
    pooled = torch.empty((x.N, hp, wp, x.C), dtype=torch.float32, device=x.t.device)
    nwork = L.lib().tdvc_avgpool_k_work_floats(x.N, hp, wp, x.C, scale)
    work = torch.empty((nwork,), dtype=torch.float32, device=x.t.device)
    dx = x.desc()
    L.check(L.lib().tdvc_avgpool_k(C.byref(dx), scale, pooled.data_ptr(), hp, wp, work.data_ptr(), nwork, _stream()), "avgpool_k")
    return pooled


def patch_match(pin: torch.Tensor, pref: torch.Tensor) -> torch.Tensor:
    N, hp, wp, Cc = pin.shape
    Lp = ((hp + 3) // 3 + 1) * ((wp + 3) // 3 + 1)
    idx = torch.empty((N, Lp), dtype=torch.int32, device=pin.device)
    L.check(L.lib().tdvc_patch_match(pin.data_ptr(), pref.data_ptr(), N, hp, wp, Cc, idx.data_ptr(), _stream()),
            "patch_match")
    return idx


def match_gather(fin: FM, fref: FM, idx: torch.Tensor, scale: int, cat: FM):
    df, dr, dc = fin.desc(), fref.desc(), cat.desc()
    L.check(L.lib().tdvc_match_gather(C.byref(df), C.byref(dr), idx.data_ptr(), scale, fin.H // scale, fin.W // scale,
                                      C.byref(dc), _stream()), "match_gather")
    _rec("match_gather", fin, fref, idx, scale, cat)


def match_gather_backward(fin: FM, fref: FM, idx: torch.Tensor, scale: int, dcat: FM, dfin: FM, dfref: FM) -> None:
    d1, d2, d3, d4, d5 = fin.desc(), fref.desc(), dcat.desc(), dfin.desc(), dfref.desc()
    L.check(L.lib().tdvc_match_gather_backward(C.byref(d1), C.byref(d2), idx.data_ptr(), scale, fin.H // scale, fin.W // scale,
                                               C.byref(d3), C.byref(d4), C.byref(d5), _stream()), "match_gather_backward")


def eb_forward(z: FM, params: torch.Tensor, z_hat: FM, bits_out: torch.Tensor, noise: FM | None = None):
    numel = z.N * z.H * z.W * z.C
    cap = (numel + 255) // 256
    partial = torch.empty(cap, dtype=torch.float32, device=z.t.device)
    dz, dh = z.desc(), z_hat.desc()
    dn = noise.desc() if noise is not None else None
    L.check(L.lib().tdvc_eb_forward(C.byref(dz), params.data_ptr(), C.byref(dn) if dn is not None else None, C.byref(dh),
                                    bits_out.data_ptr(), partial.data_ptr(), cap, _stream()), "eb_forward")
    _rec("eb_forward", z, params, z_hat, noise)


def eb_pack(raw_table: torch.Tensor, quantiles: torch.Tensor, packed: torch.Tensor, Cn: int) -> None:
    L.check(L.lib().tdvc_eb_pack(raw_table.data_ptr(), quantiles.data_ptr(), packed.data_ptr(), Cn, _stream()), "eb_pack")


def eb_param_chain(dpacked: torch.Tensor, raw_table: torch.Tensor, grad_table: torch.Tensor, scale: float, Cn: int) -> None:
    assert dpacked.is_contiguous() and dpacked.dtype == torch.float32 and tuple(dpacked.shape) == (Cn, 59)
    L.check(L.lib().tdvc_eb_param_chain(dpacked.data_ptr(), raw_table.data_ptr(), grad_table.data_ptr(), scale, Cn, _stream()), "eb_param_chain")


def eb_aux(params: torch.Tensor, quantiles: torch.Tensor, target: float, dq: torch.Tensor, loss: torch.Tensor, Cn: int) -> None:
    assert quantiles.is_contiguous() and dq.is_contiguous() and quantiles.numel() == 3 * Cn == dq.numel() and dq.dtype == torch.float32
    L.check(L.lib().tdvc_eb_aux(params.data_ptr(), quantiles.data_ptr(), target, dq.data_ptr(), loss.data_ptr(), Cn, _stream()), "eb_aux")


def eb_backward(z: FM, params: torch.Tensor, noise: FM, gscale: float, dz: FM, dparams: torch.Tensor) -> None:
    d1, d2, d3 = z.desc(), noise.desc(), dz.desc()
    L.check(L.lib().tdvc_eb_backward(C.byref(d1), params.data_ptr(), C.byref(d2), gscale, C.byref(d3), dparams.data_ptr(), _stream()), "eb_backward")


def gc_backward(y: FM, gp: FM, noise: FM, gscale: float, dy: FM, dgp: FM) -> None:
    d1, d2, d3, d4, d5 = y.desc(), gp.desc(), noise.desc(), dy.desc(), dgp.desc()
    L.check(L.lib().tdvc_gc_backward(C.byref(d1), C.byref(d2), C.byref(d3), gscale, C.byref(d4), C.byref(d5), _stream()), "gc_backward")


def gc_forward(y: FM, gp: FM, bits_out: torch.Tensor, noise: FM | None = None):
    numel = y.N * y.H * y.W * y.C
    cap = (numel + 255) // 256
    partial = torch.empty(cap, dtype=torch.float32, device=y.t.device)
    dy, dg = y.desc(), gp.desc()
    dn = noise.desc() if noise is not None else None
    L.check(L.lib().tdvc_gc_forward(C.byref(dy), C.byref(dg), C.byref(dn) if dn is not None else None,
                                    bits_out.data_ptr(), partial.data_ptr(), cap, _stream()), "gc_forward")
    _rec("gc_forward", y, gp, noise)


def quantize(y: FM, out: FM, noise: FM | None = None) -> FM:
    dy, do = y.desc(), out.desc()
    dn = noise.desc() if noise is not None else None
    L.check(L.lib().tdvc_quantize(C.byref(dy), C.byref(dn) if dn is not None else None, C.byref(do), _stream()), "quantize")
    _rec("quantize", y, out, noise)
    return out


def pmf_to_quantized_cdf(pmf: np.ndarray, precision: int = 16) -> np.ndarray:
    p = np.ascontiguousarray(pmf, dtype=np.float32)
    out = np.zeros(p.size + 1, dtype=np.int32)
    L.check(L.lib().tdvc_pmf_to_quantized_cdf(p.ctypes.data, p.size, precision, out.ctypes.data), "pmf_to_quantized_cdf")
    return out


class CdfTables:

    def __init__(self, cdf: torch.Tensor, lengths: torch.Tensor, offsets: torch.Tensor):
        self.cdf = np.ascontiguousarray(cdf.detach().cpu().numpy(), dtype=np.int32)
        self.sizes = np.ascontiguousarray(lengths.detach().cpu().numpy().reshape(-1), dtype=np.int32)
        self.offsets = np.ascontiguousarray(offsets.detach().cpu().numpy().reshape(-1), dtype=np.int32)
        self.stride = self.cdf.shape[1]


def rans_encode(symbols: np.ndarray, indexes: np.ndarray, t: CdfTables) -> bytes:
    s = np.ascontiguousarray(symbols.reshape(-1), dtype=np.int32)
    i = np.ascontiguousarray(indexes.reshape(-1), dtype=np.int32)
    out = np.empty(4 * s.size + 64, dtype=np.uint8)
    n = L.lib().tdvc_rans_encode(s.ctypes.data, i.ctypes.data, s.size, t.cdf.ctypes.data, t.stride, t.sizes.ctypes.data,
                                 t.offsets.ctypes.data, out.ctypes.data, out.size)
    if n < 0:
        L.check(int(n), "rans_encode")
    return out[:n].tobytes()


class RansDecoder:
    def __init__(self, data: bytes):
        self._buf = np.frombuffer(data, dtype=np.uint8)
        self._h = L.lib().tdvc_rans_decoder_create(self._buf.ctypes.data, self._buf.size)
        if not self._h:
            L.check(-1, "rans_decoder_create")

    def decode(self, indexes: np.ndarray, t: CdfTables) -> np.ndarray:
        i = np.ascontiguousarray(indexes.reshape(-1), dtype=np.int32)
        out = np.empty(i.size, dtype=np.int32)
        L.check(L.lib().tdvc_rans_decoder_decode(self._h, i.ctypes.data, i.size, t.cdf.ctypes.data, t.stride,
                                                 t.sizes.ctypes.data, t.offsets.ctypes.data, out.ctypes.data), "rans_decode")
        return out

    def close(self):
        if self._h:
            L.lib().tdvc_rans_decoder_destroy(self._h)
            self._h = None

    def __del__(self):
        self.close()


def ar_decode_serial(data: bytes, t: CdfTables, y_hat: FM, params: FM, x1: FM, pc: FM, descs: list, gp: FM, pos_table: torch.Tensor,
                     M: int, W: int, scale_table: torch.Tensor, idx: torch.Tensor, sym: torch.Tensor) -> None:
    buf = np.frombuffer(data, dtype=np.uint8)
    arr = (L.ConvDesc * len(descs))(*descs)
    dy, dp, dx, dc, dg = y_hat.desc(), params.desc(), x1.desc(), pc.desc(), gp.desc()
    L.check(L.lib().tdvc_ar_decode_serial(buf.ctypes.data, buf.size, t.cdf.ctypes.data, t.stride, t.sizes.ctypes.data, t.offsets.ctypes.data,
                                          C.byref(dy), C.byref(dp), C.byref(dx), C.byref(dc), arr, len(descs), C.byref(dg),
                                          pos_table.data_ptr(), pos_table.shape[0], M, W, scale_table.data_ptr(), scale_table.numel(),
                                          idx.data_ptr(), sym.data_ptr(), _stream()), "ar_decode_serial")


def ar_wavefront(data: bytes | None, t: CdfTables | None, y: FM | None, y_hat: FM, params: FM, x1: FM, pc: FM, descs: list, gp: FM,
                 pos: torch.Tensor, step_sizes: np.ndarray, M: int, W: int, scale_table: torch.Tensor, idx: torch.Tensor, sym: torch.Tensor) -> None:
    buf = np.frombuffer(data, dtype=np.uint8) if data is not None else None
    arr = (L.ConvDesc * len(descs))(*descs)
    ss = np.ascontiguousarray(step_sizes, dtype=np.int32)
    dyh, dp, dx, dc, dg = y_hat.desc(), params.desc(), x1.desc(), pc.desc(), gp.desc()
    dy = y.desc() if y is not None else None
    L.check(L.lib().tdvc_ar_wavefront(buf.ctypes.data if buf is not None else None, buf.size if buf is not None else 0,
                                      t.cdf.ctypes.data if t else None, t.stride if t else 0, t.sizes.ctypes.data if t else None,
                                      t.offsets.ctypes.data if t else None, C.byref(dy) if dy is not None else None, C.byref(dyh), C.byref(dp),
                                      C.byref(dx), C.byref(dc), arr, len(descs), C.byref(dg), pos.data_ptr(), ss.ctypes.data, ss.size, M, W,
                                      scale_table.data_ptr(), scale_table.numel(), idx.data_ptr(), sym.data_ptr(), _stream()), "ar_wavefront")


def ar_gather(y_hat: FM, params: FM, pos: torch.Tensor, npos: int, x1: FM, pc: FM):
    dy, dp, dx, dc = y_hat.desc(), params.desc(), x1.desc(), pc.desc()
    L.check(L.lib().tdvc_ar_gather(C.byref(dy), C.byref(dp), pos.data_ptr(), npos, C.byref(dx), C.byref(dc), _stream()), "ar_gather")


def ar_quantize(y: FM | None, gp: FM, pos: torch.Tensor, npos: int, table: torch.Tensor, y_hat: FM, symbols: torch.Tensor,
                indexes: torch.Tensor, symbols_in: torch.Tensor | None = None):
    dg, dh = gp.desc(), y_hat.desc()
    dy = y.desc() if y is not None else None
    L.check(L.lib().tdvc_ar_quantize(C.byref(dy) if dy is not None else None, C.byref(dg), pos.data_ptr(), npos, table.data_ptr(),
                                     table.numel(), symbols_in.data_ptr() if symbols_in is not None else None, C.byref(dh),
                                     symbols.data_ptr(), indexes.data_ptr(), _stream()), "ar_quantize")


def ar_indexes(gp: FM, pos: torch.Tensor, npos: int, table: torch.Tensor, M: int, W: int, indexes: torch.Tensor):
    dg = gp.desc()
    L.check(L.lib().tdvc_ar_indexes(C.byref(dg), pos.data_ptr(), npos, table.data_ptr(), table.numel(), M, W,
                                    indexes.data_ptr(), _stream()), "ar_indexes")


def round_symbols(z: FM, median: torch.Tensor) -> torch.Tensor:
    out = torch.empty((z.N, z.H, z.W, z.C), dtype=torch.int32, device=z.t.device)
    dz = z.desc()
    L.check(L.lib().tdvc_round_symbols(C.byref(dz), median.data_ptr(), out.data_ptr(), _stream()), "round_symbols")
    return out


def dcn_v2_forward(input, weight, bias, offset, mask, kh, kw, sh, sw, ph, pw, dh, dw, deformable_group):
    ts = (input, weight, bias, offset, mask)
    for t in ts:
        if not (torch.is_tensor(t) and t.is_cuda):
            raise RuntimeError("dcn_v2_forward: all tensors must be CUDA/HIP tensors (Not compiled with CPU support)")
        if t.dtype != torch.float32:
            raise RuntimeError("dcn_v2_forward: fp32 tensors only")
    input, weight, bias, offset, mask = [t.contiguous() for t in ts]
    B, Cc, H, W = input.shape
    Cout, Ck, kh_, kw_ = weight.shape
    if (kh_, kw_) != (kh, kw):
        raise RuntimeError(f"Input shape and kernel shape wont match: ({kh} x {kw} vs {kh_} x {kw_}).")
    if Cc != Ck:
        raise RuntimeError(f"Input shape and kernel channels wont match: ({Cc} vs {Ck}).")
    Ho = (H + 2 * ph - (dh * (kh - 1) + 1)) // sh + 1
    Wo = (W + 2 * pw - (dw * (kw - 1) + 1)) // sw + 1
    if offset.shape != (B, 2 * deformable_group * kh * kw, Ho, Wo) or mask.shape != (B, deformable_group * kh * kw, Ho, Wo):
        raise RuntimeError("dcn_v2_forward: offset/mask shape mismatch")
    out = torch.empty((B, Cout, Ho, Wo), dtype=torch.float32, device=input.device)
    with torch.cuda.device(input.device):
        L.check(L.lib().tdvc_dcn_v2_forward_f32(input.data_ptr(), weight.data_ptr(), bias.data_ptr(), offset.data_ptr(),
                                                mask.data_ptr(), out.data_ptr(), B, Cc, H, W, Cout, kh, kw, sh, sw, ph, pw,
                                                dh, dw, deformable_group, _stream()), "dcn_v2_forward")
    return out
```

Baseline: 48.01 frames/s.

## Fuse GDN/IGDN normalization into the conv_row 3x3 128-channel kernel epilogue

```diff
diff --git a/include/tdvc_hip.h b/include/tdvc_hip.h
--- a/include/tdvc_hip.h
+++ b/include/tdvc_hip.h
@@ -50,12 +50,16 @@
   int32_t bcast_T;
   float bcast_slope;
   float* chan_sum;
+  int32_t post_gdn;
+  const void* post_gdn_w;
+  const float* post_gdn_beta;
 } tdvc_conv_desc;
 
 int tdvc_abi_version(void);
 const char* tdvc_last_error(void);
 int tdvc_prepare_device(void);
 const char* tdvc_last_conv_kernel(void);
+void tdvc_debug_enable_row_gdn(int enable);
 
 
 int tdvc_conv_plan(int cin, int kh, int kw, int stride);
diff --git a/tdvc_amd/_lib.py b/tdvc_amd/_lib.py
--- a/tdvc_amd/_lib.py
+++ b/tdvc_amd/_lib.py
@@ -11,6 +11,7 @@
 ACT_NONE, ACT_RELU, ACT_LRELU, ACT_CLAMP01, ACT_SIGMOID = 0, 1, 2, 3, 4
 GDN_NONE, GDN_FWD, GDN_INV = 0, 1, 2
 OUT_NHWC, OUT_SHUFFLE2, OUT_NCHW_F32 = 0, 1, 2
+EINVAL, ENOSUP = -1, -2
 
 
 class FMapDesc(C.Structure):
@@ -26,7 +27,8 @@
                 ("ck", C.c_int32), ("square_input", C.c_int32), ("gdn", C.c_int32),
                 ("aux", FMapDesc), ("act", C.c_int32), ("slope", C.c_float),
                 ("round_before_act", C.c_int32), ("res", FMapDesc), ("res2", FMapDesc), ("out_mode", C.c_int32), ("s2d", C.c_int32),
-                ("bcast_T", C.c_int32), ("bcast_slope", C.c_float), ("chan_sum", C.c_void_p)]
+                ("bcast_T", C.c_int32), ("bcast_slope", C.c_float), ("chan_sum", C.c_void_p),
+                ("post_gdn", C.c_int32), ("post_gdn_w", C.c_void_p), ("post_gdn_beta", C.c_void_p)]
 
 
 class DcnDesc(C.Structure):
@@ -55,6 +57,7 @@
     "tdvc_conv_chan_sum_rows": (_i, [C.POINTER(ConvDesc)]),
     "tdvc_last_error": (C.c_char_p, []),
     "tdvc_last_conv_kernel": (C.c_char_p, []),
+    "tdvc_debug_enable_row_gdn": (None, [_i]),
     "tdvc_prepare_device": (_i, []),
     "tdvc_conv_plan": (_i, [_i, _i, _i, _i]),
     "tdvc_conv_packed_bytes": (_i64, [_i, _i, _i, _i]),
diff --git a/tdvc_amd/csrc/conv_mfma.hip b/tdvc_amd/csrc/conv_mfma.hip
--- a/tdvc_amd/csrc/conv_mfma.hip
+++ b/tdvc_amd/csrc/conv_mfma.hip
@@ -14,6 +14,8 @@
 bool conv_v11_eligible(const tdvc_conv_desc* d, const ConvParams& p, int Ho, int Wo);
 int launch_conv_row(int geo, const ConvParams& p, int N, hipStream_t st);
 int conv_row_geometry(const tdvc_conv_desc* d, const ConvParams& p, int Ho, int Wo);
+bool conv_row_gdn_eligible(const tdvc_conv_desc* d, const ConvParams& p, int Ho, int Wo);
+int launch_conv_row_gdn(const tdvc_conv_desc* d, const ConvParams& p, int N, hipStream_t st);
 int launch_conv_v10(const ConvParams& p, int cout_blocks, int N, hipStream_t st);
 bool conv_v10_eligible(const tdvc_conv_desc* d, const ConvParams& p, int Ho, int Wo);
 int launch_conv_v9(const ConvParams& p, int ck8, int cout_tiles32, int N, hipStream_t st);
@@ -360,6 +362,16 @@
   }
   hipStream_t st = reinterpret_cast<hipStream_t>(stream);
   auto chose = [](const char* name) { snprintf(g_last_kernel, sizeof(g_last_kernel), "%s", name); };
+  if (d->post_gdn) {
+    const bool row = !d->bcast_T && !d->s2d && !conv_v9_eligible(d, Ho, Wo, conv_v3_eligible(d, Ho, Wo)) && !gdn128_eligible(d, p, Ho, Wo) &&
+                     !conv_v5_eligible(d, Ho, Wo) && !conv_c8_eligible(d, p, Ho, Wo) && !conv_n16_eligible(d, Ho, Wo) && conv_row_gdn_eligible(d, p, Ho, Wo);
+    if (!row) {
+      tdvc_set_error("tdvc_conv2d: the GDN post-op needs a 3x3 / stride 1 conv 128 -> 128 on conv_row, no activation, fp16 NHWC output, at most one fp16 residual");
+      return TDVC_ENOSUP;
+    }
+    chose("conv_row+gdn");
+    return launch_conv_row_gdn(d, p, d->x.N, st);
+  }
   if (d->bcast_T) {
     TDVC_CHECK(d->bcast_T == 4 && d->kh == 1 && d->kw == 1 && d->stride == 1 && d->pad == 0 && d->cout == 64 && d->y.C == 64 && d->y.sp >= 4 * 64 &&
                    d->y.dtype == TDVC_F16 && d->out_mode == TDVC_OUT_NHWC && d->act == TDVC_ACT_NONE && !d->gdn && !d->res.p && !d->res2.p &&
diff --git a/tdvc_amd/csrc/conv_row.hip b/tdvc_amd/csrc/conv_row.hip
--- a/tdvc_amd/csrc/conv_row.hip
+++ b/tdvc_amd/csrc/conv_row.hip
@@ -6,11 +6,12 @@
 
 namespace {
 
-enum { GEO_C128 = 0, GEO_C64 = 1, GEO_C128W = 2, GEO_S2D64 = 3 };
+enum { GEO_C128 = 0, GEO_C64 = 1, GEO_C128W = 2, GEO_S2D64 = 3, GEO_C128G = 4 };
 template <int GID> struct RowGeo;
 template <> struct RowGeo<GEO_C128> { static constexpr int NKC = 4, KH = 3, KW = 3, SW = 32, NCG = 8, PIECES = 9, XRING = 8, PF = 6, HD = 4, DMA_POS = 1, CORIG = 128; static constexpr bool S2D = false; };
 template <> struct RowGeo<GEO_C64> { static constexpr int NKC = 2, KH = 3, KW = 3, SW = 64, NCG = 4, PIECES = 9, XRING = 8, PF = 6, HD = 4, DMA_POS = 2, CORIG = 64; static constexpr bool S2D = false; };
 template <> struct RowGeo<GEO_C128W> { static constexpr int NKC = 4, KH = 3, KW = 3, SW = 64, NCG = 4, PIECES = 17, XRING = 6, PF = 4, HD = 2, DMA_POS = 2, CORIG = 128; static constexpr bool S2D = false; };
+template <> struct RowGeo<GEO_C128G> { static constexpr int NKC = 4, KH = 3, KW = 3, SW = 32, NCG = 8, PIECES = 9, XRING = 5, PF = 3, HD = 1, DMA_POS = 1, CORIG = 128; static constexpr bool S2D = false; };
 template <> struct RowGeo<GEO_S2D64> { static constexpr int NKC = 8, KH = 2, KW = 2, SW = 32, NCG = 8, PIECES = 17, XRING = 6, PF = 4, HD = 2, DMA_POS = 1, CORIG = 64; static constexpr bool S2D = true; };
 template <int GID> struct RowDerived : RowGeo<GID> {
   using G = RowGeo<GID>;
@@ -21,18 +22,28 @@
   static constexpr int ROWB = G::PIECES * 1024;
   static constexpr int STEPS = (G::KH * G::KW * 4 + 1) / 2;
   static constexpr int NP = G::PIECES / 4 + 1;
-  static constexpr int X0 = 0, S0 = G::XRING * ROWB, B0 = S0 + 4 * 8192, LDS = B0 + 512;
+  static constexpr int X0 = 0, S0 = G::XRING * ROWB;
   static_assert(G::SW * CO * 2 == 8192, "a staging row is 8 KB = 512 items of 16 bytes");
   static_assert((G::SW + G::KW - 1) * PXB <= ROWB && (G::PIECES % 4) == 1, "ring row");
   static_assert(G::SW / 16 == 2 * (8 / G::NCG), "a wave computes two column blocks");
   static_assert(G::PF + 2 <= G::XRING && G::PF >= G::HD + 2, "ring conditions (BI = 2)");
-  static_assert(G::HD == 4 || G::HD == 2, "land_wait(): four-step history with the odd piece going round the loaders, or two steps with a fixed owner");
+  static_assert(G::HD == 4 || G::HD == 2 || G::HD == 1, "land_wait(): four-step history with the odd piece going round the loaders, or two / one steps with a fixed owner");
+};
+constexpr int RW_BI = 2;
+constexpr int RW_SROW = 8192;
+constexpr int RW_NTHR = 512;
+template <int GID, int GDN> struct RowLds {
+  static constexpr int SDEL = GDN ? 2 * RW_BI : RW_BI;
+  static constexpr int SRING = SDEL + RW_BI;
+  static constexpr int NRING = GDN ? 2 * RW_BI : 0;
+  static constexpr int S0 = RowDerived<GID>::S0, N0 = S0 + SRING * RW_SROW, GM0 = N0 + NRING * RW_SROW, B0 = GM0 + (GDN ? 32768 : 0), BETA0 = B0 + 512;
+  static constexpr int LDS = BETA0 + (GDN ? 512 : 0);
+  static_assert(SRING >= SDEL + RW_BI, "staging ring");
+  static_assert(!GDN || NRING >= 2 * RW_BI, "norm ring");
+  static_assert(!GDN || SDEL - RW_BI >= RW_BI, "norm / store one barrier apart");
+  static_assert(!GDN || GID == GEO_C128G, "GDN post-op: its own 128-channel geometry");
   static_assert(LDS <= 160 * 1024, "LDS");
 };
-constexpr int RW_BI = 2;
-constexpr int RW_SRING = 2 * RW_BI;
-constexpr int RW_SROW = 8192;
-constexpr int RW_NTHR = 512;
 #ifndef RW_DMA_POS
 #define RW_DMA_POS G::DMA_POS
 #endif
@@ -43,6 +54,8 @@
   const half_t* res; long r1_sn; int r1_sp;
   const half_t* w;
   const float* bias;
+  const half_t* gw;
+  const float* gbeta;
   const half_t* zeros;
   half_t* dump;
   int N, H, W;
@@ -108,10 +121,13 @@
   return -1;
 }
 
-template <int GID, int ACT, int NRES, bool SHUF>
+template <int GID, int ACT, int NRES, bool SHUF, int GDN = 0>
 __global__ __launch_bounds__(RW_NTHR, 1) void conv_row_kernel(const RowParams p) {
   using G = RowDerived<GID>;
+  using L = RowLds<GID, GDN>;
+  static_assert(!GDN || (ACT == 0 && !SHUF), "GDN post-op: no activation, plain NHWC");
   constexpr int NKC = G::NKC, KH = G::KH, KW = G::KW, SW = G::SW, CO = G::CO, PXB = G::PXB, XRING = G::XRING, PF = G::PF, NP = G::NP;
+  constexpr int SDEL = L::SDEL, SRING = L::SRING, NRING = L::NRING;
   constexpr int NG = rw_ngroups<GID>(), G0 = rw_first_group_of_row0<GID>();
   extern __shared__ __attribute__((aligned(1024))) unsigned char smem[];
   const unsigned lds0 = static_cast<unsigned>(reinterpret_cast<uintptr_t>(smem));
@@ -147,8 +163,14 @@
         if (rw_frag<GID>(tap / KW, tap % KW, kc))
           wf[tap * NKC + kc] = *reinterpret_cast<const half8*>(wb + ((long)kc * G::STEPS + tap * 2) * 512);
   }
-  if (tid < CO) reinterpret_cast<float*>(smem + G::B0)[tid] = p.bias[cbk * CO + tid];
-  const int boff = G::B0 + (16 * cg + 4 * kb) * 4;
+  if (tid < CO) reinterpret_cast<float*>(smem + L::B0)[tid] = p.bias[cbk * CO + tid];
+  if constexpr (GDN != 0) {
+    if (tid < 128) reinterpret_cast<float*>(smem + L::BETA0)[tid] = p.gbeta[tid];
+#pragma unroll
+    for (int j = 0; j < 4; ++j)
+      reinterpret_cast<half8*>(smem + L::GM0)[tid + RW_NTHR * j] = reinterpret_cast<const half8*>(p.gw)[tid + RW_NTHR * j];
+  }
+  const int boff = L::B0 + (16 * cg + 4 * kb) * 4;
 
   int foff[KW];
 #pragma unroll
@@ -200,6 +222,7 @@
   const half4 sl4 = {hs, hs, hs, hs};
   f32x4 acc[KH][2];
   half8 r1v[2] = {};
+  constexpr bool NORM = LOADER && GDN != 0;
 
   for (long pos = run_begin; pos < run_end;) {
     const int sid = (int)(pos / p.H);
@@ -272,16 +295,20 @@
     asm volatile("s_waitcnt vmcnt(0)" ::: "memory");
     rw_barrier();
 
-    const int K = (rows + KH - 1 + RW_BI + RW_BI - 1) & ~(RW_BI - 1);
+    const int K = (rows + KH - 1 + SDEL + RW_BI - 1) & ~(RW_BI - 1);
     auto land_wait = [&](int nvm) __attribute__((always_inline)) {
       if (!nvm) { asm volatile("s_waitcnt vmcnt(0)" ::: "memory"); return; }
       if constexpr (G::HD == 4) {
         static_assert(G::HD != 4 || NP == 3, "vmcnt(9)");
         asm volatile("s_waitcnt vmcnt(9)" ::: "memory");
-      } else {
+      } else if constexpr (G::HD == 2) {
         static_assert(G::HD != 2 || NP == 5, "vmcnt(10) / vmcnt(8)");
         if (wq == 0) asm volatile("s_waitcnt vmcnt(10)" ::: "memory");
         else asm volatile("s_waitcnt vmcnt(8)" ::: "memory");
+      } else {
+        static_assert(G::HD != 1 || NP == 3, "vmcnt(3) / vmcnt(2)");
+        if (wq == 0) asm volatile("s_waitcnt vmcnt(3)" ::: "memory");
+        else asm volatile("s_waitcnt vmcnt(2)" ::: "memory");
       }
     };
 
@@ -289,15 +316,56 @@
       constexpr int PH = decltype(PHc)::value;
       constexpr bool FULL = decltype(FULLc)::value;
       constexpr int SD = (PH + 1) % KH;
+      if constexpr (NORM) {
+        const int nr = k - RW_BI, nrow = ra + nr - (KH - 1);
+        if (FULL || (nrow >= ra && nrow < rb)) {
+          const unsigned char* tb = smem + L::S0 + rw_slot<SRING>(nr) * RW_SROW;
+          int ln = lane;
+          asm volatile("" : "+v"(ln));
+          const int r = ln & 31, hh = ln >> 5, gr = rw_g(r);
+          const int toff = r * (CO * 2) + ((hh ^ gr) << 4);
+          const f32x16 zero = {};
+          f32x16 na;
+#pragma unroll
+          for (int ks = 0; ks < 8; ++ks) {
+            const half8 a = *reinterpret_cast<const half8*>(smem + L::GM0 + ((wq * 8 + ks) * 64 + ln) * 16);
+            half8 b = *reinterpret_cast<const half8*>(tb + (toff ^ (ks << 5)));
+            b = b * b;
+            na = __builtin_amdgcn_mfma_f32_32x32x16_f16(a, b, ks == 0 ? zero : na, 0, 0, 0);
+            if (ks & 1) __builtin_amdgcn_sched_barrier(0);
+          }
+          unsigned char* nb = smem + L::N0 + (nr & (NRING - 1)) * RW_SROW;
+#pragma unroll
+          for (int g = 0; g < 4; ++g) {
+            const f32x4 b4 = *reinterpret_cast<const f32x4*>(smem + L::BETA0 + (32 * wq + 8 * g + 4 * hh) * 4);
+            half4 o;
+#pragma unroll
+            for (int i = 0; i < 4; ++i) o[i] = (half_t)(na[4 * g + i] + b4[i]);
+            *reinterpret_cast<half4*>(nb + r * (CO * 2) + (((4 * wq + g) ^ gr) << 4) + 8 * hh) = o;
+          }
+        }
+      }
       if constexpr (!LOADER) {
-        const int srow = ra + k - RW_BI - (KH - 1);
+        const int srow = ra + k - SDEL - (KH - 1);
         if (FULL || (srow >= ra && srow < rb)) {
-          const unsigned char* sb = smem + G::S0 + ((k - RW_BI) & (RW_SRING - 1)) * RW_SROW;
+          const unsigned char* sb = smem + L::S0 + rw_slot<SRING>(k - SDEL) * RW_SROW;
           half_t* const yrow = const_cast<half_t*>(yimg) + srow * yrow_stride;
 #pragma unroll
           for (int j = 0; j < 2; ++j) {
             half8 yv = *reinterpret_cast<const half8*>(sb + (s_t + 256 * j) * 16);
-            if constexpr (NRES >= 1) yv = yv + r1v[j];
+            if constexpr (GDN != 0) {
+              const half8 nv = *reinterpret_cast<const half8*>(smem + L::N0 + ((k - SDEL) & (NRING - 1)) * RW_SROW + (s_t + 256 * j) * 16);
+              half8 o;
+#pragma unroll
+              for (int e = 0; e < 8; ++e) {
+                float v = (float)yv[e] * (GDN == TDVC_GDN_INV ? sqrtf((float)nv[e]) : rsqrtf((float)nv[e]));
+                if constexpr (NRES >= 1) v += (float)r1v[j][e];
+                o[e] = (half_t)v;
+              }
+              yv = o;
+            } else if constexpr (NRES >= 1) {
+              yv = yv + r1v[j];
+            }
             *reinterpret_cast<half8*>(s_ok[j] ? yrow + y_lo[j] : p.dump + (s_t + 256 * j) * 8) = yv;
           }
         }
@@ -309,10 +377,11 @@
           for (int j = 0; j < 2; ++j) r1v[j] = *reinterpret_cast<const half8*>(rrow + r_lo[j]);
         }
       }
+      if constexpr (GDN != 0) __builtin_amdgcn_sched_barrier(0);
       int nvm = 0;
       if (FULL || k <= last_in) {
         const unsigned char* xb = smem + G::X0 + rw_slot<XRING>(k) * G::ROWB;
-        constexpr int FBN = (PXB == 256 && (NRES == 1 || GID == GEO_C128W)) ? 2 : 3;
+        constexpr int FBN = (PXB == 256 && (NRES == 1 || GID == GEO_C128W || GDN)) ? 2 : 3;
         half8 fb[FBN][2];
         auto load_group = [&](int gi, int buf) __attribute__((always_inline)) {
           const int g = rw_group_at<GID>(gi), kc = g / KW, dx = g - KW * kc;
@@ -344,7 +413,7 @@
         }
         if (RW_DMA_POS == 2 && LOADER && k + PF <= last_in) nvm = issue_row(k + PF);
         {
-          unsigned char* sb = smem + G::S0 + (k & (RW_SRING - 1)) * RW_SROW;
+          unsigned char* sb = smem + L::S0 + rw_slot<SRING>(k) * RW_SROW;
 #pragma unroll
           for (int cb = 0; cb < 2; ++cb) {
             const f32x4 v = acc[SD][cb];
@@ -369,7 +438,7 @@
         if (k0 + 2 < kend) step(std::integral_constant<int, 2 % KH>{}, FULLc, k0 + 2);
       }
     };
-    constexpr int KF = ((RW_BI + KH - 1 + KH - 1) / KH) * KH;
+    constexpr int KF = ((SDEL + KH - 1 + KH - 1) / KH) * KH;
     int k = 0;
     for (; k < KF; k += KH) steps_of(std::false_type{}, k, KF);
     for (; k + KH - 1 <= last_in; k += KH) steps_of(std::true_type{}, k, k + KH);
@@ -385,6 +454,9 @@
 
 static int g_row_enabled = 15;
 extern "C" void tdvc_debug_enable_conv_row(int enable) { g_row_enabled = enable; }
+
+static bool g_row_gdn_enabled = true;
+extern "C" void tdvc_debug_enable_row_gdn(int enable) { g_row_gdn_enabled = enable != 0; }
 
 static bool row_off() {
   static const bool off = getenv("TDVC_CONV_NO_ROW") != nullptr || getenv("TDVC_CONV_V1") != nullptr;
@@ -412,8 +484,16 @@
   return -1;
 }
 
+bool conv_row_gdn_eligible(const tdvc_conv_desc* d, const ConvParams& p, int Ho, int Wo) {
+  if (!g_row_gdn_enabled || (d->post_gdn != TDVC_GDN_FWD && d->post_gdn != TDVC_GDN_INV) || !d->post_gdn_w || !d->post_gdn_beta) return false;
+  if ((reinterpret_cast<uintptr_t>(d->post_gdn_w) & 15) || d->gdn || d->square_input || d->s2d || d->bcast_T || d->chan_sum || d->res2.p) return false;
+  if (d->cout != 128 || d->act != TDVC_ACT_NONE || d->out_mode != TDVC_OUT_NHWC || d->y.dtype != TDVC_F16 || d->y.C < 128) return false;
+  if (d->res.p && (d->res.dtype != TDVC_F16 || d->res.C < 128)) return false;
+  return (long)Ho * Wo >= 8192 && conv_row_geometry(d, p, Ho, Wo) == GEO_C128;
+}
+
 template <int GID>
-static int launch_conv_row_t(const ConvParams& p, int N, hipStream_t st) {
+static int launch_conv_row_t(const ConvParams& p, int N, hipStream_t st, const tdvc_conv_desc* gd) {
   using G = RowDerived<GID>;
   const void* zeros = nullptr;
   void* dump = nullptr;
@@ -423,6 +503,9 @@
   q.y = reinterpret_cast<half_t*>(p.y.p); q.y_sn = p.y.sn; q.y_sp = p.y.sp;
   q.res = reinterpret_cast<const half_t*>(p.res.p); q.r1_sn = p.res.p ? p.res.sn : 0; q.r1_sp = p.res.p ? p.res.sp : 0;
   q.w = p.w; q.bias = p.bias;
+  const int gdn = gd ? gd->post_gdn : TDVC_GDN_NONE;
+  q.gw = gd ? reinterpret_cast<const half_t*>(gd->post_gdn_w) : nullptr;
+  q.gbeta = gd ? gd->post_gdn_beta : nullptr;
   q.zeros = reinterpret_cast<const half_t*>(zeros);
   q.dump = reinterpret_cast<half_t*>(dump);
   q.N = N; q.H = p.Ho; q.W = p.Wo; q.Win = p.W;
@@ -442,29 +525,38 @@
   }
   const bool has1 = q.res != nullptr;
   const int act = q.slope == 1.f ? 0 : (q.slope == 0.f ? 1 : 2);
-  auto go = [&](auto kern) -> int {
-    hipError_t err = hipFuncSetAttribute(reinterpret_cast<const void*>(kern), hipFuncAttributeMaxDynamicSharedMemorySize, G::LDS);
+  auto go = [&](auto kern, int lds) -> int {
+    hipError_t err = hipFuncSetAttribute(reinterpret_cast<const void*>(kern), hipFuncAttributeMaxDynamicSharedMemorySize, lds);
     if (err != hipSuccess) { tdvc_set_error("conv_row: hipFuncSetAttribute failed: %s", hipGetErrorString(err)); return (int)err; }
-    hipLaunchKernelGGL(kern, dim3(grid), dim3(RW_NTHR), G::LDS, st, q);
+    hipLaunchKernelGGL(kern, dim3(grid), dim3(RW_NTHR), lds, st, q);
     return 0;
   };
   const int nres = has1 ? 1 : 0;
   int rc = TDVC_EINVAL;
-#define RW_CASE(A, R, S) if (act == A && nres == R && shuf == S) rc = go(&conv_row_kernel<GID, A, R, S>);
-  RW_CASE(0, 0, false) RW_CASE(0, 1, false) RW_CASE(1, 0, false) RW_CASE(1, 1, false) RW_CASE(2, 0, false) RW_CASE(2, 1, false)
+#define RW_CASE(A, R, S) if (act == A && nres == R && shuf == S) rc = go(&conv_row_kernel<GID, A, R, S>, RowLds<GID, 0>::LDS);
+  if constexpr (GID != GEO_C128G) {
+    RW_CASE(0, 0, false) RW_CASE(0, 1, false) RW_CASE(1, 0, false) RW_CASE(1, 1, false) RW_CASE(2, 0, false) RW_CASE(2, 1, false)
+  }
   if constexpr (GID == GEO_C128) {
     RW_CASE(0, 0, true) RW_CASE(0, 1, true) RW_CASE(1, 0, true) RW_CASE(1, 1, true) RW_CASE(2, 0, true) RW_CASE(2, 1, true)
   }
 #undef RW_CASE
+  if constexpr (GID == GEO_C128G) {
+#define RW_GDN(R, M) if (act == 0 && nres == R && !shuf && gdn == M) rc = go(&conv_row_kernel<GID, 0, R, false, M>, RowLds<GID, M>::LDS);
+    RW_GDN(0, TDVC_GDN_FWD) RW_GDN(1, TDVC_GDN_FWD) RW_GDN(0, TDVC_GDN_INV) RW_GDN(1, TDVC_GDN_INV)
+#undef RW_GDN
+  }
   if (rc) return rc;
-  return tdvc_launch_status("tdvc_conv2d(conv_row)");
+  return tdvc_launch_status(gdn ? "tdvc_conv2d(conv_row+gdn)" : "tdvc_conv2d(conv_row)");
 }
 
 int launch_conv_row(int geo, const ConvParams& p, int N, hipStream_t st) {
   switch (geo) {
-    case GEO_C128: return launch_conv_row_t<GEO_C128>(p, N, st);
-    case GEO_C64: return launch_conv_row_t<GEO_C64>(p, N, st);
-    case GEO_C128W: return launch_conv_row_t<GEO_C128W>(p, N, st);
-    default: return launch_conv_row_t<GEO_S2D64>(p, N, st);
-  }
-}
+    case GEO_C128: return launch_conv_row_t<GEO_C128>(p, N, st, nullptr);
+    case GEO_C64: return launch_conv_row_t<GEO_C64>(p, N, st, nullptr);
+    case GEO_C128W: return launch_conv_row_t<GEO_C128W>(p, N, st, nullptr);
+    default: return launch_conv_row_t<GEO_S2D64>(p, N, st, nullptr);
+  }
+}
+
+int launch_conv_row_gdn(const tdvc_conv_desc* d, const ConvParams& p, int N, hipStream_t st) { return launch_conv_row_t<GEO_C128G>(p, N, st, d); }
diff --git a/tdvc_amd/csrc/lib.cpp b/tdvc_amd/csrc/lib.cpp
--- a/tdvc_amd/csrc/lib.cpp
+++ b/tdvc_amd/csrc/lib.cpp
@@ -15,7 +15,7 @@
   va_end(ap);
 }
 
-extern "C" int tdvc_abi_version(void) { return 4; }
+extern "C" int tdvc_abi_version(void) { return 5; }
 extern "C" const char* tdvc_last_error(void) { return g_err; }
 
 namespace {
diff --git a/tdvc_amd/model/coder.py b/tdvc_amd/model/coder.py
--- a/tdvc_amd/model/coder.py
+++ b/tdvc_amd/model/coder.py
@@ -57,7 +57,7 @@
         self.gamma_reparam = NonNegativeParametrizer()
         self.gamma = nn.Parameter(self.gamma_reparam.init(gamma_init * torch.eye(ch)))
 
-    def run(self, x: FM, out: FM | None = None, res: FM | None = None) -> FM:
+    def packed(self):
         def build():
             g = self.gamma_reparam.effective(self.gamma.detach())
             b = self.beta_reparam.effective(self.beta.detach())
@@ -65,8 +65,17 @@
             pc = ops.pack_conv(g.reshape(c, c, 1, 1).contiguous(), b.contiguous(), stride=1, pad=0, device=self.gamma.device)
             pc.owner = self
             return pc
-        pc = self._pk("gdn", build)
-        return ops.conv(x, pc, out=out, square=True, gdn=GDN_INV if self.inverse else GDN_FWD, aux=x, res=res)
+        return self._pk("gdn", build)
+
+    def run(self, x: FM, out: FM | None = None, res: FM | None = None) -> FM:
+        return ops.conv(x, self.packed(), out=out, square=True, gdn=GDN_INV if self.inverse else GDN_FWD, aux=x, res=res)
+
+    def run_after_conv(self, x: FM, pc, out: FM | None = None, res: FM | None = None) -> FM:
+        if ops.TAPE is None and not x.f32:
+            y = ops.conv(x, pc, out=out, res=res, post_gdn=(self.packed(), self.inverse))
+            if y is not None:
+                return y
+        return self.run(ops.conv(x, pc), out=out, res=res)
 
     def refresh_packed(self):
         pc = self.__dict__.get("_packed", {}).get("gdn")
@@ -168,6 +177,9 @@
 
     def run(self, x: FM, out: FM | None = None) -> FM:
         t = ops.conv(x, pk_conv(self, "c1", self.conv1), **LR)
+        if ops.TAPE is None and not t.f32:
+            idt = x if self.skip is None else ops.conv(x, pk_conv(self, "sk", self.skip))
+            return self.gdn.run_after_conv(t, pk_conv(self, "c2", self.conv2), out=out, res=idt)
         t = ops.conv(t, pk_conv(self, "c2", self.conv2))
         idt = x if self.skip is None else ops.conv(x, pk_conv(self, "sk", self.skip))
         return self.gdn.run(t, out=out, res=idt)
@@ -184,6 +196,9 @@
 
     def run(self, x: FM, out: FM | None = None) -> FM:
         t = ops.conv(x, pk_conv(self, "sp", self.subpel_conv[0], shuffle=True), **LR)
+        if ops.TAPE is None and not t.f32:
+            up = ops.conv(x, pk_conv(self, "up", self.upsample[0], shuffle=True))
+            return self.igdn.run_after_conv(t, pk_conv(self, "c", self.conv), out=out, res=up)
         t = ops.conv(t, pk_conv(self, "c", self.conv))
         up = ops.conv(x, pk_conv(self, "up", self.upsample[0], shuffle=True))
         return self.igdn.run(t, out=out, res=up)
diff --git a/tdvc_amd/ops.py b/tdvc_amd/ops.py
--- a/tdvc_amd/ops.py
+++ b/tdvc_amd/ops.py
@@ -399,7 +399,8 @@
 
 def conv(x: FM, pc: PackedConv, out: FM | None = None, act=ACT_NONE, slope=0.0, res: FM | None = None,
          res2: FM | None = None, gdn=GDN_NONE, aux: FM | None = None, square=False, out_dtype=None,
-         round16=False, nchw_out: torch.Tensor | None = None, bcast_T=0, bcast_slope=0.0, chan_sum: list | None = None) -> FM | torch.Tensor:
+         round16=False, nchw_out: torch.Tensor | None = None, bcast_T=0, bcast_slope=0.0, chan_sum: list | None = None,
+         post_gdn: tuple | None = None) -> FM | torch.Tensor | None:
     d, ret, Ho, Wo, pc, rec_pc = conv_desc(x, pc, out, act, slope, res, res2, gdn, aux, square, out_dtype, round16, nchw_out, bcast_T, bcast_slope)
     if chan_sum is not None and TAPE is None and FUSE_CHAN_SUM:
         rows = L.lib().tdvc_conv_chan_sum_rows(C.byref(d))
@@ -411,6 +412,28 @@
         raise L.TdvcHipError("conv: the fp32 form has no backward (the fp32 islands are an inference / coding mode)")
     if bcast_T and TAPE is not None and not _IN_BACKWARD:
         raise L.TdvcHipError("conv: bcast_T is an inference-only fusion (under the tape use conv + bcast_add_act)")
+    if post_gdn is not None:
+        gpc, inverse = post_gdn
+        if TAPE is not None or x.f32 or gpc.ck != 32 or gpc.cout != 128:
+            return None
+        d.post_gdn = GDN_INV if inverse else GDN_FWD
+        d.post_gdn_w, d.post_gdn_beta = gpc.w.data_ptr(), gpc.bias.data_ptr()
+        e0 = e1 = None
+        if PROFILE is not None:
+            e0, e1 = torch.cuda.Event(enable_timing=True), torch.cuda.Event(enable_timing=True)
+            e0.record()
+        rc = L.lib().tdvc_conv2d(C.byref(d), _stream())
+        if rc == L.ENOSUP:
+            return None
+        L.check(rc, "conv2d(post_gdn)")
+        if PROFILE is not None:
+            e1.record()
+            px = x.N * Ho * Wo
+            fl = 2.0 * px * pc.cout * x.C * len(pc.taps) + 2.0 * px * 128 * 128
+            PROFILE.append(dict(kernel=L.lib().tdvc_last_conv_kernel().decode(),
+                                shape=f"{pc.kh}x{pc.kw} s{pc.stride} {x.C}->{pc.cout} +{'igdn' if inverse else 'gdn'} @{x.H}x{x.W}", e0=e0, e1=e1,
+                                flops=fl, flops_real=fl, bytes=2.0 * x.N * (x.H * x.W * x.C + Ho * Wo * pc.cout * (2 if res is not None else 1))))
+        return ret
     if PROFILE is not None:
         e0, e1 = torch.cuda.Event(enable_timing=True), torch.cuda.Event(enable_timing=True)
         e0.record()
```

Result: no change. 48.47 frames/s (median of 6 runs) (+0.9%).
